# alexklibisz/deep-calcium

Measured on AMD Instinct MI355X. Metric: 512x512 summary images/sec (train step), higher is better.
Workload: dtype f32 (fp16x3 split, fp32 accumulate); 1 GPU; UNet2DS train step (fwd+BCE+bwd+Keras-Adam), batch=16 512x512 per GPU, nfb=32 (BASELINE.json configs[2]; configs[3] at 8 GPUs); global_batch=16, parallelism=dp1, bn=local

## Files before the change

### deep_calcium_amd/_build.py

```python
import os
import subprocess
import sys
from concurrent.futures import ThreadPoolExecutor

HERE = os.path.dirname(os.path.abspath(__file__))
CSRC = os.path.join(HERE, 'csrc')
LIBDIR = os.path.join(HERE, 'lib')
LIB = os.path.join(LIBDIR, 'libdcunet.so')
SOURCES = ['common.cpp', 'comm.cpp', 'nf_score.cpp', 'tape.cpp', 'igemm_conv.hip', 'igemm_f16x3.hip', 'igemm_pp.hip', 'wgrad.hip', 'wgrad_f16x3.hip', 'bwd_joint.hip', 'conv_c1.hip', 'elementwise.hip', 'series.hip', 'traces.hip', 'footprints.hip', 'roi_pairs.hip', 'trace_pairs.hip', 'frame_quality.hip', 'dff.hip', 'deconv.hip', 'trace_dyn.hip', 'spikes.hip', 'spikes_train.hip', 'motion.hip']
FLAGS = ['--offload-arch=gfx950', '-O3', '-std=c++17', '-fPIC', '-Wall', '-Wno-unused-function']
FILE_FLAGS = {'nf_score.cpp': ['-ffp-contract=off'], 'series.hip': ['-ffp-contract=off'], 'traces.hip': ['-ffp-contract=off'],
              'footprints.hip': ['-ffp-contract=off'], 'roi_pairs.hip': ['-ffp-contract=off'], 'trace_pairs.hip': ['-ffp-contract=off'],
              'frame_quality.hip': ['-ffp-contract=off'], 'dff.hip': ['-ffp-contract=off'], 'deconv.hip': ['-ffp-contract=off'],
              'trace_dyn.hip': ['-ffp-contract=off']}


def _hipcc():
    for c in (os.environ.get('HIPCC'), '/opt/rocm/bin/hipcc', 'hipcc'):
        if c and (os.path.isabs(c) and os.path.exists(c) or not os.path.isabs(c)):
            return c
    raise RuntimeError('hipcc not found')


def _newest_src():
    t = 0.0
    for root, _, files in os.walk(CSRC):
        for f in files:
            t = max(t, os.path.getmtime(os.path.join(root, f)))
    t = max(t, os.path.getmtime(os.path.join(HERE, '..', 'include', 'dcunet.h')))
    return t


def build(force=False, verbose=True):
    os.makedirs(LIBDIR, exist_ok=True)
    if not force and os.path.exists(LIB) and os.path.getmtime(LIB) >= _newest_src():
        return LIB
    hipcc = _hipcc()
    from . import _gen_tape
    _gen_tape.generate()
    objdir = os.path.join(LIBDIR, 'obj')
    os.makedirs(objdir, exist_ok=True)

    def compile_one(src):
        obj = os.path.join(objdir, os.path.splitext(src)[0] + '.o')
        cmd = [hipcc] + FLAGS + FILE_FLAGS.get(src, []) + ['-x', 'hip', '-c', os.path.join(CSRC, src), '-o', obj]
        r = subprocess.run(cmd, capture_output=True, text=True)
        if r.returncode != 0:
            raise RuntimeError('hipcc failed for %s:\n%s' % (src, r.stderr[-6000:]))
        if verbose and r.stderr.strip():
            sys.stderr.write(r.stderr)
        return obj

    with ThreadPoolExecutor(max_workers=4) as ex:
        objs = list(ex.map(compile_one, SOURCES))
    r = subprocess.run([hipcc, '--offload-arch=gfx950', '-shared', '-fPIC', '-o', LIB] + objs,
                       capture_output=True, text=True)
    if r.returncode != 0:
        raise RuntimeError('link failed:\n%s' % r.stderr[-6000:])
    return LIB


if __name__ == '__main__':
    print(build(force='--force' in sys.argv))
```

### deep_calcium_amd/csrc/tape_tramp.inc

```

static int t_dc_pack_weights(const DcArg* a) { return dc_pack_weights((const float*)a[0].p, (float*)a[1].p, (int)a[2].l, (int)a[3].l, (int)a[4].l, (long)a[5].l, (long)a[6].l, (long)a[7].l, (int)a[8].l, (dc_stream_t)a[9].p); }
static int t_dc_conv3x3_fwd(const DcArg* a) { return dc_conv3x3_fwd((const float*)a[0].p, (const float*)a[1].p, (const float*)a[2].p, (float*)a[3].p, (long)a[4].l, (double*)a[5].p, (const float*)a[6].p, (const float*)a[7].p, (int)a[8].l, (int)a[9].l, (int)a[10].l, (int)a[11].l, (int)a[12].l, (int)a[13].l, (dc_stream_t)a[14].p); }
static int t_dc_conv3x3_c1_fwd(const DcArg* a) { return dc_conv3x3_c1_fwd((const float*)a[0].p, (const float*)a[1].p, (const float*)a[2].p, (float*)a[3].p, (long)a[4].l, (double*)a[5].p, (const float*)a[6].p, (const float*)a[7].p, (int)a[8].l, (float*)a[9].p, (long)a[10].l, (int)a[11].l, (int)a[12].l, (int)a[13].l, (int)a[14].l, (dc_stream_t)a[15].p); }
static int t_dc_conv3x3_dgrad(const DcArg* a) { return dc_conv3x3_dgrad((const float*)a[0].p, (const float*)a[1].p, (float*)a[2].p, (int)a[3].l, (int)a[4].l, (int)a[5].l, (int)a[6].l, (int)a[7].l, (dc_stream_t)a[8].p); }
static int t_dc_conv3x3_wgrad(const DcArg* a) { return dc_conv3x3_wgrad((const float*)a[0].p, (const float*)a[1].p, (float*)a[2].p, (float*)a[3].p, (int)a[4].l, (int)a[5].l, (int)a[6].l, (int)a[7].l, (int)a[8].l, (dc_stream_t)a[9].p); }
static int t_dc_pack_weights_f16x3(const DcArg* a) { return dc_pack_weights_f16x3((const float*)a[0].p, (void*)a[1].p, (int)a[2].l, (int)a[3].l, (int)a[4].l, (long)a[5].l, (long)a[6].l, (long)a[7].l, (int)a[8].l, (dc_stream_t)a[9].p); }
static int t_dc_pack_weights_f16x3_batch(const DcArg* a) { return dc_pack_weights_f16x3_batch((const long*)a[0].p, (int)a[1].l, (int)a[2].l, (dc_stream_t)a[3].p); }
static int t_dc_conv3x3_fwd_f16x3(const DcArg* a) { return dc_conv3x3_fwd_f16x3((const float*)a[0].p, (const void*)a[1].p, (const float*)a[2].p, (float*)a[3].p, (long)a[4].l, (double*)a[5].p, (int)a[6].l, (const float*)a[7].p, (const float*)a[8].p, (int)a[9].l, (const float*)a[10].p, (long)a[11].l, (float*)a[12].p, (long)a[13].l, (float*)a[14].p, (int)a[15].l, (int)a[16].l, (int)a[17].l, (int)a[18].l, (int)a[19].l, (dc_stream_t)a[20].p); }
static int t_dc_conv3x3_dgrad_f16x3(const DcArg* a) { return dc_conv3x3_dgrad_f16x3((const float*)a[0].p, (const void*)a[1].p, (float*)a[2].p, (const float*)a[3].p, (const float*)a[4].p, (int)a[5].l, (float*)a[6].p, (int)a[7].l, (int)a[8].l, (int)a[9].l, (int)a[10].l, (int)a[11].l, (dc_stream_t)a[12].p); }
static int t_dc_convT2x2_fwd_f16x3(const DcArg* a) { return dc_convT2x2_fwd_f16x3((const float*)a[0].p, (const void*)a[1].p, (const float*)a[2].p, (float*)a[3].p, (long)a[4].l, (double*)a[5].p, (const float*)a[6].p, (const float*)a[7].p, (int)a[8].l, (const float*)a[9].p, (long)a[10].l, (float*)a[11].p, (long)a[12].l, (int)a[13].l, (int)a[14].l, (int)a[15].l, (int)a[16].l, (int)a[17].l, (dc_stream_t)a[18].p); }
static int t_dc_convT2x2_dgrad_f16x3(const DcArg* a) { return dc_convT2x2_dgrad_f16x3((const float*)a[0].p, (const void*)a[1].p, (float*)a[2].p, (const float*)a[3].p, (const float*)a[4].p, (int)a[5].l, (float*)a[6].p, (int)a[7].l, (int)a[8].l, (int)a[9].l, (int)a[10].l, (int)a[11].l, (dc_stream_t)a[12].p); }
static int t_dc_conv3x3_wgrad_f16x3(const DcArg* a) { return dc_conv3x3_wgrad_f16x3((const float*)a[0].p, (const float*)a[1].p, (float*)a[2].p, (float*)a[3].p, (const float*)a[4].p, (const float*)a[5].p, (int)a[6].l, (int)a[7].l, (int)a[8].l, (int)a[9].l, (int)a[10].l, (dc_stream_t)a[11].p); }
static int t_dc_convT2x2_wgrad_f16x3(const DcArg* a) { return dc_convT2x2_wgrad_f16x3((const float*)a[0].p, (const float*)a[1].p, (float*)a[2].p, (float*)a[3].p, (const float*)a[4].p, (const float*)a[5].p, (int)a[6].l, (int)a[7].l, (int)a[8].l, (int)a[9].l, (int)a[10].l, (dc_stream_t)a[11].p); }
static int t_dc_bn_stats_finalize_affine(const DcArg* a) { return dc_bn_stats_finalize_affine((const double*)a[0].p, (int)a[1].l, (int)a[2].l, (int)a[3].l, (double)a[4].d, (float)a[5].d, (float)a[6].d, (float*)a[7].p, (float*)a[8].p, (float*)a[9].p, (float*)a[10].p, (const float*)a[11].p, (const float*)a[12].p, (float*)a[13].p, (float*)a[14].p, (float*)a[15].p, (dc_stream_t)a[16].p); }
static int t_dc_conv3x3_fwd_bnin_f16x3(const DcArg* a) { return dc_conv3x3_fwd_bnin_f16x3((const float*)a[0].p, (const float*)a[1].p, (const float*)a[2].p, (const float*)a[3].p, (const void*)a[4].p, (const float*)a[5].p, (float*)a[6].p, (long)a[7].l, (double*)a[8].p, (int)a[9].l, (const float*)a[10].p, (const float*)a[11].p, (int)a[12].l, (float*)a[13].p, (int)a[14].l, (int)a[15].l, (int)a[16].l, (int)a[17].l, (int)a[18].l, (dc_stream_t)a[19].p); }
static int t_dc_convT2x2_fwd_bnin_f16x3(const DcArg* a) { return dc_convT2x2_fwd_bnin_f16x3((const float*)a[0].p, (const float*)a[1].p, (const float*)a[2].p, (const float*)a[3].p, (const void*)a[4].p, (const float*)a[5].p, (float*)a[6].p, (long)a[7].l, (double*)a[8].p, (const float*)a[9].p, (const float*)a[10].p, (int)a[11].l, (int)a[12].l, (int)a[13].l, (int)a[14].l, (int)a[15].l, (int)a[16].l, (dc_stream_t)a[17].p); }
static int t_dc_conv3x3_wgrad_bnin_f16x3(const DcArg* a) { return dc_conv3x3_wgrad_bnin_f16x3((const float*)a[0].p, (const float*)a[1].p, (const float*)a[2].p, (const float*)a[3].p, (const float*)a[4].p, (float*)a[5].p, (float*)a[6].p, (const float*)a[7].p, (int)a[8].l, (int)a[9].l, (int)a[10].l, (int)a[11].l, (int)a[12].l, (dc_stream_t)a[13].p); }
static int t_dc_convT2x2_wgrad_bnin_f16x3(const DcArg* a) { return dc_convT2x2_wgrad_bnin_f16x3((const float*)a[0].p, (const float*)a[1].p, (const float*)a[2].p, (const float*)a[3].p, (const float*)a[4].p, (float*)a[5].p, (float*)a[6].p, (const float*)a[7].p, (int)a[8].l, (int)a[9].l, (int)a[10].l, (int)a[11].l, (int)a[12].l, (dc_stream_t)a[13].p); }
static int t_dc_head_fwd_bnin(const DcArg* a) { return dc_head_fwd_bnin((const float*)a[0].p, (const float*)a[1].p, (const float*)a[2].p, (const float*)a[3].p, (const float*)a[4].p, (const uint8_t*)a[5].p, (float*)a[6].p, (float*)a[7].p, (long)a[8].l, (int)a[9].l, (dc_stream_t)a[10].p); }
static int t_dc_head_bwd_bnin(const DcArg* a) { return dc_head_bwd_bnin((const float*)a[0].p, (const float*)a[1].p, (const float*)a[2].p, (const float*)a[3].p, (const uint8_t*)a[4].p, (const float*)a[5].p, (float*)a[6].p, (float*)a[7].p, (int)a[8].l, (const double*)a[9].p, (long)a[10].l, (int)a[11].l, (dc_stream_t)a[12].p); }
static int t_dc_convT2x2_fwd(const DcArg* a) { return dc_convT2x2_fwd((const float*)a[0].p, (const float*)a[1].p, (const float*)a[2].p, (float*)a[3].p, (long)a[4].l, (double*)a[5].p, (const float*)a[6].p, (const float*)a[7].p, (int)a[8].l, (int)a[9].l, (int)a[10].l, (int)a[11].l, (int)a[12].l, (int)a[13].l, (dc_stream_t)a[14].p); }
static int t_dc_convT2x2_dgrad(const DcArg* a) { return dc_convT2x2_dgrad((const float*)a[0].p, (const float*)a[1].p, (float*)a[2].p, (int)a[3].l, (int)a[4].l, (int)a[5].l, (int)a[6].l, (int)a[7].l, (dc_stream_t)a[8].p); }
static int t_dc_convT2x2_wgrad(const DcArg* a) { return dc_convT2x2_wgrad((const float*)a[0].p, (const float*)a[1].p, (float*)a[2].p, (float*)a[3].p, (int)a[4].l, (int)a[5].l, (int)a[6].l, (int)a[7].l, (int)a[8].l, (dc_stream_t)a[9].p); }
static int t_dc_bn_stats_finalize(const DcArg* a) { return dc_bn_stats_finalize((const double*)a[0].p, (int)a[1].l, (int)a[2].l, (int)a[3].l, (double)a[4].d, (float)a[5].d, (float)a[6].d, (float*)a[7].p, (float*)a[8].p, (float*)a[9].p, (float*)a[10].p, (dc_stream_t)a[11].p); }
static int t_dc_bn_fold(const DcArg* a) { return dc_bn_fold((const float*)a[0].p, (const float*)a[1].p, (const float*)a[2].p, (const float*)a[3].p, (const float*)a[4].p, (float)a[5].d, (float*)a[6].p, (float*)a[7].p, (int)a[8].l, (dc_stream_t)a[9].p); }
static int t_dc_bn_relu_drop_fwd(const DcArg* a) { return dc_bn_relu_drop_fwd((const float*)a[0].p, (const float*)a[1].p, (const float*)a[2].p, (const float*)a[3].p, (const float*)a[4].p, (const uint8_t*)a[5].p, (float)a[6].d, (uint64_t)a[7].u, (float*)a[8].p, (long)a[9].l, (long)a[10].l, (int)a[11].l, (double)a[12].d, (float*)a[13].p, (dc_stream_t)a[14].p); }
static int t_dc_bn_relu_drop_pool_fwd(const DcArg* a) { return dc_bn_relu_drop_pool_fwd((const float*)a[0].p, (const float*)a[1].p, (const float*)a[2].p, (const float*)a[3].p, (const float*)a[4].p, (const uint8_t*)a[5].p, (float)a[6].d, (uint64_t)a[7].u, (float*)a[8].p, (long)a[9].l, (float*)a[10].p, (uint8_t*)a[11].p, (int)a[12].l, (int)a[13].l, (int)a[14].l, (int)a[15].l, (double)a[16].d, (float*)a[17].p, (dc_stream_t)a[18].p); }
static int t_dc_bn_bwd_reduce(const DcArg* a) { return dc_bn_bwd_reduce((const float*)a[0].p, (long)a[1].l, (const float*)a[2].p, (const float*)a[3].p, (const float*)a[4].p, (const float*)a[5].p, (const float*)a[6].p, (const uint8_t*)a[7].p, (float)a[8].d, (uint64_t)a[9].u, (float*)a[10].p, (float*)a[11].p, (long)a[12].l, (int)a[13].l, (dc_stream_t)a[14].p); }
static int t_dc_bn_bwd_apply(const DcArg* a) { return dc_bn_bwd_apply((const float*)a[0].p, (long)a[1].l, (const float*)a[2].p, (const float*)a[3].p, (const float*)a[4].p, (const float*)a[5].p, (const float*)a[6].p, (const uint8_t*)a[7].p, (float)a[8].d, (uint64_t)a[9].u, (const float*)a[10].p, (const float*)a[11].p, (float*)a[12].p, (float*)a[13].p, (float*)a[14].p, (long)a[15].l, (int)a[16].l, (dc_stream_t)a[17].p); }
static int t_dc_pow2_scale_from_absmax(const DcArg* a) { return dc_pow2_scale_from_absmax((const float*)a[0].p, (int)a[1].l, (float)a[2].d, (float*)a[3].p, (dc_stream_t)a[4].p); }
static int t_dc_bn_bwd_apply_finalize(const DcArg* a) { return dc_bn_bwd_apply_finalize((const float*)a[0].p, (const float*)a[1].p, (int)a[2].l, (int)a[3].l, (float)a[4].d, (float*)a[5].p, (float*)a[6].p, (dc_stream_t)a[7].p); }
static int t_dc_conv3x3_fwd_pool_f16x3(const DcArg* a) { return dc_conv3x3_fwd_pool_f16x3((const float*)a[0].p, (const void*)a[1].p, (const float*)a[2].p, (float*)a[3].p, (long)a[4].l, (const float*)a[5].p, (const float*)a[6].p, (int)a[7].l, (float*)a[8].p, (float*)a[9].p, (int)a[10].l, (int)a[11].l, (int)a[12].l, (int)a[13].l, (int)a[14].l, (dc_stream_t)a[15].p); }
static int t_dc_conv3x3_dgrad_bnred_f16x3(const DcArg* a) { return dc_conv3x3_dgrad_bnred_f16x3((const float*)a[0].p, (const void*)a[1].p, (float*)a[2].p, (const float*)a[3].p, (const float*)a[4].p, (int)a[5].l, (const float*)a[6].p, (const float*)a[7].p, (const float*)a[8].p, (const float*)a[9].p, (const float*)a[10].p, (float*)a[11].p, (float*)a[12].p, (int)a[13].l, (int)a[14].l, (int)a[15].l, (int)a[16].l, (int)a[17].l, (dc_stream_t)a[18].p); }
static int t_dc_head_bwd_bnin_bnred(const DcArg* a) { return dc_head_bwd_bnin_bnred((const float*)a[0].p, (const float*)a[1].p, (const float*)a[2].p, (const float*)a[3].p, (const uint8_t*)a[4].p, (const float*)a[5].p, (float*)a[6].p, (float*)a[7].p, (int)a[8].l, (const double*)a[9].p, (const float*)a[10].p, (const float*)a[11].p, (float*)a[12].p, (float*)a[13].p, (long)a[14].l, (int)a[15].l, (dc_stream_t)a[16].p); }
static int t_dc_convT2x2_dgrad_bnred_f16x3(const DcArg* a) { return dc_convT2x2_dgrad_bnred_f16x3((const float*)a[0].p, (const void*)a[1].p, (float*)a[2].p, (const float*)a[3].p, (const float*)a[4].p, (int)a[5].l, (const float*)a[6].p, (const float*)a[7].p, (const float*)a[8].p, (const float*)a[9].p, (const float*)a[10].p, (float*)a[11].p, (float*)a[12].p, (int)a[13].l, (int)a[14].l, (int)a[15].l, (int)a[16].l, (int)a[17].l, (dc_stream_t)a[18].p); }
static int t_dc_maxpool2x2_bwd_bnred(const DcArg* a) { return dc_maxpool2x2_bwd_bnred((const float*)a[0].p, (const uint8_t*)a[1].p, (const float*)a[2].p, (long)a[3].l, (float*)a[4].p, (const float*)a[5].p, (const float*)a[6].p, (const float*)a[7].p, (const float*)a[8].p, (const float*)a[9].p, (const uint8_t*)a[10].p, (float)a[11].d, (uint64_t)a[12].u, (float*)a[13].p, (float*)a[14].p, (int)a[15].l, (int)a[16].l, (int)a[17].l, (int)a[18].l, (dc_stream_t)a[19].p); }
static int t_dc_bn_bwd_finalize_dzin(const DcArg* a) { return dc_bn_bwd_finalize_dzin((const float*)a[0].p, (const float*)a[1].p, (int)a[2].l, (int)a[3].l, (const float*)a[4].p, (const float*)a[5].p, (const float*)a[6].p, (const float*)a[7].p, (double)a[8].d, (float*)a[9].p, (float*)a[10].p, (float*)a[11].p, (float*)a[12].p, (dc_stream_t)a[13].p); }
static int t_dc_conv3x3_dgrad_dzin_f16x3(const DcArg* a) { return dc_conv3x3_dgrad_dzin_f16x3((const float*)a[0].p, (const float*)a[1].p, (const float*)a[2].p, (const void*)a[3].p, (float*)a[4].p, (float*)a[5].p, (const float*)a[6].p, (const float*)a[7].p, (const float*)a[8].p, (const float*)a[9].p, (const float*)a[10].p, (float*)a[11].p, (float*)a[12].p, (int)a[13].l, (int)a[14].l, (int)a[15].l, (int)a[16].l, (int)a[17].l, (dc_stream_t)a[18].p); }
static int t_dc_conv3x3_wgrad_dzin_f16x3(const DcArg* a) { return dc_conv3x3_wgrad_dzin_f16x3((const float*)a[0].p, (const float*)a[1].p, (const float*)a[2].p, (const float*)a[3].p, (const float*)a[4].p, (const float*)a[5].p, (const float*)a[6].p, (float*)a[7].p, (float*)a[8].p, (int)a[9].l, (int)a[10].l, (int)a[11].l, (int)a[12].l, (int)a[13].l, (dc_stream_t)a[14].p); }
static int t_dc_conv3x3_c1_wgrad_dzin_zre(const DcArg* a) { return dc_conv3x3_c1_wgrad_dzin_zre((const float*)a[0].p, (const float*)a[1].p, (const float*)a[2].p, (const float*)a[3].p, (const float*)a[4].p, (float*)a[5].p, (float*)a[6].p, (int)a[7].l, (int)a[8].l, (int)a[9].l, (int)a[10].l, (dc_stream_t)a[11].p); }
static int t_dc_conv3x3_bwd_joint_f16x3(const DcArg* a) { return dc_conv3x3_bwd_joint_f16x3((const float*)a[0].p, (const float*)a[1].p, (const float*)a[2].p, (const float*)a[3].p, (const float*)a[4].p, (const float*)a[5].p, (const float*)a[6].p, (const void*)a[7].p, (float*)a[8].p, (const float*)a[9].p, (const float*)a[10].p, (const float*)a[11].p, (const float*)a[12].p, (const float*)a[13].p, (float*)a[14].p, (float*)a[15].p, (float*)a[16].p, (float*)a[17].p, (int)a[18].l, (int)a[19].l, (int)a[20].l, (int)a[21].l, (int)a[22].l, (dc_stream_t)a[23].p); }
static int t_dc_conv3x3_bwd_joint_r1_f16x3(const DcArg* a) { return dc_conv3x3_bwd_joint_r1_f16x3((const float*)a[0].p, (const float*)a[1].p, (const float*)a[2].p, (const float*)a[3].p, (const float*)a[4].p, (const float*)a[5].p, (const float*)a[6].p, (const float*)a[7].p, (const void*)a[8].p, (float*)a[9].p, (const float*)a[10].p, (const float*)a[11].p, (const float*)a[12].p, (const float*)a[13].p, (const float*)a[14].p, (float*)a[15].p, (float*)a[16].p, (float*)a[17].p, (float*)a[18].p, (int)a[19].l, (int)a[20].l, (int)a[21].l, (int)a[22].l, (int)a[23].l, (dc_stream_t)a[24].p); }
static int t_dc_bn_stats_reduce(const DcArg* a) { return dc_bn_stats_reduce((const double*)a[0].p, (int)a[1].l, (int)a[2].l, (int)a[3].l, (double*)a[4].p, (dc_stream_t)a[5].p); }
static int t_dc_bn_stats_rows_fold(const DcArg* a) { return dc_bn_stats_rows_fold((const double*)a[0].p, (int)a[1].l, (int)a[2].l, (int)a[3].l, (int)a[4].l, (double*)a[5].p, (dc_stream_t)a[6].p); }
static int t_dc_bn_stats_finalize_sums(const DcArg* a) { return dc_bn_stats_finalize_sums((const double*)a[0].p, (int)a[1].l, (double)a[2].d, (float)a[3].d, (float)a[4].d, (float*)a[5].p, (float*)a[6].p, (float*)a[7].p, (float*)a[8].p, (const float*)a[9].p, (const float*)a[10].p, (float*)a[11].p, (float*)a[12].p, (float*)a[13].p, (dc_stream_t)a[14].p); }
static int t_dc_bn_bwd_apply_count(const DcArg* a) { return dc_bn_bwd_apply_count((const float*)a[0].p, (long)a[1].l, (const float*)a[2].p, (const float*)a[3].p, (const float*)a[4].p, (const float*)a[5].p, (const float*)a[6].p, (const uint8_t*)a[7].p, (float)a[8].d, (uint64_t)a[9].u, (const float*)a[10].p, (const float*)a[11].p, (float*)a[12].p, (float*)a[13].p, (float*)a[14].p, (long)a[15].l, (double)a[16].d, (int)a[17].l, (dc_stream_t)a[18].p); }
static int t_dc_maxpool2x2_fwd(const DcArg* a) { return dc_maxpool2x2_fwd((const float*)a[0].p, (long)a[1].l, (float*)a[2].p, (uint8_t*)a[3].p, (int)a[4].l, (int)a[5].l, (int)a[6].l, (int)a[7].l, (dc_stream_t)a[8].p); }
static int t_dc_maxpool2x2_bwd(const DcArg* a) { return dc_maxpool2x2_bwd((const float*)a[0].p, (const uint8_t*)a[1].p, (const float*)a[2].p, (long)a[3].l, (float*)a[4].p, (int)a[5].l, (int)a[6].l, (int)a[7].l, (int)a[8].l, (dc_stream_t)a[9].p); }
static int t_dc_upsample2x_drop_fwd(const DcArg* a) { return dc_upsample2x_drop_fwd((const float*)a[0].p, (float*)a[1].p, (long)a[2].l, (const uint8_t*)a[3].p, (float)a[4].d, (uint64_t)a[5].u, (const float*)a[6].p, (long)a[7].l, (float*)a[8].p, (long)a[9].l, (int)a[10].l, (int)a[11].l, (int)a[12].l, (int)a[13].l, (dc_stream_t)a[14].p); }
static int t_dc_upsample2x_drop_bwd(const DcArg* a) { return dc_upsample2x_drop_bwd((const float*)a[0].p, (long)a[1].l, (const uint8_t*)a[2].p, (float)a[3].d, (uint64_t)a[4].u, (float*)a[5].p, (int)a[6].l, (int)a[7].l, (int)a[8].l, (int)a[9].l, (dc_stream_t)a[10].p); }
static int t_dc_head_fwd(const DcArg* a) { return dc_head_fwd((const float*)a[0].p, (const float*)a[1].p, (const float*)a[2].p, (const uint8_t*)a[3].p, (float*)a[4].p, (float*)a[5].p, (long)a[6].l, (int)a[7].l, (dc_stream_t)a[8].p); }
static int t_dc_head_bwd(const DcArg* a) { return dc_head_bwd((const float*)a[0].p, (const float*)a[1].p, (const uint8_t*)a[2].p, (const float*)a[3].p, (float*)a[4].p, (float*)a[5].p, (int)a[6].l, (const double*)a[7].p, (long)a[8].l, (int)a[9].l, (dc_stream_t)a[10].p); }
static int t_dc_head_fwd_bwd(const DcArg* a) { return dc_head_fwd_bwd((const float*)a[0].p, (const float*)a[1].p, (const float*)a[2].p, (const float*)a[3].p, (const float*)a[4].p, (const uint8_t*)a[5].p, (float*)a[6].p, (float*)a[7].p, (float*)a[8].p, (float*)a[9].p, (int)a[10].l, (const float*)a[11].p, (const float*)a[12].p, (float*)a[13].p, (float*)a[14].p, (long)a[15].l, (int)a[16].l, (dc_stream_t)a[17].p); }
static int t_dc_head_fwd_bwd_s(const DcArg* a) { return dc_head_fwd_bwd_s((const float*)a[0].p, (const float*)a[1].p, (const float*)a[2].p, (const float*)a[3].p, (const float*)a[4].p, (const uint8_t*)a[5].p, (float*)a[6].p, (float*)a[7].p, (float*)a[8].p, (float*)a[9].p, (int)a[10].l, (const float*)a[11].p, (const float*)a[12].p, (float*)a[13].p, (float*)a[14].p, (long)a[15].l, (int)a[16].l, (dc_stream_t)a[17].p); }
static int t_dc_head_bwd_bnin_bnred_s(const DcArg* a) { return dc_head_bwd_bnin_bnred_s((const float*)a[0].p, (const float*)a[1].p, (const float*)a[2].p, (const float*)a[3].p, (const uint8_t*)a[4].p, (const float*)a[5].p, (float*)a[6].p, (float*)a[7].p, (int)a[8].l, (const double*)a[9].p, (const float*)a[10].p, (const float*)a[11].p, (float*)a[12].p, (float*)a[13].p, (long)a[14].l, (int)a[15].l, (dc_stream_t)a[16].p); }
static int t_dc_head_grad_finalize(const DcArg* a) { return dc_head_grad_finalize((const float*)a[0].p, (int)a[1].l, (int)a[2].l, (float*)a[3].p, (float*)a[4].p, (dc_stream_t)a[5].p); }
static int t_dc_reduce_partials(const DcArg* a) { return dc_reduce_partials((const float*)a[0].p, (int)a[1].l, (long)a[2].l, (float)a[3].d, (float*)a[4].p, (float*)a[5].p, (dc_stream_t)a[6].p); }
static int t_dc_reduce_partials_f64(const DcArg* a) { return dc_reduce_partials_f64((const float*)a[0].p, (int)a[1].l, (int)a[2].l, (double*)a[3].p, (dc_stream_t)a[4].p); }
static int t_dc_bn_bwd_finalize(const DcArg* a) { return dc_bn_bwd_finalize((const float*)a[0].p, (int)a[1].l, (int)a[2].l, (float*)a[3].p, (float*)a[4].p, (dc_stream_t)a[5].p); }
static int t_dc_adam_step_flat(const DcArg* a) { return dc_adam_step_flat((float*)a[0].p, (const float*)a[1].p, (float*)a[2].p, (float*)a[3].p, (long)a[4].l, (float)a[5].d, (float)a[6].d, (float)a[7].d, (float)a[8].d, (float)a[9].d, (dc_stream_t)a[10].p); }
static int t_dc_gather_maps(const DcArg* a) { return dc_gather_maps((const float*)a[0].p, (const int*)a[1].p, (float*)a[2].p, (int)a[3].l, (long)a[4].l, (dc_stream_t)a[5].p); }
static int t_dc_tta_merge(const DcArg* a) { return dc_tta_merge((const float*)a[0].p, (const int*)a[1].p, (int)a[2].l, (int)a[3].l, (int)a[4].l, (int)a[5].l, (int)a[6].l, (double)a[7].d, (uint8_t*)a[8].p, (float*)a[9].p, (dc_stream_t)a[10].p); }
static int t_dc_round_window_u8(const DcArg* a) { return dc_round_window_u8((const float*)a[0].p, (int)a[1].l, (int)a[2].l, (int)a[3].l, (int)a[4].l, (int)a[5].l, (int)a[6].l, (int)a[7].l, (uint8_t*)a[8].p, (dc_stream_t)a[9].p); }
static int t_dc_series_accumulate(const DcArg* a) { return dc_series_accumulate((const void*)a[0].p, (int)a[1].l, (int)a[2].l, (long)a[3].l, (long)a[4].l, (uint16_t*)a[5].p, (int16_t*)a[6].p, (long*)a[7].p, (long*)a[8].p, (int*)a[9].p, (int)a[10].l, (int)a[11].l, (dc_stream_t)a[12].p); }
static int t_dc_series_accumulate_xy(const DcArg* a) { return dc_series_accumulate_xy((const void*)a[0].p, (int)a[1].l, (int)a[2].l, (long)a[3].l, (long*)a[4].p, (int)a[5].l, (int)a[6].l, (dc_stream_t)a[7].p); }
static int t_dc_series_finalize(const DcArg* a) { return dc_series_finalize((const long*)a[0].p, (const long*)a[1].p, (const long*)a[2].p, (float*)a[3].p, (float*)a[4].p, (float*)a[5].p, (int)a[6].l, (int)a[7].l, (long)a[8].l, (dc_stream_t)a[9].p); }
static int t_dc_image_standardize(const DcArg* a) { return dc_image_standardize((const float*)a[0].p, (float*)a[1].p, (float*)a[2].p, (int)a[3].l, (int)a[4].l, (dc_stream_t)a[5].p); }
static int t_dc_series_bin_time(const DcArg* a) { return dc_series_bin_time((const void*)a[0].p, (int)a[1].l, (int)a[2].l, (int)a[3].l, (int)a[4].l, (int)a[5].l, (int)a[6].l, (int*)a[7].p, (void*)a[8].p, (dc_stream_t)a[9].p); }
static int t_dc_roi_trace_accumulate(const DcArg* a) { return dc_roi_trace_accumulate((const void*)a[0].p, (int)a[1].l, (int)a[2].l, (long)a[3].l, (const int*)a[4].p, (const int*)a[5].p, (const int*)a[6].p, (int)a[7].l, (int)a[8].l, (long*)a[9].p, (long)a[10].l, (int)a[11].l, (int)a[12].l, (dc_stream_t)a[13].p); }
static int t_dc_roi_trace_finalize(const DcArg* a) { return dc_roi_trace_finalize((const long*)a[0].p, (long)a[1].l, (const int*)a[2].p, (int)a[3].l, (long)a[4].l, (float*)a[5].p, (float*)a[6].p, (dc_stream_t)a[7].p); }
static int t_dc_roi_wtrace_accumulate(const DcArg* a) { return dc_roi_wtrace_accumulate((const void*)a[0].p, (int)a[1].l, (int)a[2].l, (long)a[3].l, (const int*)a[4].p, (const int*)a[5].p, (const unsigned short*)a[6].p, (const int*)a[7].p, (int)a[8].l, (int)a[9].l, (long*)a[10].p, (long)a[11].l, (int)a[12].l, (int)a[13].l, (dc_stream_t)a[14].p); }
static int t_dc_roi_pixel_accumulate(const DcArg* a) { return dc_roi_pixel_accumulate((const void*)a[0].p, (int)a[1].l, (int)a[2].l, (long)a[3].l, (const int*)a[4].p, (const int*)a[5].p, (const int*)a[6].p, (int)a[7].l, (int)a[8].l, (const long*)a[9].p, (long)a[10].l, (long*)a[11].p, (int)a[12].l, (int)a[13].l, (int)a[14].l, (dc_stream_t)a[15].p); }
static int t_dc_roi_trace_moments(const DcArg* a) { return dc_roi_trace_moments((const long*)a[0].p, (long)a[1].l, (int)a[2].l, (long)a[3].l, (long*)a[4].p, (dc_stream_t)a[5].p); }
static int t_dc_roi_pixel_corr(const DcArg* a) { return dc_roi_pixel_corr((const long*)a[0].p, (int)a[1].l, (const int*)a[2].p, (const int*)a[3].p, (int)a[4].l, (int)a[5].l, (const int*)a[6].p, (const long*)a[7].p, (long)a[8].l, (float*)a[9].p, (dc_stream_t)a[10].p); }
static int t_dc_roi_pair_accumulate(const DcArg* a) { return dc_roi_pair_accumulate((const void*)a[0].p, (int)a[1].l, (int)a[2].l, (const int*)a[3].p, (const int*)a[4].p, (const long*)a[5].p, (const int*)a[6].p, (long)a[7].l, (int)a[8].l, (long*)a[9].p, (long*)a[10].p, (int)a[11].l, (long)a[12].l, (int)a[13].l, (int)a[14].l, (dc_stream_t)a[15].p); }
static int t_dc_roi_pair_corr(const DcArg* a) { return dc_roi_pair_corr((const long*)a[0].p, (const long*)a[1].p, (const int*)a[2].p, (const long*)a[3].p, (int)a[4].l, (int)a[5].l, (long)a[6].l, (long)a[7].l, (float*)a[8].p, (dc_stream_t)a[9].p); }
static int t_dc_series_fold_segment(const DcArg* a) { return dc_series_fold_segment((const long*)a[0].p, (const long*)a[1].p, (const long*)a[2].p, (const int*)a[3].p, (long)a[4].l, (long)a[5].l, (long*)a[6].p, (long*)a[7].p, (long*)a[8].p, (int*)a[9].p, (int)a[10].l, (int)a[11].l, (dc_stream_t)a[12].p); }
static int t_dc_series_finalize_pooled(const DcArg* a) { return dc_series_finalize_pooled((const long*)a[0].p, (const long*)a[1].p, (const long*)a[2].p, (float*)a[3].p, (float*)a[4].p, (float*)a[5].p, (int)a[6].l, (int)a[7].l, (long)a[8].l, (long)a[9].l, (dc_stream_t)a[10].p); }
static int t_dc_roi_pair_fold_segment(const DcArg* a) { return dc_roi_pair_fold_segment((long*)a[0].p, (long*)a[1].p, (const int*)a[2].p, (const long*)a[3].p, (const int*)a[4].p, (long)a[5].l, (int)a[6].l, (int)a[7].l, (long)a[8].l, (long)a[9].l, (long)a[10].l, (long*)a[11].p, (dc_stream_t)a[12].p); }
static int t_dc_roi_pair_corr_pooled(const DcArg* a) { return dc_roi_pair_corr_pooled((const long*)a[0].p, (const int*)a[1].p, (const long*)a[2].p, (int)a[3].l, (int)a[4].l, (long)a[5].l, (float*)a[6].p, (dc_stream_t)a[7].p); }
static int t_dc_roi_pixel_fold_segment(const DcArg* a) { return dc_roi_pixel_fold_segment((long*)a[0].p, (int)a[1].l, (const int*)a[2].p, (const int*)a[3].p, (int)a[4].l, (int)a[5].l, (const long*)a[6].p, (long)a[7].l, (long)a[8].l, (long*)a[9].p, (long*)a[10].p, (long*)a[11].p, (int)a[12].l, (int)a[13].l, (dc_stream_t)a[14].p); }
static int t_dc_roi_pixel_corr_pooled(const DcArg* a) { return dc_roi_pixel_corr_pooled((const long*)a[0].p, (const long*)a[1].p, (const long*)a[2].p, (int)a[3].l, (const int*)a[4].p, (const int*)a[5].p, (int)a[6].l, (int)a[7].l, (const int*)a[8].p, (float*)a[9].p, (dc_stream_t)a[10].p); }
static int t_dc_trace_pair_moments(const DcArg* a) { return dc_trace_pair_moments((const long*)a[0].p, (long)a[1].l, (int)a[2].l, (long)a[3].l, (int)a[4].l, (const int*)a[5].p, (long)a[6].l, (long*)a[7].p, (dc_stream_t)a[8].p); }
static int t_dc_trace_pair_corr(const DcArg* a) { return dc_trace_pair_corr((const long*)a[0].p, (long)a[1].l, (float*)a[2].p, (dc_stream_t)a[3].p); }
static int t_dc_frame_moments(const DcArg* a) { return dc_frame_moments((const void*)a[0].p, (int)a[1].l, (int)a[2].l, (const void*)a[3].p, (int)a[4].l, (int)a[5].l, (int)a[6].l, (int)a[7].l, (int)a[8].l, (int)a[9].l, (long*)a[10].p, (dc_stream_t)a[11].p); }
static int t_dc_frame_quality(const DcArg* a) { return dc_frame_quality((const long*)a[0].p, (int)a[1].l, (long)a[2].l, (long)a[3].l, (long)a[4].l, (float*)a[5].p, (float*)a[6].p, (dc_stream_t)a[7].p); }
static int t_dc_frame_gather(const DcArg* a) { return dc_frame_gather((const void*)a[0].p, (int)a[1].l, (const int*)a[2].p, (int)a[3].l, (int)a[4].l, (int)a[5].l, (void*)a[6].p, (dc_stream_t)a[7].p); }
static int t_dc_trace_combine(const DcArg* a) { return dc_trace_combine((const long*)a[0].p, (long)a[1].l, (const int*)a[2].p, (const long*)a[3].p, (const long*)a[4].p, (const long*)a[5].p, (int)a[6].l, (long)a[7].l, (long*)a[8].p, (dc_stream_t)a[9].p); }
static int t_dc_trace_baseline(const DcArg* a) { return dc_trace_baseline((const long*)a[0].p, (long)a[1].l, (int)a[2].l, (long)a[3].l, (int)a[4].l, (int)a[5].l, (long*)a[6].p, (float*)a[7].p, (dc_stream_t)a[8].p); }
static int t_dc_trace_scale(const DcArg* a) { return dc_trace_scale((const long*)a[0].p, (long)a[1].l, (const long*)a[2].p, (int)a[3].l, (long)a[4].l, (float*)a[5].p, (dc_stream_t)a[6].p); }
static int t_dc_trace_deconv_ar1(const DcArg* a) { return dc_trace_deconv_ar1((const void*)a[0].p, (int)a[1].l, (long)a[2].l, (int)a[3].l, (long)a[4].l, (double)a[5].d, (const double*)a[6].p, (const double*)a[7].p, (const double*)a[8].p, (void*)a[9].p, (double*)a[10].p, (double*)a[11].p, (int*)a[12].p, (dc_stream_t)a[13].p); }
static int t_dc_trace_deconv_ar1_host(const DcArg* a) { return dc_trace_deconv_ar1_host((const void*)a[0].p, (int)a[1].l, (long)a[2].l, (int)a[3].l, (long)a[4].l, (const double*)a[5].p, (const double*)a[6].p, (const double*)a[7].p, (double*)a[8].p, (double*)a[9].p, (int*)a[10].p); }
static int t_dc_trace_deconv_ar1_constrained(const DcArg* a) { return dc_trace_deconv_ar1_constrained((const void*)a[0].p, (int)a[1].l, (long)a[2].l, (int)a[3].l, (long)a[4].l, (double)a[5].d, (const double*)a[6].p, (const double*)a[7].p, (long)a[8].l, (int)a[9].l, (const double*)a[10].p, (const double*)a[11].p, (int)a[12].l, (void*)a[13].p, (void*)a[14].p, (double*)a[15].p, (double*)a[16].p, (int*)a[17].p, (double*)a[18].p, (double*)a[19].p, (int*)a[20].p, (dc_stream_t)a[21].p); }
static int t_dc_trace_deconv_search_step(const DcArg* a) { return dc_trace_deconv_search_step((const void*)a[0].p, (int)a[1].l, (long)a[2].l, (int)a[3].l, (long)a[4].l, (const double*)a[5].p, (long)a[6].l, (const void*)a[7].p, (const int*)a[8].p, (int)a[9].l, (void*)a[10].p, (double*)a[11].p, (double*)a[12].p, (int*)a[13].p, (dc_stream_t)a[14].p); }
static int t_dc_trace_deconv_ar1_constrained_host(const DcArg* a) { return dc_trace_deconv_ar1_constrained_host((const void*)a[0].p, (int)a[1].l, (long)a[2].l, (int)a[3].l, (long)a[4].l, (const double*)a[5].p, (int)a[6].l, (const double*)a[7].p, (const double*)a[8].p, (int)a[9].l, (double*)a[10].p, (double*)a[11].p, (int*)a[12].p, (double*)a[13].p, (double*)a[14].p, (int*)a[15].p); }
static int t_dc_trace_deconv_ar1_base(const DcArg* a) { return dc_trace_deconv_ar1_base((const void*)a[0].p, (int)a[1].l, (long)a[2].l, (int)a[3].l, (long)a[4].l, (double)a[5].d, (const double*)a[6].p, (const double*)a[7].p, (long)a[8].l, (const double*)a[9].p, (const double*)a[10].p, (const double*)a[11].p, (void*)a[12].p, (double*)a[13].p, (double*)a[14].p, (int*)a[15].p, (dc_stream_t)a[16].p); }
static int t_dc_trace_deconv_ar1_fit_base(const DcArg* a) { return dc_trace_deconv_ar1_fit_base((const void*)a[0].p, (int)a[1].l, (long)a[2].l, (int)a[3].l, (long)a[4].l, (double)a[5].d, (const double*)a[6].p, (const double*)a[7].p, (long)a[8].l, (const double*)a[9].p, (const double*)a[10].p, (int)a[11].l, (void*)a[12].p, (double*)a[13].p, (double*)a[14].p, (int*)a[15].p, (double*)a[16].p, (dc_stream_t)a[17].p); }
static int t_dc_trace_deconv_ar1_constrained_base(const DcArg* a) { return dc_trace_deconv_ar1_constrained_base((const void*)a[0].p, (int)a[1].l, (long)a[2].l, (int)a[3].l, (long)a[4].l, (double)a[5].d, (const double*)a[6].p, (const double*)a[7].p, (long)a[8].l, (int)a[9].l, (const double*)a[10].p, (const double*)a[11].p, (int)a[12].l, (void*)a[13].p, (void*)a[14].p, (double*)a[15].p, (double*)a[16].p, (int*)a[17].p, (double*)a[18].p, (double*)a[19].p, (double*)a[20].p, (int*)a[21].p, (dc_stream_t)a[22].p); }
static int t_dc_trace_deconv_base_step(const DcArg* a) { return dc_trace_deconv_base_step((const void*)a[0].p, (int)a[1].l, (long)a[2].l, (int)a[3].l, (long)a[4].l, (const double*)a[5].p, (long)a[6].l, (const void*)a[7].p, (const int*)a[8].p, (int)a[9].l, (void*)a[10].p, (double*)a[11].p, (double*)a[12].p, (double*)a[13].p, (int*)a[14].p, (double*)a[15].p, (dc_stream_t)a[16].p); }
static int t_dc_trace_deconv_ar1_fit_base_host(const DcArg* a) { return dc_trace_deconv_ar1_fit_base_host((const void*)a[0].p, (int)a[1].l, (long)a[2].l, (int)a[3].l, (long)a[4].l, (const double*)a[5].p, (long)a[6].l, (const double*)a[7].p, (const double*)a[8].p, (int)a[9].l, (double*)a[10].p, (double*)a[11].p, (int*)a[12].p, (double*)a[13].p); }
static int t_dc_trace_deconv_ar1_constrained_base_host(const DcArg* a) { return dc_trace_deconv_ar1_constrained_base_host((const void*)a[0].p, (int)a[1].l, (long)a[2].l, (int)a[3].l, (long)a[4].l, (const double*)a[5].p, (long)a[6].l, (int)a[7].l, (const double*)a[8].p, (const double*)a[9].p, (int)a[10].l, (double*)a[11].p, (double*)a[12].p, (int*)a[13].p, (double*)a[14].p, (double*)a[15].p, (double*)a[16].p, (int*)a[17].p); }
static int t_dc_trace_deconv_ar2(const DcArg* a) { return dc_trace_deconv_ar2((const void*)a[0].p, (int)a[1].l, (long)a[2].l, (int)a[3].l, (long)a[4].l, (double)a[5].d, (double)a[6].d, (const double*)a[7].p, (long)a[8].l, (const double*)a[9].p, (const double*)a[10].p, (const double*)a[11].p, (void*)a[12].p, (double*)a[13].p, (double*)a[14].p, (int*)a[15].p, (dc_stream_t)a[16].p); }
static int t_dc_trace_deconv_ar2_host(const DcArg* a) { return dc_trace_deconv_ar2_host((const void*)a[0].p, (int)a[1].l, (long)a[2].l, (int)a[3].l, (long)a[4].l, (double)a[5].d, (double)a[6].d, (const double*)a[7].p, (long)a[8].l, (const double*)a[9].p, (const double*)a[10].p, (const double*)a[11].p, (double*)a[12].p, (double*)a[13].p, (int*)a[14].p); }
static int t_dc_trace_deconv_ar2_constrained(const DcArg* a) { return dc_trace_deconv_ar2_constrained((const void*)a[0].p, (int)a[1].l, (long)a[2].l, (int)a[3].l, (long)a[4].l, (double)a[5].d, (double)a[6].d, (const double*)a[7].p, (long)a[8].l, (int)a[9].l, (const double*)a[10].p, (const double*)a[11].p, (int)a[12].l, (void*)a[13].p, (void*)a[14].p, (double*)a[15].p, (double*)a[16].p, (int*)a[17].p, (double*)a[18].p, (double*)a[19].p, (int*)a[20].p, (dc_stream_t)a[21].p); }
static int t_dc_trace_deconv_ar2_constrained_host(const DcArg* a) { return dc_trace_deconv_ar2_constrained_host((const void*)a[0].p, (int)a[1].l, (long)a[2].l, (int)a[3].l, (long)a[4].l, (double)a[5].d, (double)a[6].d, (const double*)a[7].p, (long)a[8].l, (int)a[9].l, (const double*)a[10].p, (const double*)a[11].p, (int)a[12].l, (double*)a[13].p, (double*)a[14].p, (int*)a[15].p, (double*)a[16].p, (double*)a[17].p, (int*)a[18].p); }
static int t_dc_trace_noise(const DcArg* a) { return dc_trace_noise((const void*)a[0].p, (int)a[1].l, (long)a[2].l, (int)a[3].l, (long)a[4].l, (double*)a[5].p, (dc_stream_t)a[6].p); }
static int t_dc_trace_ar1_estimate(const DcArg* a) { return dc_trace_ar1_estimate((const void*)a[0].p, (int)a[1].l, (long)a[2].l, (int)a[3].l, (long)a[4].l, (int)a[5].l, (const double*)a[6].p, (double*)a[7].p, (double*)a[8].p, (double*)a[9].p, (dc_stream_t)a[10].p); }
static int t_dc_ar1_tables(const DcArg* a) { return dc_ar1_tables((const double*)a[0].p, (int)a[1].l, (long)a[2].l, (double*)a[3].p, (long)a[4].l, (dc_stream_t)a[5].p); }
static int t_dc_trace_deconv_ar1_each(const DcArg* a) { return dc_trace_deconv_ar1_each((const void*)a[0].p, (int)a[1].l, (long)a[2].l, (int)a[3].l, (long)a[4].l, (const double*)a[5].p, (const double*)a[6].p, (long)a[7].l, (const double*)a[8].p, (const double*)a[9].p, (void*)a[10].p, (double*)a[11].p, (double*)a[12].p, (int*)a[13].p, (dc_stream_t)a[14].p); }
static int t_dc_trace_ar1_estimate_host(const DcArg* a) { return dc_trace_ar1_estimate_host((const void*)a[0].p, (int)a[1].l, (long)a[2].l, (int)a[3].l, (long)a[4].l, (int)a[5].l, (const double*)a[6].p, (double*)a[7].p, (double*)a[8].p, (double*)a[9].p); }
static int t_dc_motion_ssd(const DcArg* a) { return dc_motion_ssd((const void*)a[0].p, (int)a[1].l, (int)a[2].l, (const void*)a[3].p, (int)a[4].l, (int)a[5].l, (int)a[6].l, (long*)a[7].p, (dc_stream_t)a[8].p); }
static int t_dc_motion_pick(const DcArg* a) { return dc_motion_pick((const long*)a[0].p, (int)a[1].l, (int)a[2].l, (int*)a[3].p, (long*)a[4].p, (dc_stream_t)a[5].p); }
static int t_dc_motion_apply(const DcArg* a) { return dc_motion_apply((const void*)a[0].p, (int)a[1].l, (const int*)a[2].p, (int)a[3].l, (int)a[4].l, (int)a[5].l, (void*)a[6].p, (dc_stream_t)a[7].p); }
static int t_dc_motion_block_ssd(const DcArg* a) { return dc_motion_block_ssd((const void*)a[0].p, (int)a[1].l, (int)a[2].l, (const void*)a[3].p, (int)a[4].l, (int)a[5].l, (int)a[6].l, (int)a[7].l, (int)a[8].l, (int)a[9].l, (const int*)a[10].p, (long*)a[11].p, (dc_stream_t)a[12].p); }
static int t_dc_motion_block_pick(const DcArg* a) { return dc_motion_block_pick((const long*)a[0].p, (const int*)a[1].p, (int)a[2].l, (int)a[3].l, (int)a[4].l, (int)a[5].l, (int)a[6].l, (int*)a[7].p, (long*)a[8].p, (dc_stream_t)a[9].p); }
static int t_dc_motion_warp(const DcArg* a) { return dc_motion_warp((const void*)a[0].p, (int)a[1].l, (const int*)a[2].p, (int)a[3].l, (int)a[4].l, (int)a[5].l, (int)a[6].l, (int)a[7].l, (void*)a[8].p, (dc_stream_t)a[9].p); }
static int t_dc_motion_refine(const DcArg* a) { return dc_motion_refine((const long*)a[0].p, (const int*)a[1].p, (int)a[2].l, (int)a[3].l, (int*)a[4].p, (dc_stream_t)a[5].p); }
static int t_dc_motion_block_refine(const DcArg* a) { return dc_motion_block_refine((const long*)a[0].p, (const int*)a[1].p, (const int*)a[2].p, (int)a[3].l, (int)a[4].l, (int)a[5].l, (int)a[6].l, (int)a[7].l, (int*)a[8].p, (dc_stream_t)a[9].p); }
static int t_dc_motion_apply_sub(const DcArg* a) { return dc_motion_apply_sub((const void*)a[0].p, (int)a[1].l, (int)a[2].l, (const int*)a[3].p, (int)a[4].l, (int)a[5].l, (int)a[6].l, (void*)a[7].p, (dc_stream_t)a[8].p); }
static int t_dc_motion_warp_sub(const DcArg* a) { return dc_motion_warp_sub((const void*)a[0].p, (int)a[1].l, (int)a[2].l, (const int*)a[3].p, (int)a[4].l, (int)a[5].l, (int)a[6].l, (int)a[7].l, (int)a[8].l, (void*)a[9].p, (dc_stream_t)a[10].p); }
static int t_dc_motion_bin(const DcArg* a) { return dc_motion_bin((const void*)a[0].p, (int)a[1].l, (int)a[2].l, (int)a[3].l, (int)a[4].l, (int)a[5].l, (void*)a[6].p, (dc_stream_t)a[7].p); }
static int t_dc_motion_ssd_around(const DcArg* a) { return dc_motion_ssd_around((const void*)a[0].p, (int)a[1].l, (int)a[2].l, (const void*)a[3].p, (int)a[4].l, (int)a[5].l, (int)a[6].l, (int)a[7].l, (const int*)a[8].p, (int)a[9].l, (long*)a[10].p, (dc_stream_t)a[11].p); }
static int t_dc_motion_pick_around(const DcArg* a) { return dc_motion_pick_around((const long*)a[0].p, (const int*)a[1].p, (int)a[2].l, (int)a[3].l, (int)a[4].l, (int)a[5].l, (int*)a[6].p, (long*)a[7].p, (int*)a[8].p, (dc_stream_t)a[9].p); }
static int t_dc_bidi_scores(const DcArg* a) { return dc_bidi_scores((const void*)a[0].p, (int)a[1].l, (int)a[2].l, (int)a[3].l, (int)a[4].l, (int)a[5].l, (long*)a[6].p, (dc_stream_t)a[7].p); }
static int t_dc_bidi_apply(const DcArg* a) { return dc_bidi_apply((const void*)a[0].p, (int)a[1].l, (int)a[2].l, (int)a[3].l, (int)a[4].l, (int)a[5].l, (void*)a[6].p, (dc_stream_t)a[7].p); }
static int t_dc_conv1d_k5_fwd(const DcArg* a) { return dc_conv1d_k5_fwd((const float*)a[0].p, (const float*)a[1].p, (const float*)a[2].p, (const float*)a[3].p, (int)a[4].l, (float*)a[5].p, (long)a[6].l, (int)a[7].l, (int)a[8].l, (int)a[9].l, (int)a[10].l, (dc_stream_t)a[11].p); }
static int t_dc_conv1d_k5_c1_fwd(const DcArg* a) { return dc_conv1d_k5_c1_fwd((const float*)a[0].p, (const float*)a[1].p, (const float*)a[2].p, (const float*)a[3].p, (int)a[4].l, (float*)a[5].p, (long)a[6].l, (int)a[7].l, (int)a[8].l, (int)a[9].l, (dc_stream_t)a[10].p); }
static int t_dc_maxpool1d_2_fwd(const DcArg* a) { return dc_maxpool1d_2_fwd((const float*)a[0].p, (long)a[1].l, (float*)a[2].p, (int)a[3].l, (int)a[4].l, (int)a[5].l, (dc_stream_t)a[6].p); }
static int t_dc_upsample1d_2x_fwd(const DcArg* a) { return dc_upsample1d_2x_fwd((const float*)a[0].p, (float*)a[1].p, (long)a[2].l, (int)a[3].l, (int)a[4].l, (int)a[5].l, (dc_stream_t)a[6].p); }
static int t_dc_spike_head_fwd(const DcArg* a) { return dc_spike_head_fwd((const float*)a[0].p, (const float*)a[1].p, (const float*)a[2].p, (int)a[3].l, (float*)a[4].p, (int)a[5].l, (int)a[6].l, (int)a[7].l, (dc_stream_t)a[8].p); }
static int t_dc_conv1d_stats(const DcArg* a) { return dc_conv1d_stats((const float*)a[0].p, (long)a[1].l, (double*)a[2].p, (long)a[3].l, (int)a[4].l, (dc_stream_t)a[5].p); }
static int t_dc_conv1d_k5_wgrad(const DcArg* a) { return dc_conv1d_k5_wgrad((const float*)a[0].p, (const float*)a[1].p, (float*)a[2].p, (float*)a[3].p, (int)a[4].l, (int)a[5].l, (int)a[6].l, (int)a[7].l, (dc_stream_t)a[8].p); }
static int t_dc_conv1d_k5_c1_wgrad(const DcArg* a) { return dc_conv1d_k5_c1_wgrad((const float*)a[0].p, (const float*)a[1].p, (float*)a[2].p, (float*)a[3].p, (int)a[4].l, (int)a[5].l, (int)a[6].l, (dc_stream_t)a[7].p); }
static int t_dc_maxpool1d_2_bwd(const DcArg* a) { return dc_maxpool1d_2_bwd((const float*)a[0].p, (const float*)a[1].p, (long)a[2].l, (const float*)a[3].p, (long)a[4].l, (float*)a[5].p, (long)a[6].l, (int)a[7].l, (int)a[8].l, (int)a[9].l, (dc_stream_t)a[10].p); }
static int t_dc_upsample1d_2x_drop_fwd(const DcArg* a) { return dc_upsample1d_2x_drop_fwd((const float*)a[0].p, (float*)a[1].p, (long)a[2].l, (const uint8_t*)a[3].p, (float)a[4].d, (uint64_t)a[5].u, (int)a[6].l, (int)a[7].l, (int)a[8].l, (dc_stream_t)a[9].p); }
static int t_dc_upsample1d_2x_drop_bwd(const DcArg* a) { return dc_upsample1d_2x_drop_bwd((const float*)a[0].p, (long)a[1].l, (const uint8_t*)a[2].p, (float)a[3].d, (uint64_t)a[4].u, (float*)a[5].p, (int)a[6].l, (int)a[7].l, (int)a[8].l, (dc_stream_t)a[9].p); }
static int t_dc_spike_head_train_fwd(const DcArg* a) { return dc_spike_head_train_fwd((const float*)a[0].p, (const float*)a[1].p, (const float*)a[2].p, (int)a[3].l, (const uint8_t*)a[4].p, (float)a[5].d, (float)a[6].d, (float*)a[7].p, (float*)a[8].p, (int)a[9].l, (int)a[10].l, (int)a[11].l, (dc_stream_t)a[12].p); }
static int t_dc_spike_head_train_bwd(const DcArg* a) { return dc_spike_head_train_bwd((const float*)a[0].p, (const float*)a[1].p, (const float*)a[2].p, (int)a[3].l, (const uint8_t*)a[4].p, (float)a[5].d, (float)a[6].d, (float*)a[7].p, (float*)a[8].p, (int)a[9].l, (int)a[10].l, (int)a[11].l, (dc_stream_t)a[12].p); }
static int t_dc_fill(const DcArg* a) { return dc_fill((float*)a[0].p, (long)a[1].l, (float)a[2].d, (dc_stream_t)a[3].p); }
static int t_dc_scale_flat(const DcArg* a) { return dc_scale_flat((float*)a[0].p, (long)a[1].l, (float)a[2].d, (dc_stream_t)a[3].p); }
static int t_dc_stream_wait_event(const DcArg* a) { return dc_stream_wait_event((dc_stream_t)a[0].p, (void*)a[1].p); }
static int t_dc_event_record(const DcArg* a) { return dc_event_record((void*)a[0].p, (dc_stream_t)a[1].p); }
static int t_dc_comm_all_reduce_sum(const DcArg* a) { return dc_comm_all_reduce_sum((void*)a[0].p, (float*)a[1].p, (long)a[2].l, (dc_stream_t)a[3].p); }
static int t_dc_comm_all_reduce_sum_f64(const DcArg* a) { return dc_comm_all_reduce_sum_f64((void*)a[0].p, (double*)a[1].p, (long)a[2].l, (dc_stream_t)a[3].p); }
static int t_dc_comm_group_start(const DcArg* a) { return dc_comm_group_start(); }
static int t_dc_comm_group_end(const DcArg* a) { return dc_comm_group_end(); }

static const DcTapeFn kTapeFns[] = {
  {"dc_pack_weights", t_dc_pack_weights, 10, "pplllllllp"},
  {"dc_conv3x3_fwd", t_dc_conv3x3_fwd, 15, "pppplpppllllllp"},
  {"dc_conv3x3_c1_fwd", t_dc_conv3x3_c1_fwd, 16, "pppplppplplllllp"},
  {"dc_conv3x3_dgrad", t_dc_conv3x3_dgrad, 9, "ppplllllp"},
  {"dc_conv3x3_wgrad", t_dc_conv3x3_wgrad, 10, "pppplllllp"},
  {"dc_pack_weights_f16x3", t_dc_pack_weights_f16x3, 10, "pplllllllp"},
  {"dc_pack_weights_f16x3_batch", t_dc_pack_weights_f16x3_batch, 4, "pllp"},
  {"dc_conv3x3_fwd_f16x3", t_dc_conv3x3_fwd_f16x3, 21, "pppplplpplplplplllllp"},
  {"dc_conv3x3_dgrad_f16x3", t_dc_conv3x3_dgrad_f16x3, 13, "ppppplplllllp"},
  {"dc_convT2x2_fwd_f16x3", t_dc_convT2x2_fwd_f16x3, 19, "pppplppplplpllllllp"},
  {"dc_convT2x2_dgrad_f16x3", t_dc_convT2x2_dgrad_f16x3, 13, "ppppplplllllp"},
  {"dc_conv3x3_wgrad_f16x3", t_dc_conv3x3_wgrad_f16x3, 12, "pppppplllllp"},
  {"dc_convT2x2_wgrad_f16x3", t_dc_convT2x2_wgrad_f16x3, 12, "pppppplllllp"},
  {"dc_bn_stats_finalize_affine", t_dc_bn_stats_finalize_affine, 17, "pllldddpppppppppp"},
  {"dc_conv3x3_fwd_bnin_f16x3", t_dc_conv3x3_fwd_bnin_f16x3, 20, "ppppppplplpplplllllp"},
  {"dc_convT2x2_fwd_bnin_f16x3", t_dc_convT2x2_fwd_bnin_f16x3, 18, "ppppppplpppllllllp"},
  {"dc_conv3x3_wgrad_bnin_f16x3", t_dc_conv3x3_wgrad_bnin_f16x3, 14, "pppppppplllllp"},
  {"dc_convT2x2_wgrad_bnin_f16x3", t_dc_convT2x2_wgrad_bnin_f16x3, 14, "pppppppplllllp"},
  {"dc_head_fwd_bnin", t_dc_head_fwd_bnin, 11, "ppppppppllp"},
  {"dc_head_bwd_bnin", t_dc_head_bwd_bnin, 13, "pppppppplpllp"},
  {"dc_convT2x2_fwd", t_dc_convT2x2_fwd, 15, "pppplpppllllllp"},
  {"dc_convT2x2_dgrad", t_dc_convT2x2_dgrad, 9, "ppplllllp"},
  {"dc_convT2x2_wgrad", t_dc_convT2x2_wgrad, 10, "pppplllllp"},
  {"dc_bn_stats_finalize", t_dc_bn_stats_finalize, 12, "pllldddppppp"},
  {"dc_bn_fold", t_dc_bn_fold, 10, "pppppdpplp"},
  {"dc_bn_relu_drop_fwd", t_dc_bn_relu_drop_fwd, 15, "ppppppdupllldpp"},
  {"dc_bn_relu_drop_pool_fwd", t_dc_bn_relu_drop_pool_fwd, 19, "ppppppduplpplllldpp"},
  {"dc_bn_bwd_reduce", t_dc_bn_bwd_reduce, 15, "plppppppduppllp"},
  {"dc_bn_bwd_apply", t_dc_bn_bwd_apply, 18, "plppppppdupppppllp"},
  {"dc_pow2_scale_from_absmax", t_dc_pow2_scale_from_absmax, 5, "pldpp"},
  {"dc_bn_bwd_apply_finalize", t_dc_bn_bwd_apply_finalize, 8, "pplldppp"},
  {"dc_conv3x3_fwd_pool_f16x3", t_dc_conv3x3_fwd_pool_f16x3, 16, "pppplpplpplllllp"},
  {"dc_conv3x3_dgrad_bnred_f16x3", t_dc_conv3x3_dgrad_bnred_f16x3, 19, "ppppplppppppplllllp"},
  {"dc_head_bwd_bnin_bnred", t_dc_head_bwd_bnin_bnred, 17, "pppppppplpppppllp"},
  {"dc_convT2x2_dgrad_bnred_f16x3", t_dc_convT2x2_dgrad_bnred_f16x3, 19, "ppppplppppppplllllp"},
  {"dc_maxpool2x2_bwd_bnred", t_dc_maxpool2x2_bwd_bnred, 20, "ppplpppppppduppllllp"},
  {"dc_bn_bwd_finalize_dzin", t_dc_bn_bwd_finalize_dzin, 14, "ppllppppdppppp"},
  {"dc_conv3x3_dgrad_dzin_f16x3", t_dc_conv3x3_dgrad_dzin_f16x3, 19, "ppppppppppppplllllp"},
  {"dc_conv3x3_wgrad_dzin_f16x3", t_dc_conv3x3_wgrad_dzin_f16x3, 15, "ppppppppplllllp"},
  {"dc_conv3x3_c1_wgrad_dzin_zre", t_dc_conv3x3_c1_wgrad_dzin_zre, 12, "pppppppllllp"},
  {"dc_conv3x3_bwd_joint_f16x3", t_dc_conv3x3_bwd_joint_f16x3, 24, "pppppppppppppppppplllllp"},
  {"dc_conv3x3_bwd_joint_r1_f16x3", t_dc_conv3x3_bwd_joint_r1_f16x3, 25, "ppppppppppppppppppplllllp"},
  {"dc_bn_stats_reduce", t_dc_bn_stats_reduce, 6, "plllpp"},
  {"dc_bn_stats_rows_fold", t_dc_bn_stats_rows_fold, 7, "pllllpp"},
  {"dc_bn_stats_finalize_sums", t_dc_bn_stats_finalize_sums, 15, "pldddpppppppppp"},
  {"dc_bn_bwd_apply_count", t_dc_bn_bwd_apply_count, 19, "plppppppdupppppldlp"},
  {"dc_maxpool2x2_fwd", t_dc_maxpool2x2_fwd, 9, "plppllllp"},
  {"dc_maxpool2x2_bwd", t_dc_maxpool2x2_bwd, 10, "ppplpllllp"},
  {"dc_upsample2x_drop_fwd", t_dc_upsample2x_drop_fwd, 15, "pplpduplplllllp"},
  {"dc_upsample2x_drop_bwd", t_dc_upsample2x_drop_bwd, 11, "plpdupllllp"},
  {"dc_head_fwd", t_dc_head_fwd, 9, "ppppppllp"},
  {"dc_head_bwd", t_dc_head_bwd, 11, "pppppplpllp"},
  {"dc_head_fwd_bwd", t_dc_head_fwd_bwd, 18, "pppppppppplppppllp"},
  {"dc_head_fwd_bwd_s", t_dc_head_fwd_bwd_s, 18, "pppppppppplppppllp"},
  {"dc_head_bwd_bnin_bnred_s", t_dc_head_bwd_bnin_bnred_s, 17, "pppppppplpppppllp"},
  {"dc_head_grad_finalize", t_dc_head_grad_finalize, 6, "pllppp"},
  {"dc_reduce_partials", t_dc_reduce_partials, 7, "plldppp"},
  {"dc_reduce_partials_f64", t_dc_reduce_partials_f64, 5, "pllpp"},
  {"dc_bn_bwd_finalize", t_dc_bn_bwd_finalize, 6, "pllppp"},
  {"dc_adam_step_flat", t_dc_adam_step_flat, 11, "ppppldddddp"},
  {"dc_gather_maps", t_dc_gather_maps, 6, "pppllp"},
  {"dc_tta_merge", t_dc_tta_merge, 11, "ppllllldppp"},
  {"dc_round_window_u8", t_dc_round_window_u8, 10, "plllllllpp"},
  {"dc_series_accumulate", t_dc_series_accumulate, 13, "pllllpppppllp"},
  {"dc_series_accumulate_xy", t_dc_series_accumulate_xy, 8, "plllpllp"},
  {"dc_series_finalize", t_dc_series_finalize, 10, "pppppplllp"},
  {"dc_image_standardize", t_dc_image_standardize, 6, "pppllp"},
  {"dc_series_bin_time", t_dc_series_bin_time, 10, "pllllllppp"},
  {"dc_roi_trace_accumulate", t_dc_roi_trace_accumulate, 14, "plllpppllplllp"},
  {"dc_roi_trace_finalize", t_dc_roi_trace_finalize, 8, "plpllppp"},
  {"dc_roi_wtrace_accumulate", t_dc_roi_wtrace_accumulate, 15, "plllppppllplllp"},
  {"dc_roi_pixel_accumulate", t_dc_roi_pixel_accumulate, 16, "plllpppllplplllp"},
  {"dc_roi_trace_moments", t_dc_roi_trace_moments, 6, "plllpp"},
  {"dc_roi_pixel_corr", t_dc_roi_pixel_corr, 11, "plppllpplpp"},
  {"dc_roi_pair_accumulate", t_dc_roi_pair_accumulate, 16, "pllppppllppllllp"},
  {"dc_roi_pair_corr", t_dc_roi_pair_corr, 10, "ppppllllpp"},
  {"dc_series_fold_segment", t_dc_series_fold_segment, 13, "ppppllppppllp"},
  {"dc_series_finalize_pooled", t_dc_series_finalize_pooled, 11, "ppppppllllp"},
  {"dc_roi_pair_fold_segment", t_dc_roi_pair_fold_segment, 13, "pppppllllllpp"},
  {"dc_roi_pair_corr_pooled", t_dc_roi_pair_corr_pooled, 8, "ppplllpp"},
  {"dc_roi_pixel_fold_segment", t_dc_roi_pixel_fold_segment, 15, "plppllpllpppllp"},
  {"dc_roi_pixel_corr_pooled", t_dc_roi_pixel_corr_pooled, 11, "ppplppllppp"},
  {"dc_trace_pair_moments", t_dc_trace_pair_moments, 9, "pllllplpp"},
  {"dc_trace_pair_corr", t_dc_trace_pair_corr, 4, "plpp"},
  {"dc_frame_moments", t_dc_frame_moments, 12, "pllpllllllpp"},
  {"dc_frame_quality", t_dc_frame_quality, 8, "pllllppp"},
  {"dc_frame_gather", t_dc_frame_gather, 8, "plplllpp"},
  {"dc_trace_combine", t_dc_trace_combine, 10, "plppppllpp"},
  {"dc_trace_baseline", t_dc_trace_baseline, 9, "plllllppp"},
  {"dc_trace_scale", t_dc_trace_scale, 7, "plpllpp"},
  {"dc_trace_deconv_ar1", t_dc_trace_deconv_ar1, 14, "plllldpppppppp"},
  {"dc_trace_deconv_ar1_host", t_dc_trace_deconv_ar1_host, 11, "pllllpppppp"},
  {"dc_trace_deconv_ar1_constrained", t_dc_trace_deconv_ar1_constrained, 22, "plllldppllpplppppppppp"},
  {"dc_trace_deconv_search_step", t_dc_trace_deconv_search_step, 15, "pllllplpplppppp"},
  {"dc_trace_deconv_ar1_constrained_host", t_dc_trace_deconv_ar1_constrained_host, 16, "pllllplpplpppppp"},
  {"dc_trace_deconv_ar1_base", t_dc_trace_deconv_ar1_base, 17, "plllldpplpppppppp"},
  {"dc_trace_deconv_ar1_fit_base", t_dc_trace_deconv_ar1_fit_base, 18, "plllldpplpplpppppp"},
  {"dc_trace_deconv_ar1_constrained_base", t_dc_trace_deconv_ar1_constrained_base, 23, "plllldppllpplpppppppppp"},
  {"dc_trace_deconv_base_step", t_dc_trace_deconv_base_step, 17, "pllllplpplppppppp"},
  {"dc_trace_deconv_ar1_fit_base_host", t_dc_trace_deconv_ar1_fit_base_host, 14, "pllllplpplpppp"},
  {"dc_trace_deconv_ar1_constrained_base_host", t_dc_trace_deconv_ar1_constrained_base_host, 18, "pllllpllpplppppppp"},
  {"dc_trace_deconv_ar2", t_dc_trace_deconv_ar2, 17, "pllllddplpppppppp"},
  {"dc_trace_deconv_ar2_host", t_dc_trace_deconv_ar2_host, 15, "pllllddplpppppp"},
  {"dc_trace_deconv_ar2_constrained", t_dc_trace_deconv_ar2_constrained, 22, "pllllddpllpplppppppppp"},
  {"dc_trace_deconv_ar2_constrained_host", t_dc_trace_deconv_ar2_constrained_host, 19, "pllllddpllpplpppppp"},
  {"dc_trace_noise", t_dc_trace_noise, 7, "pllllpp"},
  {"dc_trace_ar1_estimate", t_dc_trace_ar1_estimate, 11, "plllllppppp"},
  {"dc_ar1_tables", t_dc_ar1_tables, 6, "pllplp"},
  {"dc_trace_deconv_ar1_each", t_dc_trace_deconv_ar1_each, 15, "pllllpplppppppp"},
  {"dc_trace_ar1_estimate_host", t_dc_trace_ar1_estimate_host, 10, "plllllpppp"},
  {"dc_motion_ssd", t_dc_motion_ssd, 9, "pllplllpp"},
  {"dc_motion_pick", t_dc_motion_pick, 6, "pllppp"},
  {"dc_motion_apply", t_dc_motion_apply, 8, "plplllpp"},
  {"dc_motion_block_ssd", t_dc_motion_block_ssd, 13, "pllpllllllppp"},
  {"dc_motion_block_pick", t_dc_motion_block_pick, 10, "pplllllppp"},
  {"dc_motion_warp", t_dc_motion_warp, 10, "plplllllpp"},
  {"dc_motion_refine", t_dc_motion_refine, 6, "ppllpp"},
  {"dc_motion_block_refine", t_dc_motion_block_refine, 10, "ppplllllpp"},
  {"dc_motion_apply_sub", t_dc_motion_apply_sub, 9, "pllplllpp"},
  {"dc_motion_warp_sub", t_dc_motion_warp_sub, 11, "pllplllllpp"},
  {"dc_motion_bin", t_dc_motion_bin, 8, "plllllpp"},
  {"dc_motion_ssd_around", t_dc_motion_ssd_around, 12, "pllpllllplpp"},
  {"dc_motion_pick_around", t_dc_motion_pick_around, 10, "ppllllpppp"},
  {"dc_bidi_scores", t_dc_bidi_scores, 8, "plllllpp"},
  {"dc_bidi_apply", t_dc_bidi_apply, 8, "plllllpp"},
  {"dc_conv1d_k5_fwd", t_dc_conv1d_k5_fwd, 12, "pppplplllllp"},
  {"dc_conv1d_k5_c1_fwd", t_dc_conv1d_k5_c1_fwd, 11, "pppplpllllp"},
  {"dc_maxpool1d_2_fwd", t_dc_maxpool1d_2_fwd, 7, "plplllp"},
  {"dc_upsample1d_2x_fwd", t_dc_upsample1d_2x_fwd, 7, "ppllllp"},
  {"dc_spike_head_fwd", t_dc_spike_head_fwd, 9, "ppplplllp"},
  {"dc_conv1d_stats", t_dc_conv1d_stats, 6, "plpllp"},
  {"dc_conv1d_k5_wgrad", t_dc_conv1d_k5_wgrad, 9, "ppppllllp"},
  {"dc_conv1d_k5_c1_wgrad", t_dc_conv1d_k5_c1_wgrad, 8, "pppplllp"},
  {"dc_maxpool1d_2_bwd", t_dc_maxpool1d_2_bwd, 11, "pplplpllllp"},
  {"dc_upsample1d_2x_drop_fwd", t_dc_upsample1d_2x_drop_fwd, 10, "pplpdulllp"},
  {"dc_upsample1d_2x_drop_bwd", t_dc_upsample1d_2x_drop_bwd, 10, "plpduplllp"},
  {"dc_spike_head_train_fwd", t_dc_spike_head_train_fwd, 13, "ppplpddpplllp"},
  {"dc_spike_head_train_bwd", t_dc_spike_head_train_bwd, 13, "ppplpddpplllp"},
  {"dc_fill", t_dc_fill, 4, "pldp"},
  {"dc_scale_flat", t_dc_scale_flat, 4, "pldp"},
  {"dc_stream_wait_event", t_dc_stream_wait_event, 2, "pp"},
  {"dc_event_record", t_dc_event_record, 2, "pp"},
  {"dc_comm_all_reduce_sum", t_dc_comm_all_reduce_sum, 4, "pplp"},
  {"dc_comm_all_reduce_sum_f64", t_dc_comm_all_reduce_sum_f64, 4, "pplp"},
  {"dc_comm_group_start", t_dc_comm_group_start, 0, ""},
  {"dc_comm_group_end", t_dc_comm_group_end, 0, ""},
};
```

### deep_calcium_amd/net.py

```python
import collections
import os
import threading

import numpy as np
import torch

from . import parallel
from ._lib import lib, DcunetError, Tape, Var, ops_equal

BN_EPS = 1e-3


def _ptr(t, offset_floats=0):
    return t.data_ptr() + 4 * offset_floats


def _on_device(fn):
    import functools

    @functools.wraps(fn)
    def wrapped(self, *a, **k):
        if torch.cuda.current_device() == self.device.index:
            return fn(self, *a, **k)
        with torch.cuda.device(self.device):
            return fn(self, *a, **k)
    return wrapped


from .layers import LayerSpec, build_layer_table, assign_offsets, split_weights


_PINNED = collections.OrderedDict()
_PINNED_MAX_BYTES = 512 << 20
_PINNED_LOCK = threading.Lock()


def _pinned(tag, shape, dtype, entry=False):
    key = (tag, tuple(shape), dtype, threading.get_ident())
    with _PINNED_LOCK:
        ent = _PINNED.get(key)
        if ent is not None:
            _PINNED.move_to_end(key)
            return ent if entry else ent[0]
    new = [torch.empty(tuple(shape), dtype=dtype).pin_memory(), None]
    with _PINNED_LOCK:
        ent = _PINNED.setdefault(key, new)
        total = sum(e[0].numel() * e[0].element_size() for e in _PINNED.values())
        while total > _PINNED_MAX_BYTES and len(_PINNED) > 1:
            k0 = next(iter(_PINNED))
            if k0 == key:
                break
            old = _PINNED.pop(k0)
            total -= old[0].numel() * old[0].element_size()
    return ent if entry else ent[0]


class _TtaJob(object):

    def __init__(self, eng, count, augmentations):
        self.eng, self.count = eng, int(count)
        self.aug = list(augmentations) if augmentations is not None else [('identity', lambda a: a, lambda a: a)]
        K, H, W = len(self.aug), eng.H, eng.W
        n = H * W
        dev = eng.device
        key = ('ttamaps', K, tuple(name for name, _, _ in self.aug))
        m = eng._bufs.get(key)
        if m is None:
            idx = np.arange(n, dtype=np.int32).reshape(1, H, W)
            fwd = np.stack([np.ascontiguousarray(f(idx)).reshape(-1) for _, f, _ in self.aug])
            inv = np.stack([np.ascontiguousarray(g(idx)).reshape(-1) for _, _, g in self.aug])
            if fwd.shape != (K, n) or inv.shape != (K, n):
                raise ValueError('test-time augmentations must map (N,H,W) to (N,H,W) on a square window')
            m = eng._bufs[key] = dict(fwd=torch.from_numpy(fwd).to(dev), inv=torch.from_numpy(inv).to(dev),
                                      x=torch.empty((K, H, W), dtype=torch.float32, device=dev),
                                      src=[torch.empty(n, dtype=torch.float32, device=dev) for _ in range(2)])
        self.m = m
        self.host = [_pinned('tta_img%d' % k, (H, W), torch.float32, entry=True) for k in range(2)]
        self.mask = torch.empty((self.count, n), dtype=torch.uint8, device=dev)
        self.mask_host = _pinned('tta_mask', (max(self.count, 1), n), torch.uint8)
        self.ovf = torch.zeros(max(self.count, 1), dtype=torch.float32, device=dev)
        self.jobs = [None] * self.count

    def enqueue(self, i, img, hs, ws, threshold):
        eng, m = self.eng, self.m
        K, H, W = len(self.aug), eng.H, eng.W
        with torch.cuda.device(eng.device):
            L, st = eng.L, eng._stream()
            k = i & 1
            slot = self.host[k]
            if slot[1] is not None:
                slot[1].synchronize()
            slot[0].numpy()[...] = img
            m['src'][k].copy_(slot[0].view(-1), non_blocking=True)
            ev = torch.cuda.Event()
            ev.record()
            slot[1] = ev
            L.dc_gather_maps(_ptr(m['src'][k]), m['fwd'].data_ptr(), _ptr(m['x']), K, H * W, st)
            p = eng.forward_infer(m['x'])
            if eng.mfma == 'f16x3' and eng.range_guard and not eng.infer_measured:
                self.ovf[i:i + 1].copy_(eng._ovf[0:1])
            L.dc_tta_merge(_ptr(p), m['inv'].data_ptr(), K, H, W, int(hs), int(ws), float(threshold),
                           self.mask[i].data_ptr(), None, st)
            self.mask_host[i, :hs * ws].copy_(self.mask[i, :hs * ws], non_blocking=True)
        self.jobs[i] = (np.array(img, dtype=np.float32, copy=True), int(hs), int(ws), float(threshold))

    def finish(self):
        eng = self.eng
        torch.cuda.current_stream(eng.device).synchronize()
        redo = [i for i, f in enumerate(self.ovf.cpu().numpy()[:self.count]) if f != 0.0 and self.jobs[i] is not None]
        out = []
        for i, j in enumerate(self.jobs):
            if j is None:
                out.append(None)
                continue
            _, hs, ws, _ = j
            out.append(self.mask_host[i, :hs * ws].numpy().reshape(hs, ws).copy())
        if redo:
            eng.infer_measured = True
            for i in redo:
                img, hs, ws, thr = self.jobs[i]
                out[i] = eng.predict_tta(img, self.aug, hs, ws, thr)
        return out


class UNetEngine(object):
    SLOTS = 3
    FOLD_MIN = int(os.environ.get('DC_STATS_FOLD_MIN', '8192'))
    FOLD_ROWS = 128
    SLOTS_DEEP = 32
    SLOTS_DEEP_MAX_BYTES = 48 << 30

    def __init__(self, window_shape, nb_filters_base=32, prop_dropout_base=0.25, device=None, seed=7535, mfma=None,
                 upsampling=False, bn_mode=None, conv_kernel_init='he_normal'):
        self.mfma = mfma or os.environ.get('DC_MFMA', 'f16x3')
        if self.mfma not in ('f16x3', 'f32'):
            raise ValueError("mfma must be 'f16x3' or 'f32', got %r" % self.mfma)
        self.streams = 1 if os.environ.get('DC_STREAMS', '2') == '1' else 2
        self.bnin = self.mfma == 'f16x3' and os.environ.get('DC_BNIN', '1') == '1'
        _dz = os.environ.get('DC_DZIN', '1')
        self.dzin = self.mfma == 'f16x3' and _dz != '0'
        self.dzin_lvls = frozenset(range(5)) if _dz == 'all' else frozenset((0,))
        self.dzin_all = _dz == 'all'
        self.joint = self.dzin and _dz != '2'
        self._head_bwd_done = False
        self.range_guard = self.mfma == 'f16x3'
        self.infer_measured = os.environ.get('DC_INFER_GUARD', '0') == '1'
        bn_mode = bn_mode or os.environ.get('DC_BN_MODE', 'local')
        if bn_mode not in ('local', 'sync'):
            raise ValueError("bn_mode must be 'local' or 'sync', got %r" % (bn_mode,))
        self.bn_mode = bn_mode
        self.loss_kind = 0
        H, W = window_shape
        if H % 16 or W % 16:
            raise ValueError('window_shape must be a multiple of 16 (4 max-pools), got %r' % (window_shape,))
        nfb = nb_filters_base
        if nfb < 4 or nfb & (nfb - 1) or nfb > 64:
            raise ValueError('nb_filters_base must be a power of two in [4, 64]')
        if not torch.cuda.is_available():
            raise DcunetError('no GPU visible: the UNet2DS engine has no CPU fallback')
        self.L = lib()
        self.H, self.W, self.nfb, self.drp = H, W, nfb, float(prop_dropout_base)
        self.device = torch.device(device if device is not None else 'cuda:%d' % torch.cuda.current_device())
        if self.device.type != 'cuda':
            raise DcunetError('the UNet2DS engine runs on a GPU only, got device %r' % (device,))
        if self.device.index is None:
            self.device = torch.device('cuda', torch.cuda.current_device())
        self.upsampling = bool(upsampling)
        self.layers = build_layer_table(nfb, self.drp, self.upsampling)
        self.up_drop = {3: 2 * self.drp, 2: 2 * self.drp, 1: 2 * self.drp, 0: self.drp}
        self.by_name = {l.name: l for l in self.layers}
        nm = []
        if self.bnin:
            nm += ['e%da' % i for i in range(4)] + ['ba'] + ['d%da' % i for i in range(4)] + ['d0b']
            if not self.upsampling:
                nm += ['bb', 'd3b', 'd2b', 'd1b']
        self.nm = frozenset(n for n in nm if self.by_name[n].drop <= 0.0)
        off, soff = assign_offsets(self.layers)
        self.n_train = off
        self.n_stats = soff
        npad = (off + 3) // 4 * 4
        dev = self.device
        self.pflat = torch.zeros(npad, dtype=torch.float32, device=dev)
        self.gflat = torch.zeros(npad, dtype=torch.float32, device=dev)
        self.mflat = torch.zeros(npad, dtype=torch.float32, device=dev)
        self.vflat = torch.zeros(npad, dtype=torch.float32, device=dev)
        self.sflat = torch.zeros(soff, dtype=torch.float32, device=dev)
        self.bstat = torch.zeros(6 * soff // 2 + 8, dtype=torch.float32, device=dev)
        self._stat_off = {}
        o = 0
        for l in self.layers:
            if l.kind != 'head':
                self._stat_off[l.name] = o
                o += 6 * l.cout
        self.wp_fwd, self.wp_dgrad = {}, {}
        for l in self.layers:
            if l.kind == 'head' or (l.kind == 'conv' and l.cin == 1):
                continue
            n = int(np.prod(l.kshape))
            if self.mfma == 'f16x3':
                sz = self.L.dc_pack_weights_f16x3_floats
                fw, bw = ((9, l.cin, l.cout), (9, l.cout, l.cin)) if l.kind == 'conv' else ((1, l.cin, 4 * l.cout), (4, l.cout, l.cin))
                self.wp_fwd[l.name] = torch.empty(sz(*fw), dtype=torch.float32, device=dev)
                self.wp_dgrad[l.name] = torch.empty(sz(*bw), dtype=torch.float32, device=dev)
            else:
                self.wp_fwd[l.name] = torch.empty(n, dtype=torch.float32, device=dev)
                self.wp_dgrad[l.name] = torch.empty(n, dtype=torch.float32, device=dev)
        self._ab_off, self._ab_ld = {}, {}
        o = 0
        for lvl in range(4):
            self._ab_off['cat%d' % lvl], self._ab_ld['cat%d' % lvl] = o, self._cup(lvl) + (nfb << lvl)
            o += 8 * self._ab_ld['cat%d' % lvl]
        for l in self.layers:
            if l.kind != 'head':
                self._ab_off[l.name], self._ab_ld[l.name] = o, l.cout
                o += 8 * l.cout
        self.abound = torch.zeros(o, dtype=torch.float32, device=dev)
        self._ovf = torch.zeros(4, dtype=torch.float32, device=dev)
        self._bufs = {}
        self.dz_writeback = False
        self.deep_slots = False
        self.c1_z_on_load = True
        self.head_rank1 = True
        self.tail_main = os.environ.get('DC_TAIL_MAIN', '1') == '1'
        self.stats_per_wg = True
        self.use_tapes = os.environ.get('DC_TAPES', '1') != '0'
        self.tape_verify = int(os.environ.get('DC_TAPE_VERIFY', '0'))
        self.ar_buckets = 1 if os.environ.get('DC_AR_BUCKETS', '3') == '1' else 3
        self._tapes = {}
        self._tape_epoch = 0
        self.ar_probe = None
        self.tape_replays = 0
        self._side_stream = torch.cuda.Stream(device=self.device)
        with torch.cuda.device(self.device):
            torch.cuda.Event().record(self._side_stream)
        self._evpool, self._ev_i = [], 0
        self._evpool_f, self._evf_i = [], 0
        self._tail = None
        self._packed_dirty = True
        self._fold_dirty = True
        self.iterations = 0
        self.drop_seed = 0x5eed0000 + seed
        if conv_kernel_init is not None:
            self.set_weights(self.initial_weights(seed, conv_kernel_init))

    def initial_weights(self, seed=7535, conv_kernel_init='he_normal'):
        rs = np.random.RandomState(seed)

        def tn(shape, std):
            out = rs.standard_normal(shape)
            bad = np.abs(out) > 2
            while bad.any():
                out[bad] = rs.standard_normal(int(bad.sum()))
                bad = np.abs(out) > 2
            return (out * std).astype(np.float32)

        vs = {'he_normal': (2.0, 'fan_in', 'normal'), 'he_uniform': (2.0, 'fan_in', 'uniform'),
              'glorot_normal': (1.0, 'fan_avg', 'normal'), 'glorot_uniform': (1.0, 'fan_avg', 'uniform'),
              'lecun_normal': (1.0, 'fan_in', 'normal'), 'lecun_uniform': (1.0, 'fan_in', 'uniform')}

        def init(name, shape):
            if callable(name):
                return np.asarray(name(shape), np.float32).reshape(shape)
            rf = shape[0] * shape[1]
            fan_in, fan_out = shape[2] * rf, shape[3] * rf
            if name in vs:
                scale, mode, dist = vs[name]
                scale /= max(1.0, {'fan_in': fan_in, 'fan_out': fan_out, 'fan_avg': (fan_in + fan_out) / 2.0}[mode])
                if dist == 'normal':
                    return tn(shape, np.sqrt(scale))
                lim = np.sqrt(3.0 * scale)
                return rs.uniform(-lim, lim, shape).astype(np.float32)
            if name in ('random_normal', 'normal'):
                return (rs.standard_normal(shape) * 0.05).astype(np.float32)
            if name == 'truncated_normal':
                return tn(shape, 0.05)
            if name in ('random_uniform', 'uniform'):
                return rs.uniform(-0.05, 0.05, shape).astype(np.float32)
            if name in ('zeros', 'zero'):
                return np.zeros(shape, np.float32)
            if name in ('ones', 'one'):
                return np.ones(shape, np.float32)
            raise ValueError('conv_kernel_init %r: not a Keras-2.0.6 initializer this build restates (%s, random_normal, '
                             'random_uniform, truncated_normal, zeros, ones, or a callable shape -> array)'
                             % (name, ', '.join(sorted(vs))))

        W = []
        for l in self.layers:
            W.append(init('glorot_uniform' if l.kind == 'head' else conv_kernel_init, l.kshape))
            W.append(np.zeros(l.cout, np.float32))
            if l.kind != 'head':
                W += [np.ones(l.cout, np.float32), np.zeros(l.cout, np.float32),
                      np.zeros(l.cout, np.float32), np.ones(l.cout, np.float32)]
        return W

    def weight_shapes(self):
        out = []
        for l in self.layers:
            out += [l.kshape, (l.cout,)]
            if l.kind != 'head':
                out += [(l.cout,)] * 4
        return out

    def get_weights(self, p=None, s=None):
        p = self.pflat.cpu().numpy() if p is None else p
        s = self.sflat.cpu().numpy() if s is None else s
        return split_weights(self.layers, p, s)

    def set_weights(self, weights):
        shapes = self.weight_shapes()
        if len(weights) != len(shapes):
            raise ValueError('expected %d weight arrays, got %d' % (len(shapes), len(weights)))
        p = np.zeros(self.pflat.numel(), np.float32)
        s = np.zeros(self.n_stats, np.float32)
        i = 0
        for l in self.layers:
            for key in ('k', 'b', 'gamma', 'beta'):
                if key in l.off:
                    o, shp = l.off[key]
                    w = np.asarray(weights[i], np.float32)
                    if tuple(w.shape) != tuple(shp):
                        raise ValueError('weight %d (%s.%s): shape %r != %r' % (i, l.name, key, w.shape, shp))
                    p[o:o + w.size] = w.ravel()
                    i += 1
            if l.kind != 'head':
                for key in ('mmean', 'mvar'):
                    w = np.asarray(weights[i], np.float32)
                    s[l.soff[key]:l.soff[key] + l.cout] = w.ravel()
                    i += 1
        self.pflat.copy_(torch.from_numpy(p))
        self.sflat.copy_(torch.from_numpy(s))
        self._packed_dirty = True
        self._fold_dirty = True

    def pview(self, flat, l, key):
        o, shp = l.off[key]
        return _ptr(flat, o)

    def sview(self, l, key):
        return _ptr(self.sflat, l.soff[key])

    def stat_ptr(self, l, which):
        return _ptr(self.bstat, self._stat_off[l.name] + which * l.cout)

    def _stream(self):
        return torch.cuda.current_stream(self.device).cuda_stream

    def _ev(self):
        i = self._ev_i
        self._ev_i = i + 1
        if i == len(self._evpool):
            import ctypes
            h = ctypes.c_void_p()
            rc = self.L.cdll.dc_event_create_sync(ctypes.byref(h))
            if rc != 0:
                raise DcunetError('dc_event_create_sync failed (%d): %s' % (rc, self.L.cdll.dc_last_error().decode()))
            self._evpool.append(h.value)
        return self._evpool[i]

    def _ev_fenced(self):
        i = self._evf_i
        self._evf_i = i + 1
        if i == len(self._evpool_f):
            import ctypes
            h = ctypes.c_void_p()
            rc = self.L.cdll.dc_event_create_fenced(ctypes.byref(h))
            if rc != 0:
                raise DcunetError('dc_event_create_fenced failed (%d): %s' % (rc, self.L.cdll.dc_last_error().decode()))
            self._evpool_f.append(h.value)
        return self._evpool_f[i]

    def _record(self, stream_h, fenced=False):
        ev = self._ev_fenced() if fenced else self._ev()
        self.L.dc_event_record(ev, stream_h)
        return ev

    def _wait(self, stream_h, ev):
        self.L.dc_stream_wait_event(stream_h, ev)

    def _wait_stream(self, dst_h, src_h, fenced=False):
        self._wait(dst_h, self._record(src_h, fenced))

    def _sync_bn(self):
        return self.bn_mode == 'sync' and (parallel.world_size() > 1 or parallel.exchange_active())

    def _sync_all_reduce(self, t):
        rec = getattr(self, 'sync_events', None)
        if rec is None:
            return parallel.all_reduce_sum(t)
        e0, e1 = torch.cuda.Event(enable_timing=True), torch.cuda.Event(enable_timing=True)
        e0.record()
        parallel.all_reduce_sum(t)
        e1.record()
        rec.append((e0, e1))
        return t

    _TAPE_STATE = frozenset(('range_guard', 'bnin', 'dzin', 'dzin_lvls', 'dzin_all', 'joint', 'stats_per_wg', 'tail_main',
                             'dz_writeback', 'deep_slots', 'c1_z_on_load', 'head_rank1', 'FOLD_MIN', 'bn_mode', 'streams', 'mfma', 'upsampling', 'up_drop',
                             'infer_measured', 'SLOTS', 'SLOTS_DEEP', 'SLOTS_DEEP_MAX_BYTES', '_side_stream', 'nm', 'use_tapes',
                             'ar_buckets'))

    def __setattr__(self, name, value):
        if name in UNetEngine._TAPE_STATE and '_tapes' in self.__dict__:
            old = self.__dict__.get(name, getattr(type(self), name, None))
            if old is not value and old != value:
                self.invalidate_tapes()
        object.__setattr__(self, name, value)

    def invalidate_tapes(self):
        self._tapes.clear()
        self._tape_epoch = self.__dict__.get('_tape_epoch', 0) + 1

    def _v(self, key, value):
        return Var(key, value) if self.L.recording() else value

    def _taped(self, key, body, values, post_attrs=(), on_mark=None):
        if not self.use_tapes or not hasattr(self.L, 'record_begin'):
            return body()
        ent = self._tapes.get(key)
        if ent is not None and ent['tape'] is not None:
            self.tape_replays += 1
            if self.tape_verify and self.tape_replays % self.tape_verify == 0:
                self.L.record_begin()
                try:
                    ret = body()
                finally:
                    ops = self.L.record_end()
                if not ops_equal(ent['ops'], ops):
                    raise DcunetError('launch tape %r no longer matches the sequence the engine issues (DC_TAPE_VERIFY): some state '
                                      'the recorded phase depends on changed without invalidate_tapes()' % (key[0],))
                return ret
            ent['tape'].replay(values(), on_mark)
            for a, v in ent['post'].items():
                setattr(self, a, v)
            return ent['ret']
        self.L.record_begin()
        try:
            ret = body()
        finally:
            ops = self.L.record_end()
        post = dict((a, getattr(self, a)) for a in post_attrs)
        if ent is not None and ent['post'] == post and ops_equal(ent['ops'], ops):
            ent.update(tape=Tape(self.L, ops), ret=ret)
        else:
            self._tapes[key] = dict(ops=ops, tape=None, post=post, ret=ret)
        return ret

    def buf(self, name, numel, dtype=torch.float32):
        t = self._bufs.get(name)
        if t is None or t.numel() < numel or t.dtype != dtype:
            if t is not None:
                self.invalidate_tapes()
            t = torch.empty(int(numel), dtype=dtype, device=self.device)
            self._bufs[name] = t
        return t

    @_on_device
    def repack(self):
        if not self._packed_dirty:
            return
        L, st = self.L, self._stream()
        jobs = []
        for l in self.layers:
            if l.name not in self.wp_fwd:
                continue
            src = self.pview(self.pflat, l, 'k')
            ci, co = l.cin, l.cout
            if l.kind == 'conv':
                jobs.append((src, _ptr(self.wp_fwd[l.name]), 9, ci, co, ci * co, co, 1, 0))
                jobs.append((src, _ptr(self.wp_dgrad[l.name]), 9, co, ci, ci * co, 1, co, 1))
            else:
                jobs.append((src, _ptr(self.wp_fwd[l.name]), 1, ci, 4 * co, 0, 1, ci, 0))
                jobs.append((src, _ptr(self.wp_dgrad[l.name]), 4, co, ci, co * ci, ci, 1, 0))
        if self.mfma == 'f16x3':
            if getattr(self, '_pack_jobs', None) is None:
                rows, b = [], 0
                for j in jobs:
                    total = j[2] * ((j[3] + 7) // 8) * 8 * j[4]
                    rows.append(list(j) + [b])
                    b += max(1, min((total // 8 + 1023) // 1024, 2048))
                rows.append([0] * 9 + [b])
                self._pack_jobs = (torch.tensor(rows, dtype=torch.int64, device=self.device), len(jobs), b)
            tab, n, blocks = self._pack_jobs
            L.dc_pack_weights_f16x3_batch(tab.data_ptr(), n, blocks, st)
        else:
            for j in jobs:
                L.dc_pack_weights(*(j + (st,)))
        self._packed_dirty = False

    def refold(self):
        if not self._fold_dirty:
            return
        L, st = self.L, self._stream()
        for l in self.layers:
            if l.kind == 'head':
                continue
            L.dc_bn_fold(self.pview(self.pflat, l, 'gamma'), self.pview(self.pflat, l, 'beta'),
                         self.sview(l, 'mmean'), self.sview(l, 'mvar'), self.pview(self.pflat, l, 'b'),
                         BN_EPS, self.stat_ptr(l, 2), self.stat_ptr(l, 3), l.cout, st)
        self._fold_dirty = False

    def _ab_infer(self, l):
        if self.mfma != 'f16x3' or not self.range_guard:
            return None, 0, None, 0
        if self.infer_measured:
            return self._ab_in(l, True) + self._ab_out(l, True)
        return None, 0, self._ovf.data_ptr(), -1

    def _conv_fwd(self, x, l, bias, z, z_ld, stats, sc, sh, relu, N, h, w, st, bnin=None, measured=False, splitk=None, stats_rows=0):
        if measured:
            ab_in, ab_in_ld, ab_out, ab_out_ld = self._ab_infer(l)
        else:
            ab_in, ab_in_ld, ab_out, ab_out_ld = self._ab_in(l), 0, None, 0
        if bnin is not None:
            self.L.dc_conv3x3_fwd_bnin_f16x3(x, bnin[0], bnin[1], self._ab_in(l), _ptr(self.wp_fwd[l.name]), bias, z, z_ld,
                                             stats, stats_rows, sc, sh, relu, splitk, N, h, w, l.cin, l.cout, st)
        elif self.mfma == 'f16x3':
            self.L.dc_conv3x3_fwd_f16x3(x, _ptr(self.wp_fwd[l.name]), bias, z, z_ld, stats, stats_rows, sc, sh, relu, ab_in, ab_in_ld,
                                        ab_out, ab_out_ld, splitk, N, h, w, l.cin, l.cout, st)
        else:
            self.L.dc_conv3x3_fwd(x, _ptr(self.wp_fwd[l.name]), bias, z, z_ld, stats, sc, sh, relu,
                                  N, h, w, l.cin, l.cout, st)

    def _convT_fwd(self, x, l, bias, z, z_ld, stats, sc, sh, relu, N, h, w, st, bnin=None, measured=False):
        if measured:
            ab_in, ab_in_ld, ab_out, ab_out_ld = self._ab_infer(l)
        else:
            ab_in, ab_in_ld, ab_out, ab_out_ld = self._ab_in(l), 0, None, 0
        if bnin is not None:
            self.L.dc_convT2x2_fwd_bnin_f16x3(x, bnin[0], bnin[1], self._ab_in(l), _ptr(self.wp_fwd[l.name]), bias, z, z_ld,
                                              stats, sc, sh, relu, N, h, w, l.cin, l.cout, st)
        elif self.mfma == 'f16x3':
            self.L.dc_convT2x2_fwd_f16x3(x, _ptr(self.wp_fwd[l.name]), bias, z, z_ld, stats, sc, sh, relu, ab_in, ab_in_ld,
                                         ab_out, ab_out_ld, N, h, w, l.cin, l.cout, st)
        else:
            self.L.dc_convT2x2_fwd(x, _ptr(self.wp_fwd[l.name]), bias, z, z_ld, stats, sc, sh, relu,
                                   N, h, w, l.cin, l.cout, st)

    def _ab_key(self, l, out):
        n = l.name
        if out:
            if l.kind == 'convT':
                return 'cat%d' % l.lvl, 0
            if n[0] == 'e' and n[-1] == 'b':
                return 'cat%d' % l.lvl, self._cup(l.lvl)
            return n, 0
        if l.kind == 'convT':
            return ('bb' if l.lvl == 3 else 'd%db' % (l.lvl + 1)), 0
        if n[0] == 'd' and n[-1] == 'a':
            return 'cat%d' % l.lvl, 0
# ... 112 lines not shown
            plan.append(('block', la, A['cat%d' % lvl], A['d%da' % lvl], 0, c, h, w, None))
            plan.append(('block', lb, A['d%da' % lvl], A['d%db' % lvl], 0, c, h, w, la))
            prev, prev_l = A['d%db' % lvl], lb
        return plan

    def _check_input(self, name, t, dtype, shape=None):
        shape = tuple(shape) if shape is not None else (t.shape[0], self.H, self.W)
        if not isinstance(t, torch.Tensor) or t.dtype != dtype or tuple(t.shape) != shape or not t.is_contiguous() \
                or t.device != self.device:
            raise ValueError('%s must be a contiguous %s tensor of shape %r on %s, got %s' % (
                name, dtype, shape, self.device,
                '%s %r on %s%s' % (t.dtype, tuple(t.shape), t.device, '' if t.is_contiguous() else ' (non-contiguous)')
                if isinstance(t, torch.Tensor) else type(t).__name__))

    @_on_device
    def forward_infer(self, x_dev):
        N = x_dev.shape[0]
        self._check_input('x', x_dev, torch.float32)
        A = self._acts(N)
        key = ('infer', N, self._stream(), bool(self.infer_measured), self._packed_dirty, self._fold_dirty)
        return self._taped(key, lambda: self._forward_infer_body(x_dev, N, A), lambda: {'x': _ptr(x_dev)},
                           post_attrs=('_packed_dirty', '_fold_dirty'))

    def _forward_infer_body(self, x_dev, N, A):
        L, st = self.L, self._stream()
        xp = self._v('x', _ptr(x_dev))
        self.repack()
        self.refold()
        if self.mfma == 'f16x3' and self.range_guard:
            if self.infer_measured:
                L.dc_fill(self.abound.data_ptr(), self.abound.numel(), 0.0, st)
            else:
                L.dc_fill(self._ovf.data_ptr(), self._ovf.numel(), 0.0, st)
        plan = self._plan(A)
        sk = _ptr(A['splitk_ws']) if A.get('splitk_ws') is not None else None
        pooled_by_conv = False
        for si, step in enumerate(plan):
            if step[0] == 'pool':
                if pooled_by_conv:
                    pooled_by_conv = False
                    continue
                _, lvl, src, coff, ld, h, w = step
                L.dc_maxpool2x2_fwd(_ptr(src, coff), ld, _ptr(A['pool%d' % lvl]), None, N, h, w, self.nfb << lvl, st)
                continue
            if step[0] == 'up':
                _, lvl, src, dst, ld, h, w = step
                L.dc_upsample2x_drop_fwd(_ptr(src), _ptr(dst), ld, None, 1.0, 0,
                                         *(self._ab_up(lvl, True) if self.infer_measured else (None, 0, None, 0)),
                                         N, h // 2, w // 2, self._cup(lvl), st)
                continue
            _, l, src, dst, coff, ld, h, w, _prod = step
            sc, sh = self.stat_ptr(l, 2), self.stat_ptr(l, 3)
            if l.kind == 'conv' and l.cin == 1:
                L.dc_conv3x3_c1_fwd(xp, self.pview(self.pflat, l, 'k'), None, _ptr(dst, coff), ld, None,
                                    sc, sh, 1, *self._ab_infer(l)[2:], N, h, w, l.cout, st)
            elif l.kind == 'conv':
                nxt = plan[si + 1] if si + 1 < len(plan) else None
                if (self.mfma == 'f16x3' and not (self.range_guard and self.infer_measured)
                        and nxt is not None and nxt[0] == 'pool' and nxt[2] is dst and nxt[3] == coff
                        and L.dc_conv3x3_fwd_pool_blocks(N, h, w, l.cin, l.cout) > 0):
                    flag = self._ovf.data_ptr() if self.range_guard else None
                    L.dc_conv3x3_fwd_pool_f16x3(_ptr(src), _ptr(self.wp_fwd[l.name]), None, _ptr(dst, coff), ld, sc, sh, 1, flag,
                                                _ptr(A['pool%d' % nxt[1]]), N, h, w, l.cin, l.cout, st)
                    pooled_by_conv = True
                    continue
                self._conv_fwd(_ptr(src), l, None, _ptr(dst, coff), ld, None, sc, sh, 1, N, h, w, st, measured=True, splitk=sk)
            else:
                self._convT_fwd(_ptr(src), l, None, _ptr(dst, coff), ld, None, sc, sh, 1, N, h // 2, w // 2, st, measured=True)
        lo = self.by_name['out']
        L.dc_head_fwd(_ptr(A['d0b']), self.pview(self.pflat, lo, 'k'), self.pview(self.pflat, lo, 'b'), None,
                      _ptr(A['p']), None, N * self.H * self.W, self.nfb, st)
        return A['p']

    def forward_infer_checked(self, x_dev):
        p = self.forward_infer(x_dev)
        if self.mfma == 'f16x3' and self.range_guard and not self.infer_measured and float(self._ovf[0].item()) != 0.0:
            self.infer_measured = True
            p = self.forward_infer(x_dev)
        return p

    @_on_device
    def predict_tta(self, img, augmentations, hs, ws, threshold, return_mean=False):
        K, H, W = len(augmentations), self.H, self.W
        n = H * W
        key = ('tta', K, tuple(name for name, _, _ in augmentations))
        m = self._bufs.get(key)
        if m is None:
            idx = np.arange(n, dtype=np.int32).reshape(1, H, W)
            fwd = np.stack([np.ascontiguousarray(f(idx)).reshape(-1) for _, f, _ in augmentations])
            inv = np.stack([np.ascontiguousarray(g(idx)).reshape(-1) for _, _, g in augmentations])
            if fwd.shape != (K, n) or inv.shape != (K, n):
                raise ValueError('test-time augmentations must map (N,H,W) to (N,H,W) on a square window')
            m = dict(fwd=torch.from_numpy(fwd).to(self.device), inv=torch.from_numpy(inv).to(self.device),
                     src=torch.empty(n, dtype=torch.float32, device=self.device),
                     x=torch.empty((K, H, W), dtype=torch.float32, device=self.device),
                     mask=torch.empty(n, dtype=torch.uint8, device=self.device),
                     host=_pinned('tta1_img', (H, W), torch.float32), mask_host=_pinned('tta1_mask', (n,), torch.uint8))
            self._bufs[key] = m
        L, st = self.L, self._stream()
        m['host'].numpy()[...] = img
        m['src'].copy_(m['host'].view(-1), non_blocking=True)
        L.dc_gather_maps(_ptr(m['src']), m['fwd'].data_ptr(), _ptr(m['x']), K, n, st)
        p = self.forward_infer_checked(m['x'])
        mean = torch.empty(hs * ws, dtype=torch.float32, device=self.device) if return_mean else None
        L.dc_tta_merge(_ptr(p), m['inv'].data_ptr(), K, H, W, int(hs), int(ws), float(threshold), m['mask'].data_ptr(),
                       _ptr(mean) if return_mean else None, st)
        m['mask_host'][:hs * ws].copy_(m['mask'][:hs * ws], non_blocking=True)
        torch.cuda.current_stream(self.device).synchronize()
        mask = m['mask_host'][:hs * ws].numpy().reshape(hs, ws).copy()
        return (mask, mean.cpu().numpy().reshape(hs, ws)) if return_mean else mask

    def tta_begin(self, count, augmentations):
        return _TtaJob(self, count, augmentations)

    def _train_bufs(self, N):
        key = ('train', N)
        T = self._bufs.get(key)
        if T is not None:
            return T
        L = self.L
        T = {}
        dev = self.device
        nfb = self.nfb
        ws_floats, stats_floats, part_floats = 0, 0, 0
        for l in self.layers:
            if l.kind == 'head':
                continue
            h, w = self._hw(l.lvl)
            T['z_' + l.name] = torch.empty((N, h, w, l.cout), dtype=torch.float32, device=dev)
            if l.kind == 'conv':
                tiles = L.dc_conv3x3_c1_tiles(N, h, w, l.cout) if l.cin == 1 else L.dc_conv3x3_tiles(N, h, w, l.cout)
                stats_floats = max(stats_floats, tiles * l.cout * 2)
                ws_floats = max(ws_floats, L.dc_conv3x3_wgrad_ws_floats(N, h, w, l.cin, l.cout))
            else:
                tiles = (L.dc_convT2x2_f16x3_tiles if self.mfma == 'f16x3' else L.dc_convT2x2_tiles)(N, h // 2, w // 2, l.cout)
                stats_floats = max(stats_floats, tiles * 4 * l.cout * 2)
                ws_floats = max(ws_floats, L.dc_convT2x2_wgrad_ws_floats(N, h // 2, w // 2, l.cin, l.cout))
            blocks = L.dc_bn_bwd_blocks(N * h * w, l.cout)
            part_floats = max(part_floats, blocks * l.cout * 2)
        hb = L.dc_head_blocks(N * self.H * self.W)
        part_floats = max(part_floats, hb * (nfb + 4), hb * 12, hb * nfb * 2)
        for l in self.layers:
            if l.kind == 'conv' and l.cin > 1:
                h, w = self._hw(l.lvl)
                part_floats = max(part_floats, L.dc_conv3x3_dgrad_bnred_blocks(N, h, w, l.cin, l.cout) * l.cin * 2)
        for lvl in range(4):
            h, w = self._hw(lvl)
            part_floats = max(part_floats, L.dc_maxpool2x2_bwd_blocks(N, h, w, nfb << lvl) * (nfb << lvl) * 2)
        for l in self.layers:
            if l.kind == 'conv':
                part_floats = max(part_floats, L.dc_conv3x3_bwd_joint_blocks(N, *self._hw(l.lvl), l.cin, l.cout) * l.cin * 2)
            elif l.kind == 'convT':
                h, w = self._hw(l.lvl)
                part_floats = max(part_floats, L.dc_convT2x2_dgrad_bnred_blocks(N, h // 2, w // 2, l.cin, l.cout) * l.cin * 2)
        sk = 4
        for l in self.layers:
            if l.kind == 'conv' and l.cin > 1 and self.mfma == 'f16x3':
                h, w = self._hw(l.lvl)
                sk = max(sk, L.dc_conv3x3_splitk_ws_floats(N, h, w, l.cin, l.cout, 0), L.dc_conv3x3_splitk_ws_floats(N, h, w, l.cin, l.cout, 1))
            elif l.kind == 'convT' and self.mfma == 'f16x3':
                h, w = self._hw(l.lvl)
                sk = max(sk, L.dc_convT2x2_dgrad_splitk_ws_floats(N, h // 2, w // 2, l.cin, l.cout))
        T['splitk_ws'] = torch.empty(sk, dtype=torch.float32, device=dev)
        T['stats_ws'] = torch.empty(stats_floats, dtype=torch.float64, device=dev)
        T['stats_fold'] = torch.empty(self.FOLD_ROWS * 4 * max(l.cout for l in self.layers) * 2, dtype=torch.float64, device=dev)
        T['part_ws'] = torch.empty(part_floats, dtype=torch.float32, device=dev)
        T['part_ws2'] = torch.empty(part_floats, dtype=torch.float32, device=dev)
        T['amax_ws'] = torch.empty(part_floats // 2 + 4, dtype=torch.float32, device=dev)
        T['amax_ws2'] = torch.empty(part_floats // 2 + 4, dtype=torch.float32, device=dev)
        T['head_gpart'] = torch.empty(hb * (nfb + 4), dtype=torch.float32, device=dev)
        T['head_s'] = torch.empty(N * self.H * self.W, dtype=torch.float32, device=dev)
        big = N * self.H * self.W * nfb
        S = self.SLOTS_DEEP if (self.deep_slots and 2 * self.SLOTS_DEEP * big * 4 <= self.SLOTS_DEEP_MAX_BYTES) else self.SLOTS
        T['slots'] = S
        T['absmax'] = [torch.empty(4096, dtype=torch.float32, device=dev) for _ in range(S)]
        dpart = max(L.dc_bn_bwd_blocks(N * self._hw(l.lvl)[0] * self._hw(l.lvl)[1], l.cout) * l.cout
                    for l in self.layers if l.kind != 'head')
        T['dbias_part'] = [torch.empty(dpart, dtype=torch.float32, device=dev) for _ in range(S)]
        T['dz_scale'] = torch.ones(S * 4, dtype=torch.float32, device=dev)
        cmax = max(l.cout for l in self.layers if l.kind != 'head')
        T['dz_coef'] = [torch.zeros(7 * cmax, dtype=torch.float32, device=dev) for _ in range(S)]
        T['red_tmp'] = torch.empty(32 * 1024, dtype=torch.float32, device=dev)
        T['wgrad_ws'] = torch.empty(ws_floats, dtype=torch.float32, device=dev)
        l0 = self.layers[0]
        T['wgrad_ws_main'] = torch.empty(max(L.dc_conv3x3_wgrad_ws_floats(N, self.H, self.W, l0.cin, l0.cout), 4), dtype=torch.float32,
                                         device=dev)
        jws = max([L.dc_conv3x3_bwd_joint_ws_floats(N, *self._hw(l.lvl), l.cin, l.cout) for l in self.layers if l.kind == 'conv'] + [4])
        T['joint_ws'] = torch.empty(jws, dtype=torch.float32, device=dev)
        T['sums'] = torch.zeros(12, dtype=torch.float64, device=dev)
        T['bn_sums'] = torch.zeros(2 * max(l.cout for l in self.layers if l.kind != 'head'), dtype=torch.float64, device=dev)
        T['bn_gsum'] = torch.zeros(2 * max(l.cout for l in self.layers if l.kind != 'head'), dtype=torch.float32, device=dev)
        big = N * self.H * self.W * nfb
        T['dz'] = [torch.empty(big, dtype=torch.float32, device=dev) for _ in range(S)]
        T['g'] = [torch.empty(big, dtype=torch.float32, device=dev) for _ in range(S)]
        for lvl in range(4):
            h, w = self._hw(lvl)
            T['dcat%d' % lvl] = torch.empty(N * h * w * (self._cup(lvl) + (nfb << lvl)), dtype=torch.float32, device=dev)
        self._bufs[key] = T
        return T

    def set_crop_sources(self, S_list, M_list):
        from .model import crop_layout
        shapes = [tuple(np.shape(v)) for v in S_list]
        if [tuple(np.shape(v)) for v in M_list] != shapes or any(len(sh) != 2 for sh in shapes):
            raise ValueError('summaries and masks must be 2-D arrays of equal shapes per dataset')
        offs, total = crop_layout(shapes)
        S, M = np.zeros(total, np.float32), np.zeros(total, np.uint8)
        for o, (h, w), sv, mv in zip(offs, shapes, S_list, M_list):
            S[o:o + h * w] = np.asarray(sv, dtype=np.float32).ravel()
            M[o:o + h * w] = np.asarray(mv).astype(np.uint8).ravel()
        self._crop = dict(S=torch.from_numpy(S).to(self.device), M=torch.from_numpy(M).to(self.device), total=total)

    @_on_device
    def crop_batch(self, items):
        src = getattr(self, '_crop', None)
        if src is None:
            raise RuntimeError('set_crop_sources() first')
        if self.H != self.W:
            raise ValueError('device-side batches need a square window')
        items = np.ascontiguousarray(items, dtype=np.int64)
        n = int(items.shape[0])
        key = ('xy_in', n)
        xy = self._bufs.get(key)
        if xy is None:
            xy = self._bufs[key] = (torch.empty((n, self.H, self.W), dtype=torch.float32, device=self.device),
                                    torch.empty((n, self.H, self.W), dtype=torch.uint8, device=self.device))
        self._settle_tail()
        self.L.dc_crop_augment(src['S'].data_ptr(), src['M'].data_ptr(), src['total'], items.ctypes.data, n, self.H,
                               xy[0].data_ptr(), xy[1].data_ptr(), self._stream())
        return xy

    def _drop_args(self, l, masks, step_seed):
        if l.drop <= 0.0:
            return None, 1.0, 0
        keep = 1.0 - l.drop
        if masks is not None:
            m = masks[l.name]
            assert m.dtype == torch.uint8 and m.is_contiguous()
            return m.data_ptr(), keep, 0
        h, w = self._hw(l.lvl)
        seed = (step_seed * 1000003 + l.index * 7919) & 0xFFFFFFFFFFFFFFFF
        return None, keep, self._v(('seed', l.name), parallel.shard_drop_seed(seed, self._last[0] * h * w * l.cout))

    def _up_drop_args(self, lvl, masks, step_seed):
        rate = self.up_drop[lvl]
        if rate <= 0.0:
            return None, 1.0, 0
        if masks is not None:
            m = masks['u%d' % lvl]
            assert m.dtype == torch.uint8 and m.is_contiguous()
            return m.data_ptr(), 1.0 - rate, 0
        h, w = self._hw(lvl)
        seed = (step_seed * 1000003 + (100 + lvl) * 7919) & 0xFFFFFFFFFFFFFFFF
        return None, 1.0 - rate, self._v(('useed', lvl), parallel.shard_drop_seed(seed, self._last[0] * h * w * self._cup(lvl)))

    @_on_device
    def forward_train(self, x_dev, y_dev, masks=None, update_moving=True):
        N = x_dev.shape[0]
        self._check_input('x', x_dev, torch.float32)
        self._check_input('y', y_dev, torch.uint8, (N, self.H, self.W))
        if masks is not None:
            for l in self.layers:
                if l.drop > 0.0:
                    h, w = self._hw(l.lvl)
                    self._check_input('masks[%r]' % l.name, masks.get(l.name), torch.uint8, (N, h, w, l.cout))
            if self.upsampling:
                for lvl, rate in self.up_drop.items():
                    if rate > 0.0:
                        h, w = self._hw(lvl)
                        self._check_input("masks['u%d']" % lvl, masks.get('u%d' % lvl), torch.uint8, (N, h, w, self._cup(lvl)))
        self._settle_tail()
        self._acts(N), self._train_bufs(N)
        step_seed = self.drop_seed + self.iterations
        self._last = (N, masks, step_seed, x_dev, y_dev)
        world = parallel.world_size()
        sync = self._sync_bn()

        def body():
            return self._forward_train_body(x_dev, y_dev, masks, update_moving)
        if masks is not None or sync:
            return body()
        key = ('fwd', N, bool(update_moving), self.loss_kind, self._stream(), self._packed_dirty, world, parallel.rank())
        return self._taped(key, body, lambda: self._step_values(x_dev, y_dev, step_seed),
                           post_attrs=('_packed_dirty', '_fold_dirty', '_head_bwd_done'))

    def _step_values(self, x_dev, y_dev, step_seed):
        vals = {'x': _ptr(x_dev), 'y': y_dev.data_ptr()}
        for l in self.layers:
            if l.drop > 0.0:
                vals[('seed', l.name)] = self._drop_args(l, None, step_seed)[2]
        if self.upsampling:
            for lvl, rate in self.up_drop.items():
                if rate > 0.0:
                    vals[('useed', lvl)] = self._up_drop_args(lvl, None, step_seed)[2]
        return vals

    def _forward_train_body(self, x_dev, y_dev, masks, update_moving):
        N = x_dev.shape[0]
        L, st = self.L, self._stream()
        self.repack()
        A, T = self._acts(N), self._train_bufs(N)
        step_seed = self._last[2]
        world = parallel.world_size()
        sync = self._sync_bn()
        xp, yp = self._v('x', _ptr(x_dev)), self._v('y', y_dev.data_ptr())
        plan = self._plan(A)
        pooled_with_block = False
        for si, step in enumerate(plan):
            if step[0] == 'pool':
                if pooled_with_block:
                    pooled_with_block = False
                    continue
                _, lvl, src, coff, ld, h, w = step
                L.dc_maxpool2x2_fwd(_ptr(src, coff), ld, _ptr(A['pool%d' % lvl]), A['idx%d' % lvl].data_ptr(),
                                    N, h, w, self.nfb << lvl, st)
                continue
            if step[0] == 'up':
                _, lvl, src, dst, ld, h, w = step
                mptr, keep, seed = self._up_drop_args(lvl, masks, step_seed)
                L.dc_upsample2x_drop_fwd(_ptr(src), _ptr(dst), ld, mptr, keep, seed, *self._ab_up(lvl), N, h // 2, w // 2,
                                         self._cup(lvl), st)
                continue
            _, l, src, dst, coff, ld, h, w, prod = step
            z = T['z_' + l.name]
            bias = self.pview(self.pflat, l, 'b')
            stats = T['stats_ws'].data_ptr()
            groups = 1
            bsrc = self._bnin_src(prod, T)
            xin, bn = (bsrc[0], bsrc[1]) if bsrc is not None else (_ptr(src) if src is not None else None, None)
            if l.kind == 'conv' and l.cin == 1:
                tiles = L.dc_conv3x3_c1_tiles(N, h, w, l.cout)
                L.dc_conv3x3_c1_fwd(xp, self.pview(self.pflat, l, 'k'), bias, _ptr(z), l.cout, stats,
                                    None, None, 0, None, 0, N, h, w, l.cout, st)
            elif l.kind == 'conv':
                tiles = (L.dc_conv3x3_stats_rows(N, h, w, l.cin, l.cout) if self.mfma == 'f16x3' and self.stats_per_wg
                         else L.dc_conv3x3_tiles(N, h, w, l.cout))
                self._conv_fwd(xin, l, bias, _ptr(z), l.cout, stats, None, None, 0, N, h, w, st, bnin=bn, splitk=_ptr(T['splitk_ws']),
                               stats_rows=tiles)
            else:
                tiles = (L.dc_convT2x2_f16x3_tiles if self.mfma == 'f16x3' else L.dc_convT2x2_tiles)(N, h // 2, w // 2, l.cout)
                groups = 4
                self._convT_fwd(xin, l, bias, _ptr(z), l.cout, stats, None, None, 0, N, h // 2, w // 2, st, bnin=bn)
            pixels = N * h * w
            mom = l.mom if update_moving else -1.0
            if self.FOLD_MIN > 0 and tiles * groups >= self.FOLD_MIN and tiles >= 2:
                fold, chunks = T['stats_fold'].data_ptr(), min(self.FOLD_ROWS, tiles // 2)
                L.dc_bn_stats_rows_fold(stats, tiles, groups, l.cout, chunks, fold, st)
                stats, tiles = fold, chunks
            if sync:
                bs = T['bn_sums'][:2 * l.cout]
                L.dc_bn_stats_reduce(stats, tiles, groups, l.cout, bs.data_ptr(), st)
                self._sync_all_reduce(bs)
                nm_l = l.name in self.nm
                L.dc_bn_stats_finalize_sums(bs.data_ptr(), l.cout, float(world * pixels), BN_EPS, mom,
                                            self.stat_ptr(l, 0), self.stat_ptr(l, 1), self.sview(l, 'mmean'),
                                            self.sview(l, 'mvar'), self.pview(self.pflat, l, 'gamma'),
                                            self.pview(self.pflat, l, 'beta'), self.stat_ptr(l, 4) if nm_l else None,
                                            self.stat_ptr(l, 5) if nm_l else None, self._ab_out(l) if nm_l else None, st)
                if nm_l:
                    continue
            elif l.name in self.nm:
                L.dc_bn_stats_finalize_affine(stats, tiles, groups, l.cout, float(pixels), BN_EPS, mom,
                                              self.stat_ptr(l, 0), self.stat_ptr(l, 1), self.sview(l, 'mmean'),
                                              self.sview(l, 'mvar'), self.pview(self.pflat, l, 'gamma'),
                                              self.pview(self.pflat, l, 'beta'), self.stat_ptr(l, 4),
                                              self.stat_ptr(l, 5), self._ab_out(l), st)
                continue
            if not sync:
                L.dc_bn_stats_finalize(stats, tiles, groups, l.cout, float(pixels), BN_EPS, mom,
                                       self.stat_ptr(l, 0), self.stat_ptr(l, 1), self.sview(l, 'mmean'),
                                       self.sview(l, 'mvar'), st)
            mptr, keep, seed = self._drop_args(l, masks, step_seed)
            nxt = plan[si + 1] if si + 1 < len(plan) else None
            if nxt is not None and nxt[0] == 'pool' and nxt[2] is dst and nxt[3] == coff:
                lvl = nxt[1]
                L.dc_bn_relu_drop_pool_fwd(_ptr(z), self.stat_ptr(l, 0), self.stat_ptr(l, 1),
                                           self.pview(self.pflat, l, 'gamma'), self.pview(self.pflat, l, 'beta'),
                                           mptr, keep, seed, _ptr(dst, coff), ld, _ptr(A['pool%d' % lvl]),
                                           A['idx%d' % lvl].data_ptr(), N, h, w, l.cout,
                                           float((world if sync else 1) * pixels), self._ab_out(l), st)
                pooled_with_block = True
                continue
            L.dc_bn_relu_drop_fwd(_ptr(z), self.stat_ptr(l, 0), self.stat_ptr(l, 1),
                                  self.pview(self.pflat, l, 'gamma'), self.pview(self.pflat, l, 'beta'),
                                  mptr, keep, seed, _ptr(dst, coff), ld, pixels, l.cout,
                                  float((world if sync else 1) * pixels), self._ab_out(l), st)
        if update_moving:
            self._fold_dirty = True
        lo = self.by_name['out']
        pixels = N * self.H * self.W
        hb = L.dc_head_blocks(pixels)
        hsrc = self._bnin_src(self.by_name['d0b'], T)
        self._head_bwd_done = False
        if self.loss_kind in (0, 1):
            a_in, sc_in, sh_in = (hsrc[0], hsrc[1][0], hsrc[1][1]) if hsrc is not None else (_ptr(A['d0b']), None, None)
            ld0 = self.by_name['d0b']
            red = hsrc is not None
            s_mode = self._head_s_ok(N)
            head = L.dc_head_fwd_bwd_s if s_mode else L.dc_head_fwd_bwd
            head(a_in, sc_in, sh_in, self.pview(self.pflat, lo, 'k'), self.pview(self.pflat, lo, 'b'),
                 yp, _ptr(A['p']), _ptr(T['part_ws']), _ptr(T['head_s'] if s_mode else T['g'][0]), _ptr(T['head_gpart']),
                 self.loss_kind, self.stat_ptr(ld0, 0) if red else None, self.stat_ptr(ld0, 1) if red else None,
                 _ptr(T['part_ws2']) if red else None, _ptr(T['amax_ws2']) if red else None, pixels, self.nfb, st)
            self._head_bwd_done = 's' if s_mode else True
        elif hsrc is not None:
            L.dc_head_fwd_bnin(hsrc[0], hsrc[1][0], hsrc[1][1], self.pview(self.pflat, lo, 'k'),
                               self.pview(self.pflat, lo, 'b'), yp, _ptr(A['p']), _ptr(T['part_ws']),
                               pixels, self.nfb, st)
        else:
            L.dc_head_fwd(_ptr(A['d0b']), self.pview(self.pflat, lo, 'k'), self.pview(self.pflat, lo, 'b'),
                          yp, _ptr(A['p']), _ptr(T['part_ws']), pixels, self.nfb, st)
        L.dc_reduce_partials_f64(_ptr(T['part_ws']), hb, 12, T['sums'].data_ptr(), st)
        return A['p']

    def grad_buckets(self):
        o_ba, o_dec = self.by_name['ba'].off['k'][0], self.layers[10].off['k'][0]
        return [(o_dec, self.n_train), (o_ba, o_dec), (0, o_ba)]

    def _head_s_ok(self, N):
        l = self.by_name['d0b']
        if not (self.head_rank1 and self.joint and self.mfma == 'f16x3' and l.cin == 32 and l.cout == 32):
            return False
        if l.name not in self.nm:
            return False
        if self._dzin_ok(l, N) != 1:
            return False
        h, w = self._hw(l.lvl)
        return self.L.dc_conv3x3_bwd_joint_blocks(N, h, w, l.cin, l.cout) > 0

    def _dzin_ok(self, l, N):
        if not self.dzin or l.kind != 'conv' or l.drop > 0.0:
            return 0
        h, w = self._hw(l.lvl)
        if not self.dzin_all and N * self.H * self.W <= (1 << 20):
            return 0
        if l.lvl in self.dzin_lvls:
            if l.cin == 1:
                return 1
            return 1 if self.L.dc_conv3x3_dgrad_dzin_blocks(N, h, w, l.cin, l.cout) > 0 else 0
        if self.dz_writeback and l.cin > 32 and self.L.dc_conv3x3_dgrad_dzin_blocks(N, h, w, l.cin, l.cout) > 0:
            return 2
        return 0

    @_on_device
    def backward(self, bucket_cb=None, defer_tail=False, comm=None):
        N, masks, step_seed, x_dev, y_dev = self._last
        self._settle_tail()
        if getattr(self, '_side_stream', None) is None:
            self._side_stream = torch.cuda.Stream(device=self.device)
        side = self._side_stream if self.streams == 2 else torch.cuda.current_stream(self.device)
        world = parallel.world_size()
        sync = self._sync_bn()

        if comm is not None:
            if bucket_cb is not None:
                raise ValueError('backward: pass bucket_cb (the caller issues the collectives) OR comm (dc_comm_* from here), not both')

        def body():
            return self._backward_body(bucket_cb, defer_tail, comm)

        def on_mark(i):
            with torch.cuda.stream(side):
                bucket_cb(*self.grad_buckets()[i])
        if masks is not None or sync:
            return body()
        key = ('bwd', N, self.loss_kind, self._stream(), side.cuda_stream, self._head_bwd_done, bool(defer_tail),
               bucket_cb is not None, world, parallel.rank(), comm, self.ar_buckets)
        return self._taped(key, body, lambda: self._step_values(x_dev, y_dev, step_seed),
                           post_attrs=('_tail', '_head_bwd_done', '_ev_i', '_evf_i'), on_mark=on_mark)

    def _backward_body(self, bucket_cb, defer_tail, comm=None):
        N, masks, step_seed, x_dev, y_dev = self._last
        L, st = self.L, self._stream()
        A, T = self._acts(N), self._train_bufs(N)
        self._ev_i = 0
        self._evf_i = 0
        self._tail = None
        xp, yp = self._v('x', _ptr(x_dev)), self._v('y', y_dev.data_ptr())
        nfb = self.nfb
        f16 = self.mfma == 'f16x3'
        pixels0 = N * self.H * self.W
        lo = self.by_name['out']
        hb = L.dc_head_blocks(pixels0)
        hsrc = self._bnin_src(self.by_name['d0b'], T)
        gb = T['g']
        fused_d0b = None
        gpart = T['part_ws']
        head_s = None
        if self._head_bwd_done:
            if self._head_bwd_done == 's':
                head_s = (_ptr(T['head_s']), self.pview(self.pflat, lo, 'k'))
            self._head_bwd_done = False
            gpart = T['head_gpart']
            if hsrc is not None:
                fused_d0b = (_ptr(T['part_ws2']), _ptr(T['amax_ws2']), hb)
        elif hsrc is not None:
            ld0 = self.by_name['d0b']
            if self._head_s_ok(N):
                head_s = (_ptr(T['head_s']), self.pview(self.pflat, lo, 'k'))
            head = L.dc_head_bwd_bnin_bnred_s if head_s else L.dc_head_bwd_bnin_bnred
            head(hsrc[0], hsrc[1][0], hsrc[1][1], _ptr(A['p']), yp,
                 self.pview(self.pflat, lo, 'k'), head_s[0] if head_s else _ptr(gb[0]), _ptr(T['part_ws']), self.loss_kind,
                 T['sums'].data_ptr(), self.stat_ptr(ld0, 0), self.stat_ptr(ld0, 1),
                 _ptr(T['part_ws2']), _ptr(T['amax_ws2']), pixels0, nfb, st)
            fused_d0b = (_ptr(T['part_ws2']), _ptr(T['amax_ws2']), hb)
        else:
            L.dc_head_bwd(_ptr(A['d0b']), _ptr(A['p']), yp, self.pview(self.pflat, lo, 'k'),
                          _ptr(gb[0]), _ptr(T['part_ws']), self.loss_kind, T['sums'].data_ptr(), pixels0, nfb, st)
        L.dc_head_grad_finalize(_ptr(gpart), hb, nfb, self.pview(self.gflat, lo, 'k'),
                                self.pview(self.gflat, lo, 'b'), st)

        main = torch.cuda.current_stream(self.device)
        side = self._side_stream if self.streams == 2 else main
        two = two_streams = side is not main
        mh, sh_ = main.cuda_stream, side.cuda_stream
        if two:
            self._wait_stream(sh_, mh)
        S = T['slots']
        slot_free = [None] * S
        g_free = [None] * S
        state = {'slot': 0, 'g': 0}
        world = parallel.world_size()
        sync = self._sync_bn()

        def g_cur():
            return gb[state['g']]

        def g_next():
            k = (state['g'] + 1) % S
            if two and g_free[k] is not None:
                self._wait(mh, g_free[k])
                g_free[k] = None
            return k

        def red_of(la):
            return la if la.drop <= 0.0 else None

        def block_bwd(l, x_in, da_ptr, da_ld, dx_ptr, prod=None, fused=None, red=None, da_g=None, on_main=False, r1=None):
            two = two_streams and not on_main
            bsrc = self._bnin_src(prod, T)
            h, w = self._hw(l.lvl)
            pixels = N * h * w
            z = T['z_' + l.name]
            mptr, keep, seed = self._drop_args(l, masks, step_seed)
            mean, invstd = self.stat_ptr(l, 0), self.stat_ptr(l, 1)
            gamma, beta = self.pview(self.pflat, l, 'gamma'), self.pview(self.pflat, l, 'beta')
            dgamma, dbeta = self.pview(self.gflat, l, 'gamma'), self.pview(self.gflat, l, 'beta')
            dk, ws = self.pview(self.gflat, l, 'k'), _ptr(T['wgrad_ws_main' if on_main else 'wgrad_ws'])
            dz_mode = self._dzin_ok(l, N) if da_ld == l.cout else 0
            if dz_mode == 2 and dx_ptr is None:
                dz_mode = 0
            dzin = dz_mode > 0
            k = state['slot']
            state['slot'] = (k + 1) % S
            if fused is None:
                L.dc_bn_bwd_reduce(da_ptr, da_ld, _ptr(z), mean, invstd, gamma, beta, mptr, keep, seed,
                                   _ptr(T['part_ws']), _ptr(T['amax_ws']) if dzin else None, pixels, l.cout, st)
                fused = (_ptr(T['part_ws']), _ptr(T['amax_ws']), L.dc_bn_bwd_blocks(pixels, l.cout))
            if two_streams and slot_free[k] is not None:
                self._wait(mh, slot_free[k])
                slot_free[k] = None
            count = float((world if sync else 1) * pixels)
            gg = None
            if sync:
                L.dc_bn_bwd_finalize(fused[0], fused[2], l.cout, dgamma, dbeta, st)
                g0, _ = l.off['gamma']
                gg = T['bn_gsum'][:2 * l.cout]
                gg.copy_(self.gflat[g0:g0 + 2 * l.cout])
                self._sync_all_reduce(gg)

            if dzin:
                coef = _ptr(T['dz_coef'][k])
                if gg is not None:
                    L.dc_bn_bwd_finalize_dzin(None, fused[1], fused[2], l.cout, mean, invstd, gamma, beta, count,
                                              _ptr(gg), _ptr(gg, l.cout), coef, self.pview(self.gflat, l, 'b'), st)
                else:
                    L.dc_bn_bwd_finalize_dzin(fused[0], fused[1], fused[2], l.cout, mean, invstd, gamma, beta, count,
                                              dgamma, dbeta, coef, self.pview(self.gflat, l, 'b'), st)
                fused_next = None
                xa = (bsrc[0], bsrc[1][0], bsrc[1][1]) if bsrc is not None else (x_in, None, None)
                jrows = L.dc_conv3x3_bwd_joint_blocks(N, h, w, l.cin, l.cout) if (dx_ptr is not None and self.joint) else 0
                if jrows > 0 and l.cin != l.cout and (bsrc is not None or red is not None):
                    jrows = 0
                if jrows > 0:
                    rargs = (None,) * 7
                    if red is not None:
                        rargs = (_ptr(T['z_' + red.name]), self.stat_ptr(red, 0), self.stat_ptr(red, 1),
                                 self.pview(self.pflat, red, 'gamma'), self.pview(self.pflat, red, 'beta'),
                                 _ptr(T['part_ws']), _ptr(T['amax_ws']))
                        fused_next = (_ptr(T['part_ws']), _ptr(T['amax_ws']), jrows)
                    if r1 is not None:
                        L.dc_conv3x3_bwd_joint_r1_f16x3(xa[0], xa[1], xa[2], self._ab_in(l), r1[0], r1[1], _ptr(z), coef,
                                                        _ptr(self.wp_dgrad[l.name]), dx_ptr, *rargs, dk, _ptr(T['joint_ws']),
                                                        N, h, w, l.cin, l.cout, st)
                    else:
                        L.dc_conv3x3_bwd_joint_f16x3(xa[0], xa[1], xa[2], self._ab_in(l), da_ptr, _ptr(z), coef,
                                                     _ptr(self.wp_dgrad[l.name]), dx_ptr, *rargs, dk, _ptr(T['joint_ws']),
                                                     N, h, w, l.cin, l.cout, st)
                    return fused_next
                if r1 is not None:
                    raise DcunetError('block %s: the head wrote its rank-one gradient factors but the joint kernel does not serve '
                                      'the block (_head_s_ok and block_bwd disagree)' % l.name)
                if dx_ptr is not None:
                    rargs = (None,) * 7
                    if red is not None:
                        rows = L.dc_conv3x3_dgrad_dzin_blocks(N, h, w, l.cin, l.cout)
                        rargs = (_ptr(T['z_' + red.name]), self.stat_ptr(red, 0), self.stat_ptr(red, 1),
                                 self.pview(self.pflat, red, 'gamma'), self.pview(self.pflat, red, 'beta'),
                                 _ptr(T['part_ws']), _ptr(T['amax_ws']))
                        fused_next = (_ptr(T['part_ws']), _ptr(T['amax_ws']), rows)
                    L.dc_conv3x3_dgrad_dzin_f16x3(da_ptr, _ptr(z), coef, _ptr(self.wp_dgrad[l.name]), dx_ptr,
                                                  _ptr(T['dz'][k]) if dz_mode == 2 else None, *rargs, N, h, w, l.cin, l.cout, st)
                if two:
                    self._wait_stream(sh_, mh)
                sw = st if on_main else sh_
                if dz_mode == 2:
                    dzp, scale = _ptr(T['dz'][k]), _ptr(T['dz_scale'], 4 * k)
                    L.dc_pow2_scale_from_absmax(coef + 4 * 6 * l.cout, l.cout, 1024.0, scale, sw)
                    if bsrc is not None:
                        L.dc_conv3x3_wgrad_bnin_f16x3(bsrc[0], bsrc[1][0], bsrc[1][1], self._ab_in(l), dzp, dk, ws, scale, N, h, w,
                                                      l.cin, l.cout, sw)
                    else:
                        L.dc_conv3x3_wgrad_f16x3(x_in, dzp, dk, ws, scale, self._ab_in(l), N, h, w, l.cin, l.cout, sw)
                elif l.cin == 1 and self.c1_z_on_load and w % 4 == 0 and x_dev.data_ptr() % 16 == 0:
                    L.dc_conv3x3_c1_wgrad_dzin_zre(xa[0], self.pview(self.pflat, l, 'k'), self.pview(self.pflat, l, 'b'), da_ptr,
                                                   coef, dk, ws, N, h, w, l.cout, sw)
                else:
                    L.dc_conv3x3_wgrad_dzin_f16x3(xa[0], xa[1], xa[2], self._ab_in(l), da_ptr, _ptr(z), coef, dk, ws,
                                                  N, h, w, l.cin, l.cout, sw)
                if two:
                    ev = self._record(sh_)
                    slot_free[k] = ev
                    if da_g is not None:
                        g_free[da_g] = ev
                return fused_next

            if r1 is not None:
                raise DcunetError('block %s: the head wrote its rank-one gradient factors but the block takes the apply pass '
                                  '(_head_s_ok and block_bwd disagree)' % l.name)
            dz, scale = _ptr(T['dz'][k]), _ptr(T['dz_scale'], 4 * k)
            dpart, amaxp = _ptr(T['dbias_part'][k]), _ptr(T['absmax'][k])
            blocks = L.dc_bn_bwd_blocks(pixels, l.cout)
            if gg is not None:
                L.dc_bn_bwd_apply_count(da_ptr, da_ld, _ptr(z), mean, invstd, gamma, beta, mptr, keep, seed,
                                        _ptr(gg), _ptr(gg, l.cout), dz, dpart, amaxp, pixels, count, l.cout, st)
            else:
                L.dc_bn_bwd_finalize(fused[0], fused[2], l.cout, dgamma, dbeta, st)
                L.dc_bn_bwd_apply(da_ptr, da_ld, _ptr(z), mean, invstd, gamma, beta, mptr, keep, seed, dgamma, dbeta,
                                  dz, dpart, amaxp, pixels, l.cout, st)

            def finalize(stream):
                L.dc_bn_bwd_apply_finalize(dpart, amaxp if f16 else None, blocks, l.cout, 1024.0,
                                           self.pview(self.gflat, l, 'b'), scale if f16 else None, stream)
            side_fin = f16 and N * self.H * self.W <= (1 << 20)
            if not side_fin:
                finalize(st)
            d_scale, d_amax, d_amax_n = (None, amaxp, blocks) if side_fin else (scale, None, 0)

            def dgrad():
                if l.kind == 'conv':
                    if f16 and red is not None:
                        rows = L.dc_conv3x3_dgrad_bnred_blocks(N, h, w, l.cin, l.cout)
                        if rows > 0:
                            L.dc_conv3x3_dgrad_bnred_f16x3(dz, wpd, dx_ptr, d_scale, d_amax, d_amax_n, _ptr(T['z_' + red.name]),
                                                           self.stat_ptr(red, 0), self.stat_ptr(red, 1),
                                                           self.pview(self.pflat, red, 'gamma'), self.pview(self.pflat, red, 'beta'),
                                                           _ptr(T['part_ws']), _ptr(T['amax_ws']), N, h, w, l.cin, l.cout, st)
                            return (_ptr(T['part_ws']), _ptr(T['amax_ws']), rows)
                    if f16:
                        L.dc_conv3x3_dgrad_f16x3(dz, wpd, dx_ptr, d_scale, d_amax, d_amax_n, _ptr(T['splitk_ws']), N, h, w, l.cin, l.cout, st)
                    else:
                        L.dc_conv3x3_dgrad(dz, wpd, dx_ptr, N, h, w, l.cin, l.cout, st)
                elif f16:
                    rows = L.dc_convT2x2_dgrad_bnred_blocks(N, h // 2, w // 2, l.cin, l.cout) if red is not None else 0
                    if rows > 0:
                        L.dc_convT2x2_dgrad_bnred_f16x3(dz, wpd, dx_ptr, d_scale, d_amax, d_amax_n, _ptr(T['z_' + red.name]),
                                                        self.stat_ptr(red, 0), self.stat_ptr(red, 1),
                                                        self.pview(self.pflat, red, 'gamma'), self.pview(self.pflat, red, 'beta'),
                                                        _ptr(T['part_ws']), _ptr(T['amax_ws']), N, h // 2, w // 2, l.cin, l.cout, st)
                        return (_ptr(T['part_ws']), _ptr(T['amax_ws']), rows)
                    L.dc_convT2x2_dgrad_f16x3(dz, wpd, dx_ptr, d_scale, d_amax, d_amax_n, _ptr(T['splitk_ws']), N, h // 2, w // 2, l.cin, l.cout, st)
                else:
                    L.dc_convT2x2_dgrad(dz, wpd, dx_ptr, N, h // 2, w // 2, l.cin, l.cout, st)
                return None

            fused_next = None
            wpd = _ptr(self.wp_dgrad[l.name]) if dx_ptr is not None else None
            after = dx_ptr is not None and f16 and l.kind == 'conv' and L.dc_conv3x3_pp_blocks(N, h, w, l.cin, l.cout, 1, 0) > 0
            if after:
                fused_next = dgrad()
            if two:
                self._wait_stream(sh_, mh)
            sw = st if on_main else sh_
            if side_fin:
                finalize(sw)
            if bsrc is not None and l.kind == 'conv':
                L.dc_conv3x3_wgrad_bnin_f16x3(bsrc[0], bsrc[1][0], bsrc[1][1], self._ab_in(l), dz, dk, ws, scale, N, h, w,
                                              l.cin, l.cout, sw)
            elif bsrc is not None:
                L.dc_convT2x2_wgrad_bnin_f16x3(bsrc[0], bsrc[1][0], bsrc[1][1], self._ab_in(l), dz, dk, ws, scale, N,
                                               h // 2, w // 2, l.cin, l.cout, sw)
            elif l.kind == 'conv':
                if f16:
                    L.dc_conv3x3_wgrad_f16x3(x_in, dz, dk, ws, scale, self._ab_in(l), N, h, w, l.cin, l.cout, sw)
                else:
                    L.dc_conv3x3_wgrad(x_in, dz, dk, ws, N, h, w, l.cin, l.cout, sw)
            elif f16:
                L.dc_convT2x2_wgrad_f16x3(x_in, dz, dk, ws, scale, self._ab_in(l), N, h // 2, w // 2, l.cin, l.cout, sw)
            else:
                L.dc_convT2x2_wgrad(x_in, dz, dk, ws, N, h // 2, w // 2, l.cin, l.cout, sw)
            if two:
                slot_free[k] = self._record(sh_)
            if dx_ptr is not None and not after:
                fused_next = dgrad()
            return fused_next

        fused_up = None
        for lvl in (0, 1, 2, 3):
            c = nfb << lvl
            cat, dcat = A['cat%d' % lvl], T['dcat%d' % lvl]
            la = self.by_name['d%da' % lvl]
            ki, ko = state['g'], g_next()
            fa = block_bwd(self.by_name['d%db' % lvl], _ptr(A['d%da' % lvl]), _ptr(gb[ki]), c, _ptr(gb[ko]),
                           prod=la, fused=fused_d0b if lvl == 0 else fused_up, red=red_of(la), da_g=ki,
                           r1=head_s if lvl == 0 else None)
            state['g'] = ko
            block_bwd(la, _ptr(cat), _ptr(gb[ko]), c, _ptr(dcat), fused=fa, da_g=ko)
            x_up = A['bb'] if lvl == 3 else A['d%db' % (lvl + 1)]
            l_up = self.by_name['bb' if lvl == 3 else 'd%db' % (lvl + 1)]
            kn = g_next()
            if self.upsampling:
                h, w = self._hw(lvl)
                mptr, keep, seed = self._up_drop_args(lvl, masks, step_seed)
                L.dc_upsample2x_drop_bwd(_ptr(dcat), 3 * c, mptr, keep, seed, _ptr(gb[kn]), N, h // 2, w // 2, 2 * c, st)
                fused_up = None
            else:
                fused_up = block_bwd(self.by_name['u%d' % lvl], _ptr(x_up), _ptr(dcat), 2 * c, _ptr(gb[kn]), prod=l_up,
                                     red=red_of(l_up))
            state['g'] = kn

        def bucket_done(i):
            if comm is not None:
                if self.ar_buckets > 1:
                    if two:
                        self._wait_stream(sh_, mh, fenced=True)
                    lo, hi = self.grad_buckets()[i]
                    L.dc_comm_all_reduce_sum(comm, _ptr(self.gflat, lo), hi - lo, sh_)
                return
            if bucket_cb is None:
                return
            if two:
                self._wait_stream(sh_, mh, fenced=True)
            L.mark(i)
            with torch.cuda.stream(side):
                bucket_cb(*self.grad_buckets()[i])

        bucket_done(0)
        for lvl in (4, 3, 2, 1, 0):
            c = nfb << lvl
            h, w = self._hw(lvl)
            tag = 'b' if lvl == 4 else 'e%d' % lvl
            if lvl == 3:
                bucket_done(1)
            fused_pool = fused_up if lvl == 4 else None
            if lvl < 4:
                cup = self._cup(lvl)
                lb = self.by_name[tag + 'b']
                ki, ko = state['g'], g_next()
                mptr, keep, seed = self._drop_args(lb, masks, step_seed)
                L.dc_maxpool2x2_bwd_bnred(_ptr(gb[ki]), A['idx%d' % lvl].data_ptr(), _ptr(T['dcat%d' % lvl], cup), cup + c,
                                          _ptr(gb[ko]), _ptr(T['z_' + lb.name]), self.stat_ptr(lb, 0),
                                          self.stat_ptr(lb, 1), self.pview(self.pflat, lb, 'gamma'),
                                          self.pview(self.pflat, lb, 'beta'), mptr, keep, seed,
                                          _ptr(T['part_ws2']), _ptr(T['amax_ws2']), N, h, w, c, st)
                fused_pool = (_ptr(T['part_ws2']), _ptr(T['amax_ws2']), L.dc_maxpool2x2_bwd_blocks(N, h, w, c))
                state['g'] = ko
            la = self.by_name[tag + 'a']
            ki, ko = state['g'], g_next()
            fa = block_bwd(self.by_name[tag + 'b'], _ptr(A[tag + 'a']), _ptr(gb[ki]), c, _ptr(gb[ko]), prod=la,
                           fused=fused_pool, red=red_of(la), da_g=ki)
            state['g'] = ko
            if lvl == 0:
                tail_main = two and self.tail_main and bucket_cb is None
                if two and defer_tail and bucket_cb is None and not tail_main:
                    self._tail = self._record(sh_)
                block_bwd(la, xp, _ptr(gb[ko]), c, None, fused=fa, da_g=ko, on_main=tail_main)
            else:
                kn = g_next()
                block_bwd(la, _ptr(A['pool%d' % (lvl - 1)]), _ptr(gb[ko]), c, _ptr(gb[kn]), fused=fa, da_g=ko)
# ... 92 lines not shown
```

### include/dcunet.h

```cpp
#ifndef DCUNET_H
#define DCUNET_H
#include <stdint.h>
#ifdef __cplusplus
extern "C" {
#endif

typedef void* dc_stream_t;

#define DC_ABI_VERSION 130
int dc_version(void);
const char* dc_last_error(void);

int dc_pack_weights(const float* src, float* dst, int taps, int K, int Ncols,
                    long s_tap, long s_k, long s_n, int flip, dc_stream_t stream);

int dc_conv3x3_tiles(int N, int H, int W, int Cout);
int dc_conv3x3_fwd(const float* x, const float* wp, const float* bias, float* z, long z_ld, double* stats,
                   const float* scale, const float* shift, int relu,
                   int N, int H, int W, int Cin, int Cout, dc_stream_t stream);
int dc_conv3x3_c1_tiles(int N, int H, int W, int Cout);
int dc_conv3x3_c1_fwd(const float* x, const float* w, const float* bias, float* z, long z_ld, double* stats,
                      const float* scale, const float* shift, int relu, float* out_absmax, long out_absmax_ld,
                      int N, int H, int W, int Cout, dc_stream_t stream);
int dc_conv3x3_dgrad(const float* dz, const float* wp, float* dx,
                     int N, int H, int W, int Cin, int Cout, dc_stream_t stream);
long dc_conv3x3_wgrad_ws_floats(int N, int H, int W, int Cin, int Cout);
int dc_conv3x3_wgrad(const float* x, const float* dz, float* dw, float* ws,
                     int N, int H, int W, int Cin, int Cout, dc_stream_t stream);

#define DC_ABOUND_SLOTS 8
long dc_pack_weights_f16x3_floats(int taps, int K, int Ncols);
int dc_pack_weights_f16x3(const float* src, void* dst, int taps, int K, int Ncols,
                          long s_tap, long s_k, long s_n, int flip, dc_stream_t stream);
int dc_pack_weights_f16x3_batch(const long* jobs_dev, int njobs, int total_blocks, dc_stream_t stream);
long dc_conv3x3_splitk_ws_floats(int N, int H, int W, int Cin, int Cout, int dgrad);
long dc_convT2x2_dgrad_splitk_ws_floats(int N, int H, int W, int Cin, int Cout);
int dc_conv3x3_stats_rows(int N, int H, int W, int Cin, int Cout);
int dc_conv3x3_fwd_f16x3(const float* x, const void* wp16, const float* bias, float* z, long z_ld, double* stats, int stats_rows,
                         const float* scale, const float* shift, int relu, const float* in_abound, long in_abound_ld,
                         float* out_absmax, long out_absmax_ld, float* splitk_ws, int N, int H, int W, int Cin, int Cout,
                         dc_stream_t stream);
int dc_conv3x3_dgrad_f16x3(const float* dz, const void* wp16, float* dx, const float* dz_scale,
                           const float* dz_absmax, int dz_absmax_n, float* splitk_ws,
                           int N, int H, int W, int Cin, int Cout, dc_stream_t stream);
int dc_convT2x2_fwd_f16x3(const float* x, const void* wp16, const float* bias, float* z, long z_ld, double* stats,
                          const float* scale, const float* shift, int relu, const float* in_abound, long in_abound_ld,
                          float* out_absmax, long out_absmax_ld, int N, int H, int W, int Cin, int Cout, dc_stream_t stream);
int dc_convT2x2_dgrad_f16x3(const float* dz, const void* wp16, float* dx, const float* dz_scale,
                            const float* dz_absmax, int dz_absmax_n, float* splitk_ws,
                            int N, int H, int W, int Cin, int Cout, dc_stream_t stream);
int dc_convT2x2_f16x3_tiles(int N, int H, int W, int Cout);
int dc_conv3x3_wgrad_f16x3(const float* x, const float* dz, float* dw, float* ws, const float* dz_scale,
                           const float* x_abound, int N, int H, int W, int Cin, int Cout, dc_stream_t stream);
int dc_convT2x2_wgrad_f16x3(const float* x, const float* dz, float* dw, float* ws, const float* dz_scale,
                            const float* x_abound, int N, int H, int W, int Cin, int Cout, dc_stream_t stream);

int dc_bn_stats_finalize_affine(const double* partial, int parts, int groups, int C, double count, float eps,
                                float momentum, float* mean, float* invstd, float* moving_mean, float* moving_var,
                                const float* gamma, const float* beta, float* scale, float* shift, float* abound,
                                dc_stream_t stream);
int dc_conv3x3_fwd_bnin_f16x3(const float* z_in, const float* in_scale, const float* in_shift, const float* in_abound,
                              const void* wp16, const float* bias, float* z, long z_ld, double* stats, int stats_rows, const float* scale,
                              const float* shift, int relu, float* splitk_ws, int N, int H, int W, int Cin, int Cout,
                              dc_stream_t stream);
int dc_convT2x2_fwd_bnin_f16x3(const float* z_in, const float* in_scale, const float* in_shift, const float* in_abound,
                               const void* wp16, const float* bias, float* z, long z_ld, double* stats, const float* scale,
                               const float* shift, int relu, int N, int H, int W, int Cin, int Cout, dc_stream_t stream);
int dc_conv3x3_wgrad_bnin_f16x3(const float* z_in, const float* in_scale, const float* in_shift, const float* in_abound,
                                const float* dz, float* dw, float* ws, const float* dz_scale, int N, int H, int W,
                                int Cin, int Cout, dc_stream_t stream);
int dc_convT2x2_wgrad_bnin_f16x3(const float* z_in, const float* in_scale, const float* in_shift, const float* in_abound,
                                 const float* dz, float* dw, float* ws, const float* dz_scale, int N, int H, int W,
                                 int Cin, int Cout, dc_stream_t stream);
int dc_head_fwd_bnin(const float* z_in, const float* in_scale, const float* in_shift, const float* kh, const float* bh,
                     const uint8_t* y, float* p, float* partial, long pixels, int C, dc_stream_t stream);
int dc_head_bwd_bnin(const float* z_in, const float* in_scale, const float* in_shift, const float* p, const uint8_t* y,
                     const float* kh, float* da, float* partial, int loss_kind, const double* sums, long pixels, int C,
                     dc_stream_t stream);


int dc_convT2x2_tiles(int N, int H, int W, int Cout);
int dc_convT2x2_fwd(const float* x, const float* wp, const float* bias, float* z, long z_ld, double* stats,
                    const float* scale, const float* shift, int relu,
                    int N, int H, int W, int Cin, int Cout, dc_stream_t stream);
int dc_convT2x2_dgrad(const float* dz, const float* wp, float* dx,
                      int N, int H, int W, int Cin, int Cout, dc_stream_t stream);
long dc_convT2x2_wgrad_ws_floats(int N, int H, int W, int Cin, int Cout);
int dc_convT2x2_wgrad(const float* x, const float* dz, float* dw, float* ws,
                      int N, int H, int W, int Cin, int Cout, dc_stream_t stream);

int dc_bn_stats_finalize(const double* partial, int parts, int groups, int C, double count, float eps,
                         float momentum, float* mean, float* invstd, float* moving_mean, float* moving_var,
                         dc_stream_t stream);
int dc_bn_fold(const float* gamma, const float* beta, const float* mmean, const float* mvar, const float* bias,
               float eps, float* scale, float* shift, int C, dc_stream_t stream);
int dc_bn_relu_drop_fwd(const float* z, const float* mean, const float* invstd, const float* gamma,
                        const float* beta, const uint8_t* mask, float keep, uint64_t seed,
                        float* out, long out_ld, long pixels, int C, double count, float* abound, dc_stream_t stream);
int dc_bn_relu_drop_pool_fwd(const float* z, const float* mean, const float* invstd, const float* gamma,
                             const float* beta, const uint8_t* mask, float keep, uint64_t seed, float* out, long out_ld,
                             float* pooled, uint8_t* idx, int N, int H, int W, int C, double count, float* abound,
                             dc_stream_t stream);
int dc_bn_bwd_blocks(long pixels, int C);
int dc_bn_bwd_reduce(const float* da, long da_ld, const float* z, const float* mean, const float* invstd,
                     const float* gamma, const float* beta, const uint8_t* mask, float keep, uint64_t seed,
                     float* partial, float* amax_partial, long pixels, int C, dc_stream_t stream);
int dc_bn_bwd_apply(const float* da, long da_ld, const float* z, const float* mean, const float* invstd,
                    const float* gamma, const float* beta, const uint8_t* mask, float keep, uint64_t seed,
                    const float* dgamma, const float* dbeta, float* dz, float* dbias_partial, float* absmax_partial,
                    long pixels, int C, dc_stream_t stream);
int dc_pow2_scale_from_absmax(const float* partial, int n, float target, float* scale, dc_stream_t stream);
int dc_bn_bwd_apply_finalize(const float* dbias_partial, const float* absmax_partial, int blocks, int C, float target,
                             float* dbias, float* scale, dc_stream_t stream);

int dc_conv3x3_fwd_pool_blocks(int N, int H, int W, int Cin, int Cout);
int dc_conv3x3_fwd_pool_f16x3(const float* x, const void* wp16, const float* bias, float* z, long z_ld,
                              const float* scale, const float* shift, int relu, float* out_flag, float* pool,
                              int N, int H, int W, int Cin, int Cout, dc_stream_t stream);

int dc_conv3x3_pp_blocks(int N, int H, int W, int Cin, int Cout, int dgrad, int with_stats);
int dc_conv3x3_dgrad_bnred_blocks(int N, int H, int W, int Cin, int Cout);
int dc_conv3x3_dgrad_bnred_f16x3(const float* dz, const void* wp16, float* dx, const float* dz_scale,
                                 const float* dz_absmax, int dz_absmax_n, const float* z,
                                 const float* mean, const float* invstd, const float* gamma, const float* beta,
                                 float* bn_partial, float* amax_partial, int N, int H, int W, int Cin, int Cout,
                                 dc_stream_t stream);
int dc_head_bwd_bnin_bnred(const float* z_in, const float* in_scale, const float* in_shift, const float* p,
                           const uint8_t* y, const float* kh, float* da, float* partial, int loss_kind,
                           const double* sums, const float* bn_mean, const float* bn_invstd, float* bn_partial,
                           float* amax_partial, long pixels, int C, dc_stream_t stream);
int dc_convT2x2_dgrad_bnred_blocks(int N, int H, int W, int Cin, int Cout);
int dc_convT2x2_dgrad_bnred_f16x3(const float* dz, const void* wp16, float* dx, const float* dz_scale,
                                  const float* dz_absmax, int dz_absmax_n, const float* z,
                                  const float* mean, const float* invstd, const float* gamma, const float* beta,
                                  float* bn_partial, float* amax_partial, int N, int H, int W, int Cin, int Cout,
                                  dc_stream_t stream);
int dc_maxpool2x2_bwd_blocks(int N, int H, int W, int C);
int dc_maxpool2x2_bwd_bnred(const float* dy, const uint8_t* idx, const float* skip, long skip_ld, float* dx,
                            const float* z, const float* mean, const float* invstd, const float* gamma,
                            const float* beta, const uint8_t* mask, float keep, uint64_t seed, float* bn_partial,
                            float* amax_partial, int N, int H, int W, int C, dc_stream_t stream);

#define DC_DZ_COEF_ROWS 7
int dc_bn_bwd_finalize_dzin(const float* partial, const float* amax_partial, int P, int C, const float* mean,
                            const float* invstd, const float* gamma, const float* beta, double count,
                            float* dgamma, float* dbeta, float* dz_coef, float* dbias, dc_stream_t stream);
int dc_conv3x3_dgrad_dzin_blocks(int N, int H, int W, int Cin, int Cout);
int dc_conv3x3_dgrad_dzin_f16x3(const float* da, const float* z, const float* dz_coef, const void* wp16, float* dx, float* dz_out,
                                const float* red_z, const float* red_mean, const float* red_invstd,
                                const float* red_gamma, const float* red_beta, float* bn_partial, float* amax_partial,
                                int N, int H, int W, int Cin, int Cout, dc_stream_t stream);
int dc_conv3x3_wgrad_dzin_f16x3(const float* x, const float* in_scale, const float* in_shift, const float* x_abound,
                                const float* da, const float* z, const float* dz_coef, float* dw, float* ws,
                                int N, int H, int W, int Cin, int Cout, dc_stream_t stream);
int dc_conv3x3_c1_wgrad_dzin_zre(const float* x, const float* w, const float* bias, const float* da, const float* dz_coef,
                                 float* dw, float* ws, int N, int H, int W, int Cout, dc_stream_t stream);

int dc_conv3x3_bwd_joint_blocks(int N, int H, int W, int Cin, int Cout);
long dc_conv3x3_bwd_joint_ws_floats(int N, int H, int W, int Cin, int Cout);
int dc_conv3x3_bwd_joint_f16x3(const float* x, const float* in_scale, const float* in_shift, const float* x_abound,
                               const float* da, const float* z, const float* dz_coef, const void* wp16, float* dx,
                               const float* red_z, const float* red_mean, const float* red_invstd, const float* red_gamma,
                               const float* red_beta, float* bn_partial, float* amax_partial, float* dw, float* ws,
                               int N, int H, int W, int Cin, int Cout, dc_stream_t stream);
int dc_conv3x3_bwd_joint_r1_f16x3(const float* x, const float* in_scale, const float* in_shift, const float* x_abound,
                                  const float* s, const float* kh, const float* z, const float* dz_coef, const void* wp16,
                                  float* dx, const float* red_z, const float* red_mean, const float* red_invstd,
                                  const float* red_gamma, const float* red_beta, float* bn_partial, float* amax_partial,
                                  float* dw, float* ws, int N, int H, int W, int Cin, int Cout, dc_stream_t stream);

int dc_bn_stats_reduce(const double* partial, int parts, int groups, int C, double* sums, dc_stream_t stream);
int dc_bn_stats_rows_fold(const double* partial, int parts, int groups, int C, int chunks, double* out, dc_stream_t stream);
int dc_bn_stats_finalize_sums(const double* sums, int C, double count, float eps, float momentum, float* mean,
                              float* invstd, float* moving_mean, float* moving_var, const float* gamma,
                              const float* beta, float* scale, float* shift, float* abound, dc_stream_t stream);
int dc_bn_bwd_apply_count(const float* da, long da_ld, const float* z, const float* mean, const float* invstd,
                          const float* gamma, const float* beta, const uint8_t* mask, float keep, uint64_t seed,
                          const float* dgamma, const float* dbeta, float* dz, float* dbias_partial,
                          float* absmax_partial, long pixels, double count, int C, dc_stream_t stream);

int dc_maxpool2x2_fwd(const float* in, long in_ld, float* out, uint8_t* idx,
                      int N, int H, int W, int C, dc_stream_t stream);
int dc_maxpool2x2_bwd(const float* dy, const uint8_t* idx, const float* skip, long skip_ld, float* dx,
                      int N, int H, int W, int C, dc_stream_t stream);

int dc_upsample2x_drop_fwd(const float* in, float* out, long out_ld, const uint8_t* mask, float keep, uint64_t seed,
                           const float* abound_in, long abound_in_ld, float* abound_out, long abound_out_ld,
                           int N, int H, int W, int C, dc_stream_t stream);
int dc_upsample2x_drop_bwd(const float* dout, long dout_ld, const uint8_t* mask, float keep, uint64_t seed, float* din,
                           int N, int H, int W, int C, dc_stream_t stream);

int dc_head_blocks(long pixels);
int dc_head_fwd(const float* a, const float* kh, const float* bh, const uint8_t* y, float* p, float* partial,
                long pixels, int C, dc_stream_t stream);
int dc_head_bwd(const float* a, const float* p, const uint8_t* y, const float* kh, float* da, float* partial,
                int loss_kind, const double* sums, long pixels, int C, dc_stream_t stream);
int dc_head_fwd_bwd(const float* a, const float* in_scale, const float* in_shift, const float* kh, const float* bh,
                    const uint8_t* y, float* p, float* partial, float* da, float* grad_partial, int loss_kind,
                    const float* bn_mean, const float* bn_invstd, float* bn_partial, float* amax_partial, long pixels,
                    int C, dc_stream_t stream);
int dc_head_fwd_bwd_s(const float* a, const float* in_scale, const float* in_shift, const float* kh, const float* bh,
                      const uint8_t* y, float* p, float* partial, float* s, float* grad_partial, int loss_kind,
                      const float* bn_mean, const float* bn_invstd, float* bn_partial, float* amax_partial, long pixels,
                      int C, dc_stream_t stream);
int dc_head_bwd_bnin_bnred_s(const float* z_in, const float* in_scale, const float* in_shift, const float* p,
                             const uint8_t* y, const float* kh, float* s, float* partial, int loss_kind,
                             const double* sums, const float* bn_mean, const float* bn_invstd, float* bn_partial,
                             float* amax_partial, long pixels, int C, dc_stream_t stream);
int dc_head_grad_finalize(const float* partial, int blocks, int C, float* dkh, float* dbh, dc_stream_t stream);

int dc_reduce_partials(const float* in, int P, long L, float scale, float* out, float* tmp, dc_stream_t stream);
int dc_reduce_partials_f64(const float* in, int P, int L, double* out, dc_stream_t stream);
int dc_bn_bwd_finalize(const float* partial, int P, int C, float* dgamma, float* dbeta, dc_stream_t stream);

int dc_adam_step_flat(float* p, const float* g, float* m, float* v, long n, float lr_t, float b1, float b2,
                      float eps, float gscale, dc_stream_t stream);

int dc_gather_maps(const float* in, const int* maps, float* out, int K, long n, dc_stream_t stream);
int dc_tta_merge(const float* preds, const int* invmaps, int K, int H, int W, int hs, int ws, double threshold,
                 uint8_t* mask, float* mean_out, dc_stream_t stream);

#define DC_CROP_MAX_ITEMS 64
int dc_crop_augment(const float* S, const uint8_t* M, long src_elems, const long* items_host, int B, int hw,
                    float* x, uint8_t* y, dc_stream_t stream);
int dc_round_window_u8(const float* p, int N, int H, int W, int y0, int y1, int x0, int x1, uint8_t* out,
                       dc_stream_t stream);

long dc_host_nf_ws_bytes(int H, int W);
int dc_host_nf_pairs(const uint8_t* truth, const uint8_t* pred, int H, int W, double threshold, int* counts,
                     double* inc, double* exc, int cap, void* ws);
int dc_host_label8(const uint8_t* mask, int H, int W, int* labels, int* n, void* ws);

#define DC_SERIES_MAX_FRAMES 2147483647L
int dc_series_accumulate(const void* frames, int is_unsigned, int tc, long t0, long n_total, uint16_t* mean16,
                         int16_t* max16, long* sum, long* sumsq, int* vmax, int H, int W, dc_stream_t stream);
int dc_series_accumulate_xy(const void* frames, int is_unsigned, int tc, long t0, long* xy, int H, int W,
                            dc_stream_t stream);
int dc_series_finalize(const long* sum, const long* sumsq, const long* xy, float* mean, float* sdev, float* corr,
                       int H, int W, long T, dc_stream_t stream);
long dc_series_standardize_ws_floats(int H, int W);
int dc_image_standardize(const float* in, float* out, float* ws, int H, int W, dc_stream_t stream);
#define DC_SERIES_MAX_BIN_FRAMES 64
int dc_series_bin_time(const void* frames, int is_unsigned, int tc, int H, int W, int b, int phase, int* carry, void* out,
                       dc_stream_t stream);

#define DC_ROI_TRACE_MAX_VOLUME 70368744177664L
int dc_roi_trace_accumulate(const void* frames, int is_unsigned, int tc, long t0, const int* row_off, const int* row_pix,
                            const int* row_roi, int S, int R, long* sums, long ld, int H, int W, dc_stream_t stream);
int dc_roi_trace_finalize(const long* sums, long ld, const int* areas, int R, long T, float* mean, float* zscore,
                          dc_stream_t stream);

int dc_roi_wtrace_accumulate(const void* frames, int is_unsigned, int tc, long t0, const int* row_off, const int* row_pix,
                             const unsigned short* row_wgt, const int* row_roi, int S, int R, long* sums, long ld, int H, int W,
                             dc_stream_t stream);

#define DC_ROI_PIXEL_MAX_FRAMES 2147483647L
int dc_roi_pixel_accumulate(const void* frames, int is_unsigned, int tc, long t0, const int* row_off, const int* row_pix,
                            const int* row_roi, int S, int R, const long* sums, long ld, long* mom, int N, int H, int W,
                            dc_stream_t stream);
int dc_roi_trace_moments(const long* sums, long ld, int R, long T, long* rmom, dc_stream_t stream);
int dc_roi_pixel_corr(const long* mom, int N, const int* row_off, const int* row_roi, int S, int R, const int* inside,
                      const long* rmom, long T, float* corr, dc_stream_t stream);

#define DC_ROI_PAIR_TILE 64
#define DC_ROI_PAIR_BATCH 32
#define DC_ROI_PAIR_MAX_AREA 1024
#define DC_ROI_PAIR_MAX_STATE 134217728L
int dc_roi_pair_accumulate(const void* frames, int is_unsigned, int tc, const int* roi_off, const int* roi_pix, const long* goff,
                           const int* tiles, long ntiles, int R, long* a, long* g, int P, long G, int H, int W, dc_stream_t stream);
int dc_roi_pair_corr(const long* a, const long* g, const int* roi_off, const long* goff, int R, int P, long G, long T, float* corr,
                     dc_stream_t stream);

#define DC_DETREND_MAX_FRAMES 4096
int dc_series_fold_segment(const long* sum, const long* sumsq, const long* xy, const int* vmax, long len, long mult, long* pooled_var,
                           long* pooled_cov, long* sum_total, int* vmax_total, int H, int W, dc_stream_t stream);
int dc_series_finalize_pooled(const long* pooled_var, const long* pooled_cov, const long* sum_total, float* mean, float* sdev, float* corr,
                              int H, int W, long M, long T, dc_stream_t stream);
int dc_roi_pair_fold_segment(long* a, long* g, const int* roi_off, const long* goff, const int* tiles, long ntiles, int R, int P, long G,
                             long len, long mult, long* pooled, dc_stream_t stream);
int dc_roi_pair_corr_pooled(const long* pooled, const int* roi_off, const long* goff, int R, int P, long G, float* corr, dc_stream_t stream);
int dc_roi_pixel_fold_segment(long* mom, int N, const int* row_off, const int* row_roi, int S, int R, const long* rmom, long len, long mult,
                              long* pooled_xx, long* pooled_xs, long* pooled_ss, int H, int W, dc_stream_t stream);
int dc_roi_pixel_corr_pooled(const long* pooled_xx, const long* pooled_xs, const long* pooled_ss, int N, const int* row_off,
                             const int* row_roi, int S, int R, const int* inside, float* corr, dc_stream_t stream);

#define DC_TRACE_PAIR_MAX_PAIRS 16777216L
int dc_trace_pair_moments(const long* sums, long ld, int R, long T, int seg_len, const int* pairs, long P, long* num, dc_stream_t stream);
int dc_trace_pair_corr(const long* num, long P, float* corr, dc_stream_t stream);

#define DC_FRAME_MAX_PIXELS 268435456L
int dc_frame_moments(const void* frames, int is_unsigned, int tc, const void* tmpl, int H, int W, int y0, int y1, int x0, int x1,
                     long* moments, dc_stream_t stream);
int dc_frame_quality(const long* moments, int tc, long n, long ta, long tb, float* mean, float* corr, dc_stream_t stream);
int dc_frame_gather(const void* frames, int tc, const int* idx, int k, int H, int W, void* out, dc_stream_t stream);

#define DC_TRACE_BASELINE_MAX_HALF 2047
int dc_trace_combine(const long* sums, long ld, const int* np_row, const long* ca, const long* cb, const long* cc, int R, long T,
                     long* num, dc_stream_t stream);
int dc_trace_baseline(const long* num, long ld, int R, long T, int half, int q, long* base, float* dff, dc_stream_t stream);
int dc_trace_scale(const long* x, long ld, const long* den, int R, long T, float* out, dc_stream_t stream);

#define DC_TRACE_DECONV_SEARCH_SMIN 0
#define DC_TRACE_DECONV_SEARCH_LAM 1
#define DC_TRACE_DECONV_SEARCH_MAX_ROUNDS 64
#define DC_TRACE_DECONV_SEARCH_MAX_GROUPS 8192
#define DC_TRACE_DECONV_MAX_FRAMES 16777216L
#define DC_TRACE_DECONV_MAX_SAMPLES 2147483648L
long dc_trace_deconv_ws_bytes(int R, long T);
int dc_trace_deconv_ar1(const void* y, int is_f64, long ld, int R, long T, double g, const double* G, const double* lam,
                        const double* smin, void* ws, double* calcium, double* spikes, int* pools, dc_stream_t stream);
int dc_trace_deconv_ar1_host(const void* y, int is_f64, long ld, int R, long T, const double* G, const double* lam, const double* smin,
                             double* calcium, double* spikes, int* pools);
long dc_trace_deconv_search_state_bytes(int R);
int dc_trace_deconv_ar1_constrained(const void* y, int is_f64, long ld, int R, long T, double g, const double* gs, const double* G, long ldG,
                                    int which, const double* sigma, const double* fixed_other, int rounds, void* ws, void* state,
                                    double* calcium, double* spikes, int* pools, double* param, double* rss, int* status,
                                    dc_stream_t stream);
int dc_trace_deconv_search_step(const void* y, int is_f64, long ld, int R, long T, const double* G, long ldG, const void* ws,
                                const int* pools, int last, void* state, double* param, double* rss, int* status, dc_stream_t stream);
int dc_trace_deconv_ar1_constrained_host(const void* y, int is_f64, long ld, int R, long T, const double* G, int which, const double* sigma,
                                         const double* fixed_other, int rounds, double* calcium, double* spikes, int* pools, double* param,
                                         double* rss, int* status);
// ... 147 lines not shown
```

Measured before the change: 900.0 images/s.

## Add joint convT2x2 backward kernel fusing dz-on-load, dgrad, wgrad and BN reduce

Adds a warp-specialized HIP kernel for the transposed 2x2 conv backward. Producer waves load da/z, apply the BN-backward dz coefficients and dropout on load, and stage f16x3-split operands in double-buffered LDS. Some consumer waves compute dgrad with the next layer's BN reduction, while others compute wgrad slabs. The net routes convT layers to it when dzin is enabled, replacing separate apply, dgrad and wgrad passes and the dz round trip through memory. The cost is a complex kernel with large LDS use, one block per CU, and new workspace sizing.

```diff
diff --git a/deep_calcium_amd/_build.py b/deep_calcium_amd/_build.py
--- a/deep_calcium_amd/_build.py
+++ b/deep_calcium_amd/_build.py
@@ -7,7 +7,7 @@
 CSRC = os.path.join(HERE, 'csrc')
 LIBDIR = os.path.join(HERE, 'lib')
 LIB = os.path.join(LIBDIR, 'libdcunet.so')
-SOURCES = ['common.cpp', 'comm.cpp', 'nf_score.cpp', 'tape.cpp', 'igemm_conv.hip', 'igemm_f16x3.hip', 'igemm_pp.hip', 'wgrad.hip', 'wgrad_f16x3.hip', 'bwd_joint.hip', 'conv_c1.hip', 'elementwise.hip', 'series.hip', 'traces.hip', 'footprints.hip', 'roi_pairs.hip', 'trace_pairs.hip', 'frame_quality.hip', 'dff.hip', 'deconv.hip', 'trace_dyn.hip', 'spikes.hip', 'spikes_train.hip', 'motion.hip']
+SOURCES = ['common.cpp', 'comm.cpp', 'nf_score.cpp', 'tape.cpp', 'igemm_conv.hip', 'igemm_f16x3.hip', 'igemm_pp.hip', 'wgrad.hip', 'wgrad_f16x3.hip', 'bwd_joint.hip', 'convT_joint.hip', 'conv_c1.hip', 'elementwise.hip', 'series.hip', 'traces.hip', 'footprints.hip', 'roi_pairs.hip', 'trace_pairs.hip', 'frame_quality.hip', 'dff.hip', 'deconv.hip', 'trace_dyn.hip', 'spikes.hip', 'spikes_train.hip', 'motion.hip']
 FLAGS = ['--offload-arch=gfx950', '-O3', '-std=c++17', '-fPIC', '-Wall', '-Wno-unused-function']
 FILE_FLAGS = {'nf_score.cpp': ['-ffp-contract=off'], 'series.hip': ['-ffp-contract=off'], 'traces.hip': ['-ffp-contract=off'],
               'footprints.hip': ['-ffp-contract=off'], 'roi_pairs.hip': ['-ffp-contract=off'], 'trace_pairs.hip': ['-ffp-contract=off'],
diff --git a/deep_calcium_amd/csrc/convT_joint.hip b/deep_calcium_amd/csrc/convT_joint.hip
--- /dev/null
+++ b/deep_calcium_amd/csrc/convT_joint.hip
@@ -0,0 +1,421 @@
+#include "f16x3_common.h"
+
+struct UpJointParams {
+  const float* x; const float* xSc; const float* xSh; const float* xAbound;
+  const float* da; long daLd; const float* z; const float* dzCoef;
+  const uint8_t* mask; float keep; uint64_t seed;
+  const float* wp;
+  float* dx;
+  const float* redZ; const float* redMean; const float* redInvstd; const float* redGamma; const float* redBeta;
+  float* bnPartial; float* bnAmax;
+  float* slabs;
+  int N, H, W, tilesX, tilesY;
+};
+
+__device__ __forceinline__ float dc_dz_on_load_drop(float z, float da, float f, float sc, float sh, float mu, float A, float D, float E) {
+  return dc_dz_on_load(z, __fmul_rn(da, f), sc, sh, mu, A, D, E);
+}
+
+namespace uj {
+constexpr int CI = 64, CO = 32;
+constexpr int TH = 2, TW = 32, NPX = TH * TW;
+__device__ __forceinline__ int swz64(int rel) { return rel ^ ((rel >> 4) & 0x30); }
+__device__ __forceinline__ int swz128(int rel) { return rel ^ ((rel >> 2) & 0x40); }
+constexpr int TAP_STRIDE = NPX * 64 + 128;
+constexpr int DZ_PLANE = 4 * TAP_STRIDE, X_PLANE = NPX * 128;
+constexpr int OFF_DZ_LO = DZ_PLANE, OFF_X_HI = 2 * DZ_PLANE, OFF_X_LO = OFF_X_HI + X_PLANE, OFF_RAW = OFF_X_LO + X_PLANE;
+constexpr int STAGE = OFF_RAW + NPX * CI * 4;
+constexpr int LDS_BYTES = 2 * STAGE + 64;
+constexpr int THREADS = 512;
+constexpr int NLZ = 4 * NPX * (CO / 4) / 256, NLX = NPX * (CI / 4) / 256;
+constexpr int W_SLOTS = 4 * (CO / 8) * 2 * CI;
+constexpr long SLAB = 4L * CO * CI;
+constexpr unsigned OOB = 0x80000000u;
+constexpr unsigned PIX_OOB = 1u << 22;
+static_assert(LDS_BYTES <= 160 * 1024 && NLZ == 8 && NLX == 4 && TAP_STRIDE % 128 == 0, "LDS plan");
+
+struct Tile { int img, y0, x0; };
+__device__ __forceinline__ Tile decode(const UpJointParams& p, const DcXcdRange& tiles, int j) {
+  const int work = tiles.work(j);
+  const int ty = work % p.tilesY, t2 = work / p.tilesY;
+  Tile t;
+  t.x0 = (t2 % p.tilesX) * TW; t.img = t2 / p.tilesX; t.y0 = ty * TH;
+  return t;
+}
+
+struct XSet { f32x4 r[NLX]; unsigned live; };
+
+template <class RX, class RD, class SX, class SD>
+__device__ __forceinline__ void produce(char* smem, int nt, XSet& x0, XSet& x1, RX request_x, RD request_dz, SX stage_x, SD stage_dz) {
+  if (nt > 0) {
+    request_x(0, x0);
+    request_dz(0);
+    if (nt > 1) request_x(1, x1);
+    stage_x(x0, smem);
+    stage_dz(smem);
+    if (nt > 1) request_dz(1);
+  }
+  __syncthreads();
+  for (int i = 0; i < nt; i += 2) {
+    if (i + 2 < nt) request_x(i + 2, x0);
+    if (i + 1 < nt) { stage_x(x1, smem + STAGE); stage_dz(smem + STAGE); }
+    if (i + 2 < nt) request_dz(i + 2);
+    __syncthreads();
+    if (i + 1 < nt) {
+      if (i + 3 < nt) request_x(i + 3, x1);
+      if (i + 2 < nt) { stage_x(x0, smem); stage_dz(smem); }
+      if (i + 3 < nt) request_dz(i + 3);
+      __syncthreads();
+    }
+  }
+}
+}
+
+__global__ __launch_bounds__(uj::THREADS, 1) void convT_bwd_joint_kernel(UpJointParams p) {
+  using namespace uj;
+  extern __shared__ __attribute__((aligned(1024))) char smem[];
+  float* tmp = reinterpret_cast<float*>(smem + 2 * STAGE);
+  const int tid = threadIdx.x, lane = tid & 63;
+  const int wave = __builtin_amdgcn_readfirstlane(tid >> 6);
+
+  const float x_scale = dc_block_guard_scale(p.xAbound, CI, tmp);
+  const float dz_scale = dc_block_guard_scale(p.dzCoef + 6 * CO, CO, tmp);
+  const float w_scale = p.wp[W_SLOTS * 4];
+  const bool red_lds = p.redZ != nullptr && p.redZ == p.x;
+  const DcXcdRange tiles = dc_xcd_range(blockIdx.x, (int)gridDim.x, p.N * p.tilesX * p.tilesY);
+  const int nt = tiles.nt;
+  const long x_img = (long)p.H * p.W * CI;
+
+  if (wave >= 4) {
+    const int t = tid & 255;
+    const int q = t & 7, pb = t >> 3;
+    const int qx = t & 15, pbx = t >> 4;
+    const float* ct = p.dzCoef + 4 * q;
+    const f32x4 sc = *reinterpret_cast<const f32x4*>(ct), sh = *reinterpret_cast<const f32x4*>(ct + CO);
+    const f32x4 mu = *reinterpret_cast<const f32x4*>(ct + 2 * CO), A = *reinterpret_cast<const f32x4*>(ct + 3 * CO);
+    const f32x4 D = *reinterpret_cast<const f32x4*>(ct + 4 * CO), E = *reinterpret_cast<const f32x4*>(ct + 5 * CO);
+    const bool xbn = p.xSc != nullptr;
+    f32x4 x_sc = {1.f, 1.f, 1.f, 1.f}, x_sh = {0.f, 0.f, 0.f, 0.f};
+    if (xbn) { x_sc = *reinterpret_cast<const f32x4*>(p.xSc + 4 * qx); x_sh = *reinterpret_cast<const f32x4*>(p.xSh + 4 * qx); }
+    const bool drop = p.keep < 1.f;
+    const float inv_keep = drop ? 1.f / p.keep : 1.f;
+    const bool by_mask = drop && p.mask != nullptr, by_seed = drop && p.mask == nullptr;
+    const int H2 = 2 * p.H, W2 = 2 * p.W;
+    const long z_img = (long)H2 * W2 * CO;
+    const long da_img = (long)H2 * W2 * p.daLd;
+    const unsigned da_bytes = (unsigned)((((long)H2 * W2 - 1) * p.daLd + CO) * 4);
+    const unsigned da_row = (unsigned)(p.daLd * 4);
+    XSet x0, x1;
+    f32x4 ra[NLZ], rz[NLZ];
+    unsigned rm[NLZ];
+    unsigned live = 0u;
+    long gp0 = 0;
+    auto request_x = [&](int j, XSet& s) __attribute__((always_inline)) {
+      const Tile tl = decode(p, tiles, j);
+      const __amdgpu_buffer_rsrc_t rsX = dc_make_rsrc(p.x + tl.img * x_img, (unsigned)(x_img * 4));
+      s.live = 0u;
+#pragma unroll
+      for (int k = 0; k < NLX; ++k) {
+        const int y = tl.y0 + (k >> 1), xx = tl.x0 + pbx + 16 * (k & 1);
+        const bool ok = y < p.H && xx < p.W;
+        const unsigned off = ok ? (unsigned)(((y * p.W + xx) * CI + 4 * qx) * 4) : OOB;
+        s.r[k] = __builtin_bit_cast(f32x4, __builtin_amdgcn_raw_buffer_load_b128(rsX, off, 0, 0));
+        if (ok) s.live |= 1u << k;
+      }
+    };
+    auto stage_x = [&](const XSet& s, char* set) __attribute__((always_inline)) {
+#pragma unroll
+      for (int k = 0; k < NLX; ++k) {
+        const int px = pbx + 16 * k;
+        const bool lv = (s.live >> k) & 1u;
+        f32x4 xv;
+#pragma unroll
+        for (int e = 0; e < 4; ++e) {
+          const float xr = s.r[k][e];
+          xv[e] = xbn ? (lv ? fmaxf(__builtin_fmaf(xr, x_sc[e], x_sh[e]), 0.f) : 0.f) : xr;
+        }
+        u32x2 xh, xl;
+        dc_split_f16(xv, x_scale, xh, xl);
+        const int off = swz128(px * 128 + qx * 8);
+        *reinterpret_cast<u32x2*>(set + OFF_X_HI + off) = xh;
+        *reinterpret_cast<u32x2*>(set + OFF_X_LO + off) = xl;
+        if (red_lds) *reinterpret_cast<f32x4*>(set + OFF_RAW + (px * CI + 4 * qx) * 4) = s.r[k];
+      }
+    };
+    auto request_dz = [&](int j) __attribute__((always_inline)) {
+      const Tile tl = decode(p, tiles, j);
+      const __amdgpu_buffer_rsrc_t rsA = dc_make_rsrc(p.da + tl.img * da_img, da_bytes);
+      const __amdgpu_buffer_rsrc_t rsZ = dc_make_rsrc(p.z + tl.img * z_img, (unsigned)(z_img * 4));
+      const __amdgpu_buffer_rsrc_t rsM = dc_make_rsrc(by_mask ? p.mask + tl.img * z_img : nullptr, by_mask ? (unsigned)z_img : 0u);
+      live = 0u;
+#pragma unroll
+      for (int k = 0; k < NLZ; ++k) {
+        const int y = 2 * tl.y0 + (k >> 1), xx = 2 * tl.x0 + pb + 32 * (k & 1);
+        const bool ok = y < H2 && xx < W2;
+        const unsigned pix = ok ? (unsigned)(y * W2 + xx) : PIX_OOB;
+        rz[k] = __builtin_bit_cast(f32x4, __builtin_amdgcn_raw_buffer_load_b128(rsZ, pix * (CO * 4) + 16 * q, 0, 0));
+        ra[k] = __builtin_bit_cast(f32x4, __builtin_amdgcn_raw_buffer_load_b128(rsA, pix * da_row + 16 * q, 0, 0));
+        rm[k] = __builtin_amdgcn_raw_buffer_load_b32(rsM, pix * CO + 4 * q, 0, 0);
+        if (ok) live |= 1u << k;
+      }
+      gp0 = ((long)tl.img * H2 + 2 * tl.y0) * W2 + 2 * tl.x0 + pb;
+    };
+    auto stage_dz = [&](char* set) __attribute__((always_inline)) {
+#pragma unroll
+      for (int k = 0; k < NLZ; ++k) {
+        const bool lv = (live >> k) & 1u;
+        f32x4 f = {1.f, 1.f, 1.f, 1.f};
+        if (by_mask) {
+#pragma unroll
+          for (int e = 0; e < 4; ++e) f[e] = ((rm[k] >> (8 * e)) & 0xffu) ? inv_keep : 0.f;
+        } else if (by_seed) {
+          const uint64_t elem = (uint64_t)(gp0 + (long)(k >> 1) * W2 + 32 * (k & 1)) * CO + 4 * q;
+#pragma unroll
+          for (int e = 0; e < 4; ++e) f[e] = dc_keep_factor(p.seed, elem + e, p.keep, inv_keep);
+        }
+        f32x4 dzv;
+#pragma unroll
+        for (int e = 0; e < 4; ++e) {
+          const float v = drop ? dc_dz_on_load_drop(rz[k][e], ra[k][e], f[e], sc[e], sh[e], mu[e], A[e], D[e], E[e])
+                               : dc_dz_on_load(rz[k][e], ra[k][e], sc[e], sh[e], mu[e], A[e], D[e], E[e]);
+          dzv[e] = lv ? v : 0.f;
+        }
+        u32x2 dh, dl;
+        dc_split_f16(dzv, dz_scale, dh, dl);
+        const int a = (k >> 1) & 1, r = k >> 2, b = pb & 1, c = (pb >> 1) + 16 * (k & 1);
+        const int off = (2 * a + b) * TAP_STRIDE + swz64((r * TW + c) * 64 + q * 8);
+        *reinterpret_cast<u32x2*>(set + off) = dh;
+        *reinterpret_cast<u32x2*>(set + OFF_DZ_LO + off) = dl;
+      }
+    };
+    produce(smem, nt, x0, x1, request_x, request_dz, stage_x, stage_dz);
+    return;
+  }
+
+  const int li = lane & 31, h = lane >> 5;
+  if (wave < 2) {
+    const int wd = wave;
+    const float out_scale = 1.f / (dz_scale * w_scale);
+    const bool red = p.redZ != nullptr;
+    float gsc[2] = {0.f, 0.f}, gsh[2] = {0.f, 0.f}, rmu[2] = {0.f, 0.f}, ris[2] = {0.f, 0.f};
+    if (red) {
+#pragma unroll
+      for (int nb = 0; nb < 2; ++nb) {
+        rmu[nb] = p.redMean[nb * 32 + li]; ris[nb] = p.redInvstd[nb * 32 + li];
+        dc_bn_affine(rmu[nb], ris[nb], p.redGamma[nb * 32 + li], p.redBeta[nb * 32 + li], gsc[nb], gsh[nb]);
+      }
+    }
+    float s1[2] = {0.f, 0.f}, s2[2] = {0.f, 0.f}, amax[2] = {0.f, 0.f};
+    const int a_rel = (wd * TW + li) * 64 + h * 16;
+    u32x4 wreg[8][2][2];
+    {
+      const u32x4* wsrc = reinterpret_cast<const u32x4*>(p.wp) + h * 2 * CI + li;
+#pragma unroll
+      for (int g = 0; g < 8; ++g)
+#pragma unroll
+        for (int nb = 0; nb < 2; ++nb) {
+          wreg[g][nb][0] = wsrc[g * 4 * CI + nb * 32];
+          wreg[g][nb][1] = wsrc[g * 4 * CI + CI + nb * 32];
+        }
+    }
+    __syncthreads();
+    for (int i = 0; i < nt; ++i) {
+      const char* cur = smem + (i & 1) * STAGE;
+      int ar = a_rel;
+      asm volatile("" : "+v"(ar));
+      f32x16 acc[2];
+#pragma unroll
+      for (int nb = 0; nb < 2; ++nb)
+#pragma unroll
+        for (int r = 0; r < 16; ++r) acc[nb][r] = 0.f;
+      __builtin_amdgcn_s_setprio(2);
+      {
+        f16x8 ah[2], al[2];
+        auto fetch = [&](int g, int buf) __attribute__((always_inline)) {
+          const int ao = (g >> 1) * TAP_STRIDE + swz64(ar + (g & 1) * 32);
+          ah[buf] = __builtin_bit_cast(f16x8, *reinterpret_cast<const u32x4*>(cur + ao));
+          al[buf] = __builtin_bit_cast(f16x8, *reinterpret_cast<const u32x4*>(cur + OFF_DZ_LO + ao));
+        };
+        fetch(0, 0);
+#pragma unroll
+        for (int g = 0; g < 8; ++g) {
+          const int b = g & 1;
+          if (g + 1 < 8) fetch(g + 1, b ^ 1);
+          __builtin_amdgcn_sched_barrier(0);
+#pragma unroll
+          for (int nb = 0; nb < 2; ++nb)
+            dc_mfma3(ah[b], al[b], __builtin_bit_cast(f16x8, wreg[g][nb][0]), __builtin_bit_cast(f16x8, wreg[g][nb][1]), acc[nb]);
+          __builtin_amdgcn_sched_barrier(0);
+        }
+      }
+      __builtin_amdgcn_s_setprio(0);
+      const Tile tl = decode(p, tiles, i);
+      const __amdgpu_buffer_rsrc_t rsO = dc_make_rsrc(p.dx + tl.img * x_img, (unsigned)(x_img * 4));
+      const int oy = tl.y0 + wd, oxb = tl.x0 + 4 * h;
+      const bool row_ok = oy < p.H;
+      unsigned offs[16];
+#pragma unroll
+      for (int r = 0; r < 16; ++r) {
+        const int colc = (r & 3) + 8 * (r >> 2);
+        const bool ok = row_ok && (oxb + colc) < p.W;
+        offs[r] = ok ? (unsigned)(((oy * p.W + oxb + colc) * CI + li) * 4) : OOB;
+      }
+#pragma unroll
+      for (int nb = 0; nb < 2; ++nb) {
+        float zr[16];
+        if (red_lds) {
+          const float* raw = reinterpret_cast<const float*>(cur + OFF_RAW) + (wd * TW + 4 * h) * CI + nb * 32 + li;
+#pragma unroll
+          for (int r = 0; r < 16; ++r) zr[r] = raw[((r & 3) + 8 * (r >> 2)) * CI];
+        } else if (red) {
+          const __amdgpu_buffer_rsrc_t rsR = dc_make_rsrc(p.redZ + tl.img * x_img, (unsigned)(x_img * 4));
+#pragma unroll
+          for (int r = 0; r < 16; ++r) zr[r] = __builtin_bit_cast(float, __builtin_amdgcn_raw_buffer_load_b32(rsR, offs[r], nb * 128, 0));
+        }
+#pragma unroll
+        for (int r = 0; r < 16; ++r)
+          __builtin_amdgcn_raw_buffer_store_b32(__builtin_bit_cast(unsigned, acc[nb][r] * out_scale), rsO, offs[r], nb * 128, 0);
+        if (red) {
+#pragma unroll
+          for (int r = 0; r < 16; ++r)
+            dc_bnred_accum(acc[nb][r] * out_scale, zr[r], gsc[nb], gsh[nb], rmu[nb], ris[nb], !(offs[r] >> 31), s1[nb], s2[nb], amax[nb]);
+        }
+      }
+      __syncthreads();
+    }
+    if (red) {
+#pragma unroll
+      for (int nb = 0; nb < 2; ++nb) {
+        const float t1 = s1[nb] + __shfl_xor(s1[nb], 32), t2 = s2[nb] + __shfl_xor(s2[nb], 32);
+        const float am = fmaxf(amax[nb], __shfl_xor(amax[nb], 32));
+        if (h == 0) {
+          const long row = (long)blockIdx.x * 2 + wd;
+          const int ch = nb * 32 + li;
+          p.bnPartial[(row * CI + ch) * 2] = t1;
+          p.bnPartial[(row * CI + ch) * 2 + 1] = t2;
+          if (p.bnAmax) p.bnAmax[row * CI + ch] = am;
+        }
+      }
+    }
+    return;
+  }
+
+  const int ww = wave - 2;
+  const int cb = (lane >> 4) & 1, c16 = lane & 15, q4 = c16 >> 2, pp = c16 & 3;
+  const int fragz = (cb * 2 + (pp >> 1)) * 16 + (pp & 1) * 8;
+  const int fragx = (ww * 4 + cb * 2 + (pp >> 1)) * 16 + (pp & 1) * 8;
+  const int lane_z = (8 * h + q4) * 64 + fragz, lane_x = (8 * h + q4) * 128 + fragx;
+  f32x16 acc[4];
+#pragma unroll
+  for (int t = 0; t < 4; ++t)
+#pragma unroll
+    for (int r = 0; r < 16; ++r) acc[t][r] = 0.f;
+  __syncthreads();
+  for (int i = 0; i < nt; ++i) {
+    const char* cur = smem + (i & 1) * STAGE;
+    int lz = lane_z, lx = lane_x;
+    asm volatile("" : "+v"(lz), "+v"(lx));
+    __builtin_amdgcn_s_setprio(2);
+    {
+      f16x8 zh[2], zl[2], xh[2], xl[2];
+      auto fetch_z = [&](int g, int buf) __attribute__((always_inline)) {
+        const int rel = lz + 16 * (g >> 2) * 64;
+        const int a0 = (g & 3) * TAP_STRIDE + swz64(rel), a1 = (g & 3) * TAP_STRIDE + swz64(rel + 4 * 64);
+        zh[buf] = dc_tr_frag(cur, a0, a1);
+        zl[buf] = dc_tr_frag(cur + OFF_DZ_LO, a0, a1);
+      };
+      auto fetch_x = [&](int ks, int buf) __attribute__((always_inline)) {
+        const int rel = lx + 16 * ks * 128;
+        const int b0 = swz128(rel), b1 = swz128(rel + 4 * 128);
+        xh[buf] = dc_tr_frag(cur + OFF_X_HI, b0, b1);
+        xl[buf] = dc_tr_frag(cur + OFF_X_LO, b0, b1);
+      };
+      fetch_x(0, 0);
+      fetch_z(0, 0);
+#pragma unroll
+      for (int g = 0; g < 16; ++g) {
+        const int ks = g >> 2;
+        if (g + 1 < 16) {
+          fetch_z(g + 1, (g + 1) & 1);
+          if (((g + 1) & 3) == 0) fetch_x(ks + 1, (ks + 1) & 1);
+        }
+        __builtin_amdgcn_sched_barrier(0);
+        dc_mfma3(zh[g & 1], zl[g & 1], xh[ks & 1], xl[ks & 1], acc[g & 3]);
+        __builtin_amdgcn_sched_barrier(0);
+      }
+    }
+    __builtin_amdgcn_s_setprio(0);
+    __syncthreads();
+  }
+  const float ws_scale = 1.f / (x_scale * dz_scale);
+#pragma unroll
+  for (int tap = 0; tap < 4; ++tap) {
+    float* dst = p.slabs + ((long)blockIdx.x * 4 + tap) * CO * CI + 32 * ww + li;
+#pragma unroll
+    for (int r = 0; r < 16; ++r) dst[((r & 3) + 8 * (r >> 2) + 4 * h) * CI] = acc[tap][r] * ws_scale;
+  }
+}
+
+static int up_joint_grid(int N, int H, int W) {
+  static int cus[64] = {};
+  int dev = 0;
+  if (hipGetDevice(&dev) != hipSuccess || dev < 0 || dev >= 64) dev = 0;
+  if (cus[dev] == 0) {
+    int n = 0;
+    if (hipDeviceGetAttribute(&n, hipDeviceAttributeMultiprocessorCount, dev) != hipSuccess || n <= 0) return 0;
+    cus[dev] = n;
+  }
+  const long total = (long)N * dc_cdiv(W, uj::TW) * dc_cdiv(H, uj::TH);
+  return (int)(total < cus[dev] ? total : cus[dev]);
+}
+static bool up_joint_serves(int N, int H, int W, int Cin, int Cout) {
+  return N > 0 && H > 0 && Cin == uj::CI && Cout == uj::CO && W >= uj::TW && 4L * H * W < (long)uj::PIX_OOB &&
+         (long)N * dc_cdiv(W, uj::TW) * dc_cdiv(H, uj::TH) < (1L << 31);
+}
+
+extern "C" int dc_convT2x2_bwd_joint_blocks(int N, int H, int W, int Cin, int Cout) {
+  if (!up_joint_serves(N, H, W, Cin, Cout)) return 0;
+  return 2 * up_joint_grid(N, H, W);
+}
+extern "C" long dc_convT2x2_bwd_joint_ws_floats(int N, int H, int W, int Cin, int Cout) {
+  if (!up_joint_serves(N, H, W, Cin, Cout)) return 0;
+  return (long)up_joint_grid(N, H, W) * uj::SLAB + 32 * uj::SLAB;
+}
+extern "C" int dc_convT2x2_bwd_joint_f16x3(const float* z_in, const float* in_scale, const float* in_shift, const float* x_abound,
+                                           const float* da, long da_ld, const float* z, const float* dz_coef,
+                                           const uint8_t* mask, float keep, uint64_t seed, const void* wp16, float* dx,
+                                           const float* red_z, const float* red_mean, const float* red_invstd,
+                                           const float* red_gamma, const float* red_beta, float* bn_partial,
+                                           float* amax_partial, float* dw, float* ws, int N, int H, int W, int Cin, int Cout,
+                                           dc_stream_t stream) {
+  const char* fn = "dc_convT2x2_bwd_joint_f16x3";
+  DC_REQUIRE(z_in && da && z && dz_coef && wp16 && dx && dw && ws, DC_EINVAL, "%s: null pointer", fn);
+  DC_REQUIRE(dc_aligned16(z_in) && dc_aligned16(da) && dc_aligned16(z) && dc_aligned16(dz_coef) && dc_aligned16(wp16) && dc_aligned16(dx),
+             DC_EINVAL, "%s: pointers must be 16-byte aligned", fn);
+  DC_REQUIRE((in_scale == nullptr) == (in_shift == nullptr) && (!in_scale || (dc_aligned16(in_scale) && dc_aligned16(in_shift))), DC_EINVAL,
+             "%s: in_scale / in_shift go together, 16-byte aligned", fn);
+  DC_REQUIRE(red_z == nullptr || (red_mean && red_invstd && red_gamma && red_beta && bn_partial), DC_EINVAL,
+             "%s: red_z needs red_mean / red_invstd / red_gamma / red_beta / bn_partial", fn);
+  DC_REQUIRE(keep > 0.f && (mask == nullptr || dc_aligned(3, mask)), DC_EINVAL, "%s: keep must be positive, mask 4-byte aligned", fn);
+  DC_REQUIRE(up_joint_serves(N, H, W, Cin, Cout), DC_EUNSUP,
+             "%s: shape not served (dc_convT2x2_bwd_joint_blocks() == 0): use the separate kernels", fn);
+  DC_REQUIRE(da_ld >= Cout && da_ld % 4 == 0 && da_ld <= 128, DC_EINVAL, "%s: da_ld must be a multiple of 4 in [Cout, 128]", fn);
+  const int grid = up_joint_grid(N, H, W);
+  DC_REQUIRE(grid > 0, DC_EHIP, "%s: no device", fn);
+  static DcLdsAttr lds_attr;
+  if (int rc = dc_func_max_lds(lds_attr, reinterpret_cast<const void*>(convT_bwd_joint_kernel), uj::LDS_BYTES, fn)) return rc;
+  UpJointParams p;
+  p.x = z_in; p.xSc = in_scale; p.xSh = in_shift; p.xAbound = x_abound;
+  p.da = da; p.daLd = da_ld; p.z = z; p.dzCoef = dz_coef; p.mask = mask; p.keep = keep; p.seed = seed;
+  p.wp = reinterpret_cast<const float*>(wp16); p.dx = dx;
+  p.redZ = red_z; p.redMean = red_mean; p.redInvstd = red_invstd; p.redGamma = red_gamma; p.redBeta = red_beta;
+  p.bnPartial = bn_partial; p.bnAmax = amax_partial; p.slabs = ws;
+  p.N = N; p.H = H; p.W = W; p.tilesX = dc_cdiv(W, uj::TW); p.tilesY = dc_cdiv(H, uj::TH);
+  hipEvent_t ev0 = nullptr, ev1 = nullptr;
+  const bool bracket = dc_take_bracket(&ev0, &ev1);
+  if (bracket && ev0) (void)hipEventRecord(ev0, (hipStream_t)stream);
+  hipLaunchKernelGGL(convT_bwd_joint_kernel, dim3((unsigned)grid), dim3(uj::THREADS), uj::LDS_BYTES, (hipStream_t)stream, p);
+  if (bracket && ev1) (void)hipEventRecord(ev1, (hipStream_t)stream);
+  DC_CHECK_LAUNCH(fn);
+  return dc_reduce_partials(ws, grid, uj::SLAB, 1.0f, dw, ws + (long)grid * uj::SLAB, stream);
+}
diff --git a/deep_calcium_amd/csrc/tape_tramp.inc b/deep_calcium_amd/csrc/tape_tramp.inc
--- a/deep_calcium_amd/csrc/tape_tramp.inc
+++ b/deep_calcium_amd/csrc/tape_tramp.inc
@@ -41,6 +41,7 @@
 static int t_dc_conv3x3_c1_wgrad_dzin_zre(const DcArg* a) { return dc_conv3x3_c1_wgrad_dzin_zre((const float*)a[0].p, (const float*)a[1].p, (const float*)a[2].p, (const float*)a[3].p, (const float*)a[4].p, (float*)a[5].p, (float*)a[6].p, (int)a[7].l, (int)a[8].l, (int)a[9].l, (int)a[10].l, (dc_stream_t)a[11].p); }
 static int t_dc_conv3x3_bwd_joint_f16x3(const DcArg* a) { return dc_conv3x3_bwd_joint_f16x3((const float*)a[0].p, (const float*)a[1].p, (const float*)a[2].p, (const float*)a[3].p, (const float*)a[4].p, (const float*)a[5].p, (const float*)a[6].p, (const void*)a[7].p, (float*)a[8].p, (const float*)a[9].p, (const float*)a[10].p, (const float*)a[11].p, (const float*)a[12].p, (const float*)a[13].p, (float*)a[14].p, (float*)a[15].p, (float*)a[16].p, (float*)a[17].p, (int)a[18].l, (int)a[19].l, (int)a[20].l, (int)a[21].l, (int)a[22].l, (dc_stream_t)a[23].p); }
 static int t_dc_conv3x3_bwd_joint_r1_f16x3(const DcArg* a) { return dc_conv3x3_bwd_joint_r1_f16x3((const float*)a[0].p, (const float*)a[1].p, (const float*)a[2].p, (const float*)a[3].p, (const float*)a[4].p, (const float*)a[5].p, (const float*)a[6].p, (const float*)a[7].p, (const void*)a[8].p, (float*)a[9].p, (const float*)a[10].p, (const float*)a[11].p, (const float*)a[12].p, (const float*)a[13].p, (const float*)a[14].p, (float*)a[15].p, (float*)a[16].p, (float*)a[17].p, (float*)a[18].p, (int)a[19].l, (int)a[20].l, (int)a[21].l, (int)a[22].l, (int)a[23].l, (dc_stream_t)a[24].p); }
+static int t_dc_convT2x2_bwd_joint_f16x3(const DcArg* a) { return dc_convT2x2_bwd_joint_f16x3((const float*)a[0].p, (const float*)a[1].p, (const float*)a[2].p, (const float*)a[3].p, (const float*)a[4].p, (long)a[5].l, (const float*)a[6].p, (const float*)a[7].p, (const uint8_t*)a[8].p, (float)a[9].d, (uint64_t)a[10].u, (const void*)a[11].p, (float*)a[12].p, (const float*)a[13].p, (const float*)a[14].p, (const float*)a[15].p, (const float*)a[16].p, (const float*)a[17].p, (float*)a[18].p, (float*)a[19].p, (float*)a[20].p, (float*)a[21].p, (int)a[22].l, (int)a[23].l, (int)a[24].l, (int)a[25].l, (int)a[26].l, (dc_stream_t)a[27].p); }
 static int t_dc_bn_stats_reduce(const DcArg* a) { return dc_bn_stats_reduce((const double*)a[0].p, (int)a[1].l, (int)a[2].l, (int)a[3].l, (double*)a[4].p, (dc_stream_t)a[5].p); }
 static int t_dc_bn_stats_rows_fold(const DcArg* a) { return dc_bn_stats_rows_fold((const double*)a[0].p, (int)a[1].l, (int)a[2].l, (int)a[3].l, (int)a[4].l, (double*)a[5].p, (dc_stream_t)a[6].p); }
 static int t_dc_bn_stats_finalize_sums(const DcArg* a) { return dc_bn_stats_finalize_sums((const double*)a[0].p, (int)a[1].l, (double)a[2].d, (float)a[3].d, (float)a[4].d, (float*)a[5].p, (float*)a[6].p, (float*)a[7].p, (float*)a[8].p, (const float*)a[9].p, (const float*)a[10].p, (float*)a[11].p, (float*)a[12].p, (float*)a[13].p, (dc_stream_t)a[14].p); }
@@ -189,6 +190,7 @@
   {"dc_conv3x3_c1_wgrad_dzin_zre", t_dc_conv3x3_c1_wgrad_dzin_zre, 12, "pppppppllllp"},
   {"dc_conv3x3_bwd_joint_f16x3", t_dc_conv3x3_bwd_joint_f16x3, 24, "pppppppppppppppppplllllp"},
   {"dc_conv3x3_bwd_joint_r1_f16x3", t_dc_conv3x3_bwd_joint_r1_f16x3, 25, "ppppppppppppppppppplllllp"},
+  {"dc_convT2x2_bwd_joint_f16x3", t_dc_convT2x2_bwd_joint_f16x3, 28, "ppppplpppduppppppppppplllllp"},
   {"dc_bn_stats_reduce", t_dc_bn_stats_reduce, 6, "plllpp"},
   {"dc_bn_stats_rows_fold", t_dc_bn_stats_rows_fold, 7, "pllllpp"},
   {"dc_bn_stats_finalize_sums", t_dc_bn_stats_finalize_sums, 15, "pldddpppppppppp"},
diff --git a/deep_calcium_amd/net.py b/deep_calcium_amd/net.py
--- a/deep_calcium_amd/net.py
+++ b/deep_calcium_amd/net.py
@@ -142,6 +142,7 @@
         self.dzin_lvls = frozenset(range(5)) if _dz == 'all' else frozenset((0,))
         self.dzin_all = _dz == 'all'
         self.joint = self.dzin and _dz != '2'
+        self.up_joint = self.dzin
         self._head_bwd_done = False
         self.range_guard = self.mfma == 'f16x3'
         self.infer_measured = os.environ.get('DC_INFER_GUARD', '0') == '1'
@@ -394,7 +395,7 @@
         rec.append((e0, e1))
         return t
 
-    _TAPE_STATE = frozenset(('range_guard', 'bnin', 'dzin', 'dzin_lvls', 'dzin_all', 'joint', 'stats_per_wg', 'tail_main',
+    _TAPE_STATE = frozenset(('range_guard', 'bnin', 'dzin', 'dzin_lvls', 'dzin_all', 'joint', 'up_joint', 'stats_per_wg', 'tail_main',
                              'dz_writeback', 'deep_slots', 'c1_z_on_load', 'head_rank1', 'FOLD_MIN', 'bn_mode', 'streams', 'mfma', 'upsampling', 'up_drop',
                              'infer_measured', 'SLOTS', 'SLOTS_DEEP', 'SLOTS_DEEP_MAX_BYTES', '_side_stream', 'nm', 'use_tapes',
                              'ar_buckets'))
@@ -813,7 +814,8 @@
                 part_floats = max(part_floats, L.dc_conv3x3_bwd_joint_blocks(N, *self._hw(l.lvl), l.cin, l.cout) * l.cin * 2)
             elif l.kind == 'convT':
                 h, w = self._hw(l.lvl)
-                part_floats = max(part_floats, L.dc_convT2x2_dgrad_bnred_blocks(N, h // 2, w // 2, l.cin, l.cout) * l.cin * 2)
+                part_floats = max(part_floats, L.dc_convT2x2_dgrad_bnred_blocks(N, h // 2, w // 2, l.cin, l.cout) * l.cin * 2,
+                                  L.dc_convT2x2_bwd_joint_blocks(N, h // 2, w // 2, l.cin, l.cout) * l.cin * 2)
         sk = 4
         for l in self.layers:
             if l.kind == 'conv' and l.cin > 1 and self.mfma == 'f16x3':
@@ -846,7 +848,9 @@
         l0 = self.layers[0]
         T['wgrad_ws_main'] = torch.empty(max(L.dc_conv3x3_wgrad_ws_floats(N, self.H, self.W, l0.cin, l0.cout), 4), dtype=torch.float32,
                                          device=dev)
-        jws = max([L.dc_conv3x3_bwd_joint_ws_floats(N, *self._hw(l.lvl), l.cin, l.cout) for l in self.layers if l.kind == 'conv'] + [4])
+        jws = max([L.dc_conv3x3_bwd_joint_ws_floats(N, *self._hw(l.lvl), l.cin, l.cout) for l in self.layers if l.kind == 'conv'] +
+                  [L.dc_convT2x2_bwd_joint_ws_floats(N, self._hw(l.lvl)[0] // 2, self._hw(l.lvl)[1] // 2, l.cin, l.cout)
+                   for l in self.layers if l.kind == 'convT'] + [4])
         T['joint_ws'] = torch.empty(jws, dtype=torch.float32, device=dev)
         T['sums'] = torch.zeros(12, dtype=torch.float64, device=dev)
         T['bn_sums'] = torch.zeros(2 * max(l.cout for l in self.layers if l.kind != 'head'), dtype=torch.float64, device=dev)
@@ -1089,6 +1093,14 @@
         h, w = self._hw(l.lvl)
         return self.L.dc_conv3x3_bwd_joint_blocks(N, h, w, l.cin, l.cout) > 0
 
+    def _up_joint_rows(self, l, N, da_ld):
+        if not (self.up_joint and self.dzin and self.mfma == 'f16x3' and l.kind == 'convT' and da_ld <= 128):
+            return 0
+        if not self.dzin_all and N * self.H * self.W <= (1 << 20):
+            return 0
+        h, w = self._hw(l.lvl)
+        return self.L.dc_convT2x2_bwd_joint_blocks(N, h // 2, w // 2, l.cin, l.cout)
+
     def _dzin_ok(self, l, N):
         if not self.dzin or l.kind != 'conv' or l.drop > 0.0:
             return 0
@@ -1212,11 +1224,12 @@
             if dz_mode == 2 and dx_ptr is None:
                 dz_mode = 0
             dzin = dz_mode > 0
+            ujrows = self._up_joint_rows(l, N, da_ld) if dx_ptr is not None else 0
             k = state['slot']
             state['slot'] = (k + 1) % S
             if fused is None:
                 L.dc_bn_bwd_reduce(da_ptr, da_ld, _ptr(z), mean, invstd, gamma, beta, mptr, keep, seed,
-                                   _ptr(T['part_ws']), _ptr(T['amax_ws']) if dzin else None, pixels, l.cout, st)
+                                   _ptr(T['part_ws']), _ptr(T['amax_ws']) if (dzin or ujrows) else None, pixels, l.cout, st)
                 fused = (_ptr(T['part_ws']), _ptr(T['amax_ws']), L.dc_bn_bwd_blocks(pixels, l.cout))
             if two_streams and slot_free[k] is not None:
                 self._wait(mh, slot_free[k])
@@ -1296,6 +1309,26 @@
                         g_free[da_g] = ev
                 return fused_next
 
+            if ujrows > 0:
+                coef = _ptr(T['dz_coef'][k])
+                if gg is not None:
+                    L.dc_bn_bwd_finalize_dzin(None, fused[1], fused[2], l.cout, mean, invstd, gamma, beta, count,
+                                              _ptr(gg), _ptr(gg, l.cout), coef, self.pview(self.gflat, l, 'b'), st)
+                else:
+                    L.dc_bn_bwd_finalize_dzin(fused[0], fused[1], fused[2], l.cout, mean, invstd, gamma, beta, count,
+                                              dgamma, dbeta, coef, self.pview(self.gflat, l, 'b'), st)
+                xa = (bsrc[0], bsrc[1][0], bsrc[1][1]) if bsrc is not None else (x_in, None, None)
+                rargs, fused_next = (None,) * 7, None
+                if red is not None:
+                    rargs = (_ptr(T['z_' + red.name]), self.stat_ptr(red, 0), self.stat_ptr(red, 1),
+                             self.pview(self.pflat, red, 'gamma'), self.pview(self.pflat, red, 'beta'),
+                             _ptr(T['part_ws']), _ptr(T['amax_ws']))
+                    fused_next = (_ptr(T['part_ws']), _ptr(T['amax_ws']), ujrows)
+                L.dc_convT2x2_bwd_joint_f16x3(xa[0], xa[1], xa[2], self._ab_in(l), da_ptr, da_ld, _ptr(z), coef, mptr, keep, seed,
+                                              _ptr(self.wp_dgrad[l.name]), dx_ptr, *rargs, dk, _ptr(T['joint_ws']),
+                                              N, h // 2, w // 2, l.cin, l.cout, st)
+                return fused_next
+
             if r1 is not None:
                 raise DcunetError('block %s: the head wrote its rank-one gradient factors but the block takes the apply pass '
                                   '(_head_s_ok and block_bwd disagree)' % l.name)
diff --git a/include/dcunet.h b/include/dcunet.h
--- a/include/dcunet.h
+++ b/include/dcunet.h
@@ -7,7 +7,7 @@
 
 typedef void* dc_stream_t;
 
-#define DC_ABI_VERSION 130
+#define DC_ABI_VERSION 131
 int dc_version(void);
 const char* dc_last_error(void);
 
@@ -168,6 +168,15 @@
                                   float* dx, const float* red_z, const float* red_mean, const float* red_invstd,
                                   const float* red_gamma, const float* red_beta, float* bn_partial, float* amax_partial,
                                   float* dw, float* ws, int N, int H, int W, int Cin, int Cout, dc_stream_t stream);
+
+int dc_convT2x2_bwd_joint_blocks(int N, int H, int W, int Cin, int Cout);
+long dc_convT2x2_bwd_joint_ws_floats(int N, int H, int W, int Cin, int Cout);
+int dc_convT2x2_bwd_joint_f16x3(const float* z_in, const float* in_scale, const float* in_shift, const float* x_abound,
+                                const float* da, long da_ld, const float* z, const float* dz_coef, const uint8_t* mask,
+                                float keep, uint64_t seed, const void* wp16, float* dx, const float* red_z,
+                                const float* red_mean, const float* red_invstd, const float* red_gamma, const float* red_beta,
+                                float* bn_partial, float* amax_partial, float* dw, float* ws, int N, int H, int W, int Cin,
+                                int Cout, dc_stream_t stream);
 
 int dc_bn_stats_reduce(const double* partial, int parts, int groups, int C, double* sums, dc_stream_t stream);
 int dc_bn_stats_rows_fold(const double* partial, int parts, int groups, int C, int chunks, double* out, dc_stream_t stream);
```

Result: no change. 908.0 images/s (median of 6 runs) (+0.9%).
